# zaphB/freecad.optics_design_workbench

Measured on AMD Instinct MI355X. Metric: Monte-Carlo rays/sec (whole node), lensesAndMirrors.FCStd, higher is better.
Workload: dtype f64; 1 GPU; benchmark/lensesAndMirrors.FCStd, 1e+08 Monte-Carlo rays per step per GPU (BASELINE configs[2]), Gaussian point source sigma=1e-2, Philox4x32-10 seed 0x0D15EA5E; record_hit_rows=True, histogram=1024x1024 u64, parallelism=ray-index sharding x1, one RCCL reduce

## Files before the change

freecad/optics_design_workbench_amd/_native.py:

```python
import ctypes as C
import os
import shutil
import subprocess

import numpy as np

os.environ.setdefault('GPU_MAX_HW_QUEUES', '16')

_HERE = os.path.dirname(os.path.abspath(__file__))
CSRC = os.path.join(_HERE, 'csrc')
LIB_PATH = os.path.join(CSRC, 'libodw_trace.so')
_SOURCES = ['odw_capi.hip', 'odw_kernels.hip', 'odw_grid.hip', 'odw_mesh.hip', 'odw_posthoc.hip', 'odw_posthoc_batch.hip', 'odw_spec.hip', 'odw_device.h', 'odw_build.h']
_HEADER = os.path.normpath(os.path.join(_HERE, '..', '..', 'include', 'odw_trace.h'))

ABI_VERSION = 12
CNT_NAMES = ['traced_rays', 'recorded_hits', 'segments', 'escaped', 'died', 'capped',
             'hist_overflow', 'hits_dropped', 'grating_in_medium']
TRACE_RECORD_HITS, TRACE_HISTOGRAM, TRACE_RECORD_SEGMENTS, TRACE_POWER_HISTOGRAM = 1, 2, 4, 8
POWER_QUANTUM_BITS = 32
FLAG_FLIP_NORMAL, FLAG_CONVEX = 1, 2
COMPILE_OFF, COMPILE_STRUCTURE, COMPILE_AUTO = 0, 1, 2
COMPILE_MODES = {None: 0, False: 0, 'off': 0, 0: 0, 'structure': 1, 1: 1, True: 1, 'auto': 2, 2: 2}
ERRORS = {1: 'invalid argument', 2: 'device error', 3: 'no scene', 4: 'capacity', 5: 'unsupported'}
BUSY = 6

HIT_DTYPE = np.dtype([('point', '<f8', 3), ('direction', '<f8', 3), ('power', '<f8'), ('tag', '<u8')])
SEGMENT_DTYPE = np.dtype([('p1', '<f8', 3), ('p2', '<f8', 3), ('power', '<f8'), ('tag', '<u8')])

SYMBOLS = ['odw_abi_version', 'odw_create', 'odw_destroy', 'odw_last_error', 'odw_upload_scene',
           'odw_upload_source', 'odw_upload_surface_source', 'odw_generate_rays', 'odw_upload_surface_samplers', 'odw_set_surface_seed', 'odw_set_wavelength', 'odw_set_limits', 'odw_set_detector', 'odw_reserve_hits', 'odw_reserve_segments', 'odw_trace',
           'odw_trace_rays', 'odw_sync', 'odw_reset_results', 'odw_reset_hits', 'odw_fetch_counters', 'odw_hit_count',
           'odw_fetch_hits', 'odw_fetch_histogram', 'odw_segment_count', 'odw_fetch_segments', 'odw_reset_segments', 'odw_sample', 'odw_device_histogram',
           'odw_device_counters', 'odw_device_results', 'odw_stream', 'odw_timing_enable', 'odw_timing_read',
           'odw_swap_hit_lists', 'odw_fetch_swapped_hits', 'odw_release_swapped_hits', 'odw_mem_info', 'odw_host_alloc', 'odw_host_free', 'odw_load_hits', 'odw_hits_select', 'odw_hits_gather', 'odw_hits_project', 'odw_hits_range', 'odw_hits_bin', 'odw_hits_moments', 'odw_plane_screen',
           'odw_compile_scene', 'odw_compiled_info', 'odw_compile_check', 'odw_build_check', 'odw_hits_columns',
           'odw_upload_scene_batch', 'odw_trace_batch', 'odw_batch_select', 'odw_batch_rows',
           'odw_plane_screen_batch', 'odw_archive_append', 'odw_archive_select', 'odw_archive_reset', 'odw_batch_hits_select', 'odw_batch_hits_sample', 'odw_batch_hits_project', 'odw_batch_hits_bin',
           'odw_batch_reserve', 'odw_batch_hits_begin', 'odw_batch_hits_sampled', 'odw_batch_hits_measure', 'odw_batch_hits_measured',
           'odw_enable_power_histogram', 'odw_fetch_power_histogram', 'odw_device_power_histogram', 'odw_hits_bin_power', 'odw_compiled_power_info']

_pd = C.POINTER(C.c_double)
_pi = C.POINTER(C.c_int32)
_pu = C.POINTER(C.c_uint64)


class SceneDesc(C.Structure):
  _fields_ = [('n_prims', C.c_int32), ('prim_type', _pi), ('prim_group', _pi), ('prim_solid', _pi),
              ('prim_flags', _pi), ('prim_xform', _pd), ('prim_params', _pd), ('prim_cond_off', _pi),
              ('n_conds', C.c_int32), ('cond_prim', _pi), ('cond_inside', _pi),
              ('n_groups', C.c_int32), ('group_type', _pi), ('group_ior', _pd), ('group_refl', _pd),
              ('group_abslen', _pd), ('group_record', _pi), ('group_grating_type', _pi),
              ('group_grating_lpm', _pd), ('group_grating_dir', _pd), ('group_grating_order', _pi),
              ('seq_enabled', C.c_int32), ('seq_len', C.c_int32), ('seq_mask', _pu),
              ('ignore_mask', C.c_uint64), ('tri_normals', _pd), ('tri_edges', _pi)]


class SourceDesc(C.Structure):
  _fields_ = [('xform', C.c_double * 12), ('focal_length', C.c_double), ('wavelength', C.c_double),
              ('power', C.c_double), ('n_phi_knots', C.c_int32), ('phi_edges', _pd), ('phi_cdf', _pd),
              ('n_t_knots', C.c_int32), ('n_t_rows', C.c_int32), ('t_edges', _pd), ('t_cdf', _pd)]


class SurfaceSamplerDesc(C.Structure):
  _fields_ = [('group', C.c_int32), ('kind', C.c_int32), ('family_axis', C.c_int32), ('n_family', C.c_int32),
              ('family_lo', C.c_double), ('family_hi', C.c_double), ('n_phi_knots', C.c_int32),
              ('phi_edges', _pd), ('phi_cdf', _pd), ('n_t_knots', C.c_int32), ('n_t_rows', C.c_int32),
              ('t_edges', _pd), ('t_cdf', _pd), ('mu', C.c_double), ('n_atoms', C.c_int32),
              ('atom_mass', _pd), ('atom_theta', _pd), ('atom_phi', _pd)]


class SurfaceSourceDesc(C.Structure):
  _fields_ = [('wavelength', C.c_double), ('power', C.c_double), ('dist_tol', C.c_double),
              ('n_prims', C.c_int32), ('prim_type', _pi), ('prim_flags', _pi), ('prim_xform', _pd),
              ('prim_params', _pd), ('prim_cond_off', _pi), ('n_conds', C.c_int32), ('cond_prim', _pi),
              ('cond_inside', _pi), ('n_faces', C.c_int32), ('face_prim', _pi), ('face_id', _pi),
              ('face_area', _pd), ('n_t_knots', C.c_int32), ('t_edges', _pd), ('t_cdf', _pd), ('tri_normals', _pd)]


class LimitsDesc(C.Structure):
  _fields_ = [('max_ray_length', C.c_double), ('max_intersections', C.c_int32),
              ('dist_tol', C.c_double), ('power_tol', C.c_double)]


class DetectorDesc(C.Structure):
  _fields_ = [('group', C.c_int32), ('origin', C.c_double * 3), ('ex', C.c_double * 3),
              ('ey', C.c_double * 3), ('x_lo', C.c_double), ('x_hi', C.c_double),
              ('y_lo', C.c_double), ('y_hi', C.c_double), ('nx', C.c_int32), ('ny', C.c_int32)]


class NativeError(RuntimeError):
  pass


def hipcc():
  for cand in (os.environ.get('HIPCC'), '/opt/rocm/bin/hipcc', shutil.which('hipcc')):
    if cand and os.path.exists(cand):
      return cand
  raise NativeError('hipcc not found; the HIP library cannot be built')


def sources_hash(csrc=None, header=None):
  import hashlib
  csrc = CSRC if csrc is None else csrc
  header = _HEADER if header is None else header
  h = hashlib.sha256()
  for name in sorted(_SOURCES):
    path = os.path.join(csrc, name)
    h.update(name.encode() + b'\0')
    with open(path, 'rb') as f:
      h.update(f.read())
    h.update(b'\0')
  h.update(b'odw_trace.h\0')
  with open(header, 'rb') as f:
    h.update(f.read())
  return h.hexdigest()


def needs_build():
# ... 27 lines not shown
  runtime = subprocess.run([hipcc(), '--print-file-name=libclang_rt.asan-x86_64.so'], capture_output=True, text=True).stdout.strip()
  if not os.path.isabs(runtime) or not os.path.exists(runtime):
    raise NativeError('the sanitizer runtime of hipcc\'s clang was not found')
  deps = [os.path.join(CSRC, s) for s in _SOURCES] + [_HEADER]
  if force or not os.path.exists(ASAN_LIB_PATH) or any(os.path.getmtime(d) > os.path.getmtime(ASAN_LIB_PATH) for d in deps):
    cmd = [hipcc(), '--offload-arch=gfx950', '-O1', '-g', '-std=c++17', '-ffp-contract=on', '-fPIC', '-shared',
           '-fsanitize=address,undefined', '-fno-gpu-sanitize', '-fno-omit-frame-pointer', '-shared-libasan',
           '-o', ASAN_LIB_PATH + '.tmp', os.path.join(CSRC, 'odw_capi.hip')]
    res = subprocess.run(cmd, cwd=CSRC, capture_output=True, text=True)
    if res.returncode != 0:
      raise NativeError('hipcc (sanitized build) failed:\n' + res.stdout + res.stderr)
    os.replace(ASAN_LIB_PATH + '.tmp', ASAN_LIB_PATH)
  return ASAN_LIB_PATH, runtime


_lib = None


def lib():
  global _lib
  if _lib is None:
    if not os.path.exists(LIB_PATH):
      raise NativeError(f'{LIB_PATH} is missing: run __graft_entry__.build() '
                        f'(or freecad.optics_design_workbench_amd._native.build()) first')
    l = C.CDLL(os.environ.get('ODW_TRACE_LIB') or LIB_PATH)
    l.odw_last_error.restype = C.c_char_p
    l.odw_last_error.argtypes = [C.c_void_p]
    l.odw_create.argtypes = [C.c_int, C.POINTER(C.c_void_p)]
    l.odw_destroy.argtypes = [C.c_void_p]
    l.odw_destroy.restype = None
    for name in SYMBOLS:
      getattr(l, name)
    if l.odw_abi_version() != ABI_VERSION:
      raise NativeError('libodw_trace.so ABI version mismatch; rebuild')
    _lib = l
  return _lib


def check(ctx, rc, what):
  if rc != 0:
    msg = lib().odw_last_error(ctx)
    raise NativeError(f'{what}: {ERRORS.get(rc, rc)}: {msg.decode() if msg else ""}')


def _arr(a, dtype):
  return np.ascontiguousarray(a, dtype=dtype)


def scene_desc(sc):
  keep = dict(
      prim_type=_arr(sc.prim_type, np.int32), prim_group=_arr(sc.prim_group, np.int32),
      prim_solid=_arr(sc.prim_solid, np.int32), prim_flags=_arr(sc.prim_flags, np.int32),
      prim_xform=_arr(sc.prim_xform, np.float64), prim_params=_arr(sc.prim_params, np.float64),
      prim_cond_off=_arr(sc.prim_cond_off, np.int32), cond_prim=_arr(sc.cond_prim, np.int32),
      cond_inside=_arr(sc.cond_inside, np.int32), group_type=_arr(sc.group_type, np.int32),
      group_ior=_arr(sc.group_ior, np.float64), group_refl=_arr(sc.group_refl, np.float64),
      group_abslen=_arr(sc.group_abslen, np.float64), group_record=_arr(sc.group_record, np.int32),
      group_grating_type=_arr(sc.group_grating_type, np.int32),
      group_grating_lpm=_arr(sc.group_grating_lpm, np.float64),
      group_grating_dir=_arr(sc.group_grating_dir, np.float64),
      group_grating_order=_arr(sc.group_grating_order, np.int32),
      seq_mask=_arr(sc.seq_mask, np.uint64))
  if getattr(sc, 'tri_normals', None) is not None:
    keep_tri = _arr(sc.tri_normals, np.float64).reshape(-1, 9)
    if len(keep_tri) != len(sc.prim_type):
      raise ValueError('tri_normals needs one row of 9 values per primitive')
  d = SceneDesc()
  d.n_prims, d.n_conds, d.n_groups = len(keep['prim_type']), len(keep['cond_prim']), len(keep['group_type'])
  for name, typ in SceneDesc._fields_:
    if name in keep:
      setattr(d, name, keep[name].ctypes.data_as(typ))
  d.seq_enabled, d.seq_len, d.ignore_mask = int(sc.seq_enabled), len(keep['seq_mask']), int(sc.ignore_mask)
  if getattr(sc, 'tri_normals', None) is not None:
    keep['tri_normals'] = keep_tri
    d.tri_normals = keep_tri.ctypes.data_as(_pd)
  if getattr(sc, 'tri_edges', None) is not None:
    keep['tri_edges'] = _arr(sc.tri_edges, np.int32)
    if len(keep['tri_edges']) != len(sc.prim_type):
      raise ValueError('tri_edges needs one entry per primitive')
    d.tri_edges = keep['tri_edges'].ctypes.data_as(_pi)
  return d, keep


def compile_check(scene, limits, mode='structure', arch=None):
  d, keep = scene_desc(scene)
  lim = LimitsDesc(float(limits.max_ray_length), int(limits.max_intersections), float(limits.dist_tol),
                   float(limits.power_tol))
  buf = C.create_string_buffer(1 << 20)
  size = C.c_uint64(0)
  f = lib().odw_compile_check
  f.argtypes = [C.POINTER(SceneDesc), C.POINTER(LimitsDesc), C.c_int32, C.c_char_p, C.c_char_p, C.c_uint64,
                C.POINTER(C.c_uint64)]
  rc = f(C.byref(d), C.byref(lim), COMPILE_MODES[mode], arch.encode() if arch else None, buf, len(buf), C.byref(size))
  check(None, rc, 'odw_compile_check')
  return buf.value.decode(), int(size.value)


STRUCTURES = {0: 'flat', 1: 'grid', 2: 'bvh', 3: 'wide-bvh'}


def build_check(scene, limits, library=None):
  d, keep = scene_desc(scene)
  lim = LimitsDesc(float(limits.max_ray_length), int(limits.max_intersections), float(limits.dist_tol),
                   float(limits.power_tol))
  structure = C.c_int32(-1)
  sizes = (C.c_uint64 * 6)()
  f = (library or lib()).odw_build_check
  f.argtypes = [C.POINTER(SceneDesc), C.POINTER(LimitsDesc), C.POINTER(C.c_int32), C.POINTER(C.c_uint64)]
  rc = f(C.byref(d), C.byref(lim), C.byref(structure), sizes)
  if rc != 0:
    msg = (library or lib()).odw_last_error(None)
    raise NativeError(f'odw_build_check: {ERRORS.get(rc, rc)}: {msg.decode() if msg else ""}')
  names = ('primitives', 'nodes', 'grid_cells', 'grid_items', 'grid_lds_bytes', 'dead_primitives')
  return dict(structure=STRUCTURES[int(structure.value)], **{k: int(v) for k, v in zip(names, sizes)})


def source_desc(src):
  t = src.tables
  keep = dict(phi_edges=_arr(t.phi_edges, np.float64), phi_cdf=_arr(t.phi_cdf, np.float64),
              t_edges=_arr(t.t_edges, np.float64), t_cdf=_arr(t.t_cdf, np.float64).reshape(-1, len(t.t_edges)))
  d = SourceDesc()
  d.xform = (C.c_double * 12)(*np.asarray(src.xform, dtype=np.float64).reshape(12))
  d.focal_length, d.wavelength, d.power = float(src.focal_length), float(src.wavelength), float(src.power)
  d.n_phi_knots, d.n_t_knots, d.n_t_rows = len(keep['phi_edges']), len(keep['t_edges']), keep['t_cdf'].shape[0]
  for name in keep:
    setattr(d, name, keep[name].ctypes.data_as(_pd))
  return d, keep


def surface_sampler_descs(samplers):
  samplers = list(samplers or [])
  arr = (SurfaceSamplerDesc * max(1, len(samplers)))()
  keep = [arr]
  for d, s in zip(arr, samplers):
    phi_edges, phi_cdf = _arr(s.phi_edges, np.float64), _arr(s.phi_cdf, np.float64)
    t_edges, t_cdf = _arr(s.t_edges, np.float64), _arr(s.t_cdf, np.float64)
    keep += [phi_edges, phi_cdf, t_edges, t_cdf]
    d.group, d.kind, d.family_axis, d.n_family = int(s.group), int(s.kind), int(s.axis), int(s.n_family)
    d.family_lo, d.family_hi = float(s.lo), float(s.hi)
    d.n_phi_knots, d.n_t_knots, d.n_t_rows = len(phi_edges), len(t_edges), int(t_cdf.shape[-2])
    for name, a in (('phi_edges', phi_edges), ('phi_cdf', phi_cdf), ('t_edges', t_edges), ('t_cdf', t_cdf)):
      setattr(d, name, a.ctypes.data_as(_pd))
    d.mu = float(getattr(s, 'mu', 0.0))
    d.n_atoms = int(getattr(s, 'n_atoms', 0) or 0)
    if d.n_atoms:
      for name in ('atom_mass', 'atom_theta', 'atom_phi'):
        a = _arr(getattr(s, name), np.float64)
        keep.append(a)
        setattr(d, name, a.ctypes.data_as(_pd))
  return arr, len(samplers), keep


def surface_source_desc(src):
  keep = dict(prim_type=_arr(src.prim_type, np.int32), prim_flags=_arr(src.prim_flags, np.int32),
              prim_xform=_arr(src.prim_xform, np.float64), prim_params=_arr(src.prim_params, np.float64),
              prim_cond_off=_arr(src.prim_cond_off, np.int32),
              cond_prim=_arr(src.cond_prim if len(src.cond_prim) else [0], np.int32),
              cond_inside=_arr(src.cond_inside if len(src.cond_inside) else [0], np.int32),
              face_prim=_arr(src.face_prim, np.int32), face_id=_arr(src.face_id, np.int32),
              face_area=_arr(src.face_area, np.float64), t_edges=_arr(src.t_edges, np.float64),
              t_cdf=_arr(src.t_cdf, np.float64))
  if getattr(src, 'tri_normals', None) is not None:
    keep['tri_normals'] = _arr(src.tri_normals, np.float64).reshape(-1, 9)
    if len(keep['tri_normals']) != len(keep['prim_type']):
      raise ValueError('tri_normals needs one row of 9 values per primitive')
  d = SurfaceSourceDesc()
  d.wavelength, d.power, d.dist_tol = float(src.wavelength), float(src.power), float(src.dist_tol)
  d.n_prims, d.n_conds, d.n_faces = len(keep['prim_type']), len(src.cond_prim), len(keep['face_prim'])
  d.n_t_knots = len(keep['t_edges'])
  for name, typ in SurfaceSourceDesc._fields_:
    if name in keep:
      setattr(d, name, keep[name].ctypes.data_as(typ))
  return d, keep
```

freecad/optics_design_workbench_amd/csrc/odw_build.h:

```cpp
#pragma once

#include <algorithm>
#include <cmath>
#include <cstdint>
#include <cstdio>
#include <cstring>
#include <limits>
#include <map>
#include <string>
#include <utility>
#include <vector>

namespace {

using namespace odw;

struct HostScene {
  std::vector<double> prim_f64;
  std::vector<int32_t> prim_i32;
  std::vector<int32_t> cond;
  std::vector<double> prim_hdr;
  std::vector<char> dead;
  std::vector<double> group_f64, group_gdir;
  std::vector<int32_t> group_i32;
  std::vector<uint64_t> seq;
  bool lean = false;
  int32_t n_prims = 0, n_groups = 0, seq_enabled = 0, seq_len = 0;
  uint64_t all_mask = 0, ignore_mask = 0;
};

inline int refuse(std::string& err, int code, const char* msg) {
  err = msg;
  return code;
}

int32_t pack_cond(int32_t prim, int32_t inside) {
  return (int32_t)((uint32_t)prim | ((uint32_t)(inside >> 1) & 1u) << 30 | ((uint32_t)inside & 1u) << 31);
}

bool clauses_marked(const int32_t* cond_off, int n, const std::vector<int32_t>& cond) {
  for (int p = 0; p < n; ++p) {
    const int off = cond_off[p], end = cond_off[p + 1];
    if (end <= off || cond_opens(cond[off])) continue;
    for (int c = off + 1; c < end; ++c)
      if (cond_opens(cond[c])) return false;
  }
  return true;
}

int scene_host_tables(const odw_scene_desc* s, HostScene& hs, std::string& err) {
  if (!s) return refuse(err, ODW_ERR_INVALID, "odw_upload_scene: null argument");
  if (s->n_prims < 0 || s->n_groups < 0 || s->n_groups > ODW_MAX_GROUPS || s->seq_len < 0 ||
      s->seq_len > ODW_MAX_SEQUENCE || s->n_conds < 0 || s->n_conds >= (1 << 24))
    return refuse(err, ODW_ERR_INVALID, "odw_upload_scene: counts out of range");
  if ((s->n_prims > 0 && (!s->prim_type || !s->prim_group || !s->prim_flags || !s->prim_xform || !s->prim_params ||
                          !s->prim_cond_off)) ||
      (s->n_conds > 0 && (!s->cond_prim || !s->cond_inside)) ||
      (s->n_groups > 0 && (!s->group_type || !s->group_ior || !s->group_refl || !s->group_abslen || !s->group_record)) ||
      (s->seq_len > 0 && !s->seq_mask))
    return refuse(err, ODW_ERR_INVALID, "odw_upload_scene: null table pointer");
  const int n = s->n_prims;
  int max_solid = 0;
  for (int p = 0; p < n && s->prim_solid; ++p) max_solid = std::max(max_solid, s->prim_solid[p]);
  hs.prim_f64.assign((size_t)n * 16, 0.0);
  hs.prim_i32.assign((size_t)n * 4, 0);
  for (int p = 0; p < n; ++p) {
    const int type = s->prim_type[p], group = s->prim_group[p];
    if (type < ODW_PRIM_BOX || type > ODW_PRIM_PARABOLOID) return refuse(err, ODW_ERR_UNSUPPORTED, "unknown primitive type");
    if (group < 0 || group >= s->n_groups) return refuse(err, ODW_ERR_INVALID, "primitive group out of range");
    const int off = s->prim_cond_off[p], cnt = s->prim_cond_off[p + 1] - off;
    if (off < 0 || cnt < 0 || cnt > 255 || off + cnt > s->n_conds)
      return refuse(err, ODW_ERR_INVALID, "bad condition offsets");
    if (type == ODW_PRIM_TRIANGLE) {
      if (cnt) return refuse(err, ODW_ERR_UNSUPPORTED, "triangles cannot carry trimming conditions");
      const double* v = s->prim_xform + 12 * (size_t)p;
      double* d = &hs.prim_f64[16 * (size_t)p];
      double e1[3], e2[3], e3[3], nn[3];
      for (int k = 0; k < 3; ++k) { d[k] = v[k]; e1[k] = v[3 + k] - v[k]; e2[k] = v[6 + k] - v[k]; e3[k] = e2[k] - e1[k]; }
      nn[0] = e1[1] * e2[2] - e1[2] * e2[1];
      nn[1] = e1[2] * e2[0] - e1[0] * e2[2];
      nn[2] = e1[0] * e2[1] - e1[1] * e2[0];
      const double a2 = std::sqrt(nn[0] * nn[0] + nn[1] * nn[1] + nn[2] * nn[2]);
      if (!(a2 > 0) || !std::isfinite(a2)) return refuse(err, ODW_ERR_INVALID, "degenerate triangle");
      auto len3 = [](const double* x) { return std::sqrt(x[0] * x[0] + x[1] * x[1] + x[2] * x[2]); };
      for (int k = 0; k < 3; ++k) { d[3 + k] = e1[k]; d[6 + k] = e2[k]; d[9 + k] = nn[k] / a2; }
      d[12] = len3(e2) / a2;
      d[13] = len3(e1) / a2;
      d[14] = len3(e3) / a2;
      const int face_edges = s->tri_edges ? s->tri_edges[p] : 7;
      for (int k = 0; k < 3; ++k)
        if (!((face_edges >> k) & 1)) d[12 + k] = -d[12 + k];
      d[15] = 0.0;
    } else {
      std::memcpy(&hs.prim_f64[16 * (size_t)p], s->prim_xform + 12 * (size_t)p, 12 * sizeof(double));
      std::memcpy(&hs.prim_f64[16 * (size_t)p + 12], s->prim_params + 4 * (size_t)p, 4 * sizeof(double));
      if (type == ODW_PRIM_SPHERE) {
        const double* m = &hs.prim_f64[16 * (size_t)p];
        for (int k = 0; k < 3; ++k)
          hs.prim_f64[16 * (size_t)p + 13 + k] = -(m[k] * m[3] + m[4 + k] * m[7] + m[8 + k] * m[11]);
      }
      if (type == ODW_PRIM_PARABOLOID) {
        double* par = &hs.prim_f64[16 * (size_t)p + 12];
        if (!(par[0] > 0) || !(par[1] > 0)) return refuse(err, ODW_ERR_INVALID, "paraboloid: focal length and height must be positive");
        par[2] = 2.0 * std::sqrt(par[0] * par[1]);
      }
    }
    hs.prim_i32[4 * p] = type;
    hs.prim_i32[4 * p + 1] = group;
    const int solid = s->prim_solid ? s->prim_solid[p] : 0;
    const bool fits = s->prim_solid && solid >= 0 && solid < 0x7fff && max_solid < 0x7fff;
    hs.prim_i32[4 * p + 2] = ((s->prim_flags[p] & 0xffff & ~ODW_FLAG_ISOLATED) & (fits ? ~0 : ~ODW_FLAG_CONVEX)) | ((fits ? solid : 0x7fff) << ODW_SOLID_SHIFT);
    hs.prim_i32[4 * p + 3] = off | (cnt << 24);
  }
  std::vector<int32_t> cond((size_t)std::max(1, s->n_conds), 0);
  for (int c = 0; c < s->n_conds; ++c) {
    if (s->cond_prim[c] < 0 || s->cond_prim[c] >= n || s->cond_prim[c] >= (1 << 30))
      return refuse(err, ODW_ERR_INVALID, "condition primitive out of range");
    if (s->prim_type[s->cond_prim[c]] == ODW_PRIM_TRIANGLE)
      return refuse(err, ODW_ERR_UNSUPPORTED, "trimming against a triangle (no inside/outside of a facet)");
    if (s->cond_inside[c] < 0 || s->cond_inside[c] > 3)
      return refuse(err, ODW_ERR_INVALID, "cond_inside: bit 0 inside, bit 1 opens a clause; nothing else");
    cond[c] = pack_cond(s->cond_prim[c], s->cond_inside[c]);
  }
  if (!clauses_marked(s->prim_cond_off, n, cond))
    return refuse(err, ODW_ERR_INVALID, "a trimming list of several clauses must mark its first condition too");
  hs.cond = cond;
  std::vector<double> gf(ODW_MAX_GROUPS * 4, 0.0), gd(ODW_MAX_GROUPS * 3, 0.0);
  std::vector<int32_t> gi(ODW_MAX_GROUPS * 4, 0);
  hs.lean = true;
  for (int g = 0; g < s->n_groups; ++g)
// ... 868 lines not shown
```

freecad/optics_design_workbench_amd/csrc/odw_capi.hip:

```cpp
#include <hip/hip_runtime.h>
#include <hipcub/hipcub.hpp>

#include <algorithm>
#include <atomic>
#include <array>
#include <cmath>
#include <cstdio>
#include <cstdlib>
#include <cstring>
#include <condition_variable>
#include <functional>
#include <mutex>
#include <new>
#include <thread>
#include <string>
#include <utility>
#include <vector>

#include "odw_kernels.hip"
#include "odw_grid.hip"
#include "odw_mesh.hip"
#include "odw_build.h"

using namespace odw;

namespace {

constexpr int kGuide = 1 << 16;
constexpr uint32_t kHitBlock = 512;
constexpr uint64_t kHitBlockMinRows = 1ull << 16;
static inline uint64_t hit_block_room(uint64_t capacity, uint64_t waves, uint64_t block) { return capacity * 64 / block + 64 + waves * block; }
constexpr int kPhiGuide = 1 << 8;
constexpr int kSurfaceGuide = 1 << 10;
constexpr int kBvhThreshold = 64;

std::string g_error;

struct DevBuf {
  void* p = nullptr;
  size_t bytes = 0;
};

}

struct odw_ctx {
  int device = 0;
  hipStream_t stream = nullptr;
  void* up_pin = nullptr;
  size_t up_off = 0;
  bool up_unstaged = false;
  int n_cu = 256;
  std::string err;

  HostScene hs;
  int compile_mode = 0;
  bool spec_dirty = true;
  hipFunction_t spec_fn = nullptr;
  bool spec_lean = false, spec_stoch = false;
  bool spec_pending = false;
  std::string spec_key;
  uint64_t spec_hot_rays = 50000000;
  double spec_seconds = 0;
  int spec_cache_hit = 0;
  bool have_scene = false, have_source = false, have_limits = false;
  bool bvh_dirty = true;
  int flat_limit = kBvhThreshold;

  DevBuf prim_f64, prim_hdr, prim_i32, cond_i32, group_f64, group_i32, group_gdir, seq_mask;
  DevBuf bvh_nodes, bvh_prims, tri_nrm;
  DevBuf bvh_leaf, bvh_wide;
  DevBuf grid_bounds, grid_cells, grid_items, dbg;
  DevBuf phi_tab, t_tab, t_guide, phi_guide, d_source, d_det;
  DeviceSource h_source;
  DeviceDetector h_det;
  DevBuf hits, hit_count, chunk_counter;
  DevBuf results, hist, counters;
  DevBuf segs, seg_count;
  uint64_t seg_capacity = 0;
  DevBuf ray_o, ray_d, ray_p, ray_aos, samp_t, samp_phi;
  DevBuf sort_keys[2], sort_vals[2], sort_tmp, sorted_rows;
  DevBuf ph_sel_entering, ph_flags, ph_x, ph_y, ph_sorted, ph_small, ph_part, ph_edges, ph_edges_b, ph_counts, ph_sel_hist;
  DevBuf ph_accel;
  DevBuf ph_bitmap, ph_before, ph_row_of;
  uint64_t alt_hit_ray_end = 0;
  uint64_t hit_ray_end = 0;
  uint64_t hit_ray_begin = 0, alt_hit_ray_begin = 0;
  uint64_t ph_n = 0, ph_n_entering = 0;
  int ph_group = -1;
  bool ph_valid = false, ph_projected = false, ph_entering_built = false;
  std::vector<double> ph_moment_sums;
  unsigned ph_moment_grid = 0;
  struct SurfaceBufs { DevBuf phi_tab, t_tab, t_guide, atom_mass; };
  std::vector<SurfaceBufs> surf_bufs;
  DevBuf d_samplers, d_group_sampler;
  int n_samplers = 0;
  uint64_t surface_seed = 0;
  DevBuf em_prim_f64, em_prim_i32, em_cond, em_face_i32, em_face_cdf, em_t_tab, em_t_guide, em_o, em_d, em_tri_nrm;
  DeviceEmitter h_emitter;
  bool emitter_active = false;
  uint64_t hit_capacity = 0, n_bins = 0;
  bool power_on = false;
  uint64_t hit_slots = 0;
  DevBuf batch_values, batch_hits, batch_hit_count, batch_rays_buf;
  int batch_n = 0;
  size_t batch_prims = 0;
  bool batch_launch = false;
  uint64_t batch_stride = 0;
  uint64_t batch_seg_slots = 0, batch_seg_capacity = 0, batch_rays = 0, batch_first = 0;
  int batch_traced = 0;
  bool batch_rows_ok = false;
  bool batch_marked = false;
  bool batch_pts = false;
  int batch_selected = -1;
  std::string batch_spec_text;
  hipFunction_t spec_batch_fn = nullptr;
  bool spec_batch_failed = false;
  hipFunction_t spec_power_fn = nullptr;
  bool spec_power_failed = false;
  const std::atomic<bool>* spec_power_wait = nullptr;
  DevBuf own_hits, own_hit_count;
  uint64_t own_capacity = 0, own_slots = 0, own_ray_begin = 0, own_ray_end = 0;
  DevBuf archive, archive_count;
  uint64_t archive_slots = 0, archive_unused = 0, archive_ray_begin = 0, archive_ray_end = 0;
  bool archive_selected = false;
  DevBuf phb_row_of, phb_words, phb_sel, phb_small, phb_rows, phb_x, phb_y, phb_part, phb_sel_hist, phb_cand, phb_counts;
  DevBuf phb_scenes, phb_hist, phb_planes, phb_strides, phb_origins, phb_accel, phb_pts;
  void* phb_pin_p = nullptr;
  size_t phb_pin_bytes = 0;
  hipEvent_t phb_ev = nullptr;
  int phb_stage = 0, phb_S = 0;
  uint64_t phb_cap = 0, phb_nbins = 0, phb_keep = 0;
  size_t phb_part_stride = 0;
  std::vector<double> phb_edges_host;
  int phb_edges_na = 0, phb_edges_nb = 0, phb_edges_polar = -1;
  std::vector<uint64_t> phb_used, phb_n, phb_leaving;
  std::vector<int32_t> phb_ordered;
  std::vector<char> phb_on;
  uint64_t phb_xy_stride = 0;
  int phb_group = -1;
// ... 179 lines not shown
  const uint64_t row = t >> 2;
  if (row < n) {
    const double2* src = reinterpret_cast<const double2*>(hits + order[row]);
    reinterpret_cast<double2*>(out + row)[t & 3] = src[t & 3];
  }
}

}
#include "odw_spec.hip"
namespace {

int presort_rays(odw_ctx* ctx, uint64_t first, uint64_t n, uint64_t seed) {
  const bool off = getenv("ODW_MESH_PRESORT") && getenv("ODW_MESH_PRESORT")[0] == '0';
  const char* e_min = getenv("ODW_MESH_PRESORT_MIN");
  const uint64_t min_rays = e_min ? (uint64_t)atoll(e_min) : (1ull << 16);
  if (off || n < min_rays || n > 0x7FFFFFFFull) return ODW_OK;
  int rc;
  for (int k = 0; k < 2; ++k) {
    if ((rc = ensure(ctx, ctx->sort_keys[k], n * sizeof(uint64_t)))) return rc;
    if ((rc = ensure(ctx, ctx->sort_vals[k], n * sizeof(uint32_t)))) return rc;
  }
  const DeviceScene& sc = ctx->P.scene;
  double lo[3], scale[3];
  for (int a = 0; a < 3; ++a) {
    lo[a] = sc.wide_lo[a];
    const double w = sc.wide_hi[a] - sc.wide_lo[a];
    scale[a] = w > 0 ? 1024.0 / w : 0.0;
  }
  uint64_t* k_in = (uint64_t*)ctx->sort_keys[0].p;
  uint64_t* k_out = (uint64_t*)ctx->sort_keys[1].p;
  uint32_t* v_in = (uint32_t*)ctx->sort_vals[0].p;
  uint32_t* v_out = (uint32_t*)ctx->sort_vals[1].p;
  const bool dir_only = ctx->h_source.finite_focal && ctx->h_source.focal_length == 0.0;
  const unsigned kgrid = (unsigned)((n + 255) / 256);
  size_t tmp_bytes = 0;
  if (dir_only) {
    uint32_t* k32_in = (uint32_t*)k_in;
    uint32_t* k32_out = (uint32_t*)k_out;
    hipLaunchKernelGGL(odw_ray_key_kernel<uint32_t>, dim3(kgrid), dim3(256), 0, ctx->stream, ctx->P.source, first, n, seed,
                       lo[0], lo[1], lo[2], scale[0], scale[1], scale[2], k32_in, v_in);
    HIPCHK(ctx, hipGetLastError());
    HIPCHK(ctx, hipcub::DeviceRadixSort::SortPairs(nullptr, tmp_bytes, k32_in, k32_out, v_in, v_out, (int)n, 0, 32, ctx->stream));
    if ((rc = ensure(ctx, ctx->sort_tmp, tmp_bytes))) return rc;
    HIPCHK(ctx, hipcub::DeviceRadixSort::SortPairs(ctx->sort_tmp.p, tmp_bytes, k32_in, k32_out, v_in, v_out, (int)n, 0, 32, ctx->stream));
  } else {
    hipLaunchKernelGGL(odw_ray_key_kernel<uint64_t>, dim3(kgrid), dim3(256), 0, ctx->stream, ctx->P.source, first, n, seed,
                       lo[0], lo[1], lo[2], scale[0], scale[1], scale[2], k_in, v_in);
    HIPCHK(ctx, hipGetLastError());
    HIPCHK(ctx, hipcub::DeviceRadixSort::SortPairs(nullptr, tmp_bytes, k_in, k_out, v_in, v_out, (int)n, 0, 62, ctx->stream));
    if ((rc = ensure(ctx, ctx->sort_tmp, tmp_bytes))) return rc;
    HIPCHK(ctx, hipcub::DeviceRadixSort::SortPairs(ctx->sort_tmp.p, tmp_bytes, k_in, k_out, v_in, v_out, (int)n, 0, 62, ctx->stream));
  }
  ctx->P.ray_order = v_out;
  ctx->ph_valid = false;
  return ODW_OK;
}


enum class TraceKernel { flat = kAccelFlat, grid = kAccelGrid, tree = kAccelTree, mesh = kAccelWide, compiled };

TraceKernel choose_kernel(const odw_ctx* ctx, uint32_t flags, bool batch) {
  const DeviceScene& S = ctx->P.scene;
  const bool segments = (flags & ODW_TRACE_RECORD_SEGMENTS) != 0, stoch = ctx->n_samplers > 0;
  const hipFunction_t fn = batch ? ctx->spec_batch_fn : (flags & ODW_TRACE_POWER_HISTOGRAM) ? ctx->spec_power_fn : ctx->spec_fn;
  if (fn && ctx->spec_lean == ctx->hs.lean && ctx->spec_stoch == stoch && !segments) return TraceKernel::compiled;
  return (TraceKernel)accel_kind(ctx->P.grid.nx > 0 && !stoch && !segments, S.n_nodes != 0, S.bvh_leaf != nullptr && !segments);
}

int launch_trace(odw_ctx* ctx, uint64_t first, uint64_t n, uint64_t seed, uint32_t flags,
                 const double* ray_o, const double* ray_d, const double* ray_p) {
  const bool explicit_rays = ray_o != nullptr;
  if (!ctx->have_scene || !ctx->have_limits) return fail(ctx, ODW_ERR_NO_SCENE, "scene/limits not uploaded");
  if (!explicit_rays && !ctx->have_source) return fail(ctx, ODW_ERR_NO_SCENE, "source not uploaded");
  if (n == 0) return ODW_OK;
  ctx->ph_valid = false;
  if (!ctx->batch_launch) {
    ctx->hit_ray_begin = ctx->hit_ray_end ? std::min<uint64_t>(ctx->hit_ray_begin, first) : first;
    ctx->hit_ray_end = std::max<uint64_t>(ctx->hit_ray_end, std::min<uint64_t>(first + n, 1ull << 48));
  }
  if (ctx->bvh_dirty) {
    int rc = build_bvh(ctx);
    if (rc) return rc;
  }
  if (ctx->spec_dirty) {
    if (spec_bind(ctx) != ODW_OK) ctx->spec_fn = nullptr;
  }
  if ((flags & ODW_TRACE_RECORD_HITS) && (ctx->batch_launch ? ctx->batch_seg_capacity : ctx->hit_capacity) == 0)
    return fail(ctx, ODW_ERR_CAPACITY, "ODW_TRACE_RECORD_HITS without odw_reserve_hits");
  if (flags & ODW_TRACE_RECORD_SEGMENTS) {
    if (ctx->seg_capacity == 0)
      return fail(ctx, ODW_ERR_CAPACITY, "ODW_TRACE_RECORD_SEGMENTS without odw_reserve_segments");
    if (first + n > ODW_SEG_MAX_RAY || ctx->P.lim.max_intersections > ODW_SEG_MAX_ORDINAL)
      return fail(ctx, ODW_ERR_INVALID, "ODW_TRACE_RECORD_SEGMENTS: ray index or max_intersections beyond the row tag");
  }
  if ((flags & ODW_TRACE_HISTOGRAM) && !ctx->P.det_enabled) flags &= ~ODW_TRACE_HISTOGRAM;
  if (!(flags & ODW_TRACE_HISTOGRAM) || !ctx->power_on) flags &= ~(uint32_t)ODW_TRACE_POWER_HISTOGRAM;
  TraceParams& P = ctx->P;
  const bool batch = ctx->batch_launch;
  std::memset(&P.batch, 0, sizeof P.batch);
  if (batch) {
    if (P.scene.n_nodes || P.grid.nx > 0 || ctx->n_samplers > 0 || explicit_rays || (flags & ODW_TRACE_RECORD_SEGMENTS))
      return fail(ctx, ODW_ERR_UNSUPPORTED, "odw_trace_batch: batches are traced by the flat kernels (analytic scenes of up to 64 "
                                            "primitives, no stochastic surfaces, no segment rows)");
    flags &= ~(uint32_t)(ODW_TRACE_HISTOGRAM | ODW_TRACE_POWER_HISTOGRAM);
  }
  P.first_ray = first;
  P.n_rays = n;
  P.seed = seed;
  P.flags = flags;
  P.samplers = (const DeviceSurfaceSampler*)ctx->d_samplers.p;
  P.group_sampler = (const int32_t*)ctx->d_group_sampler.p;
  P.ray_origins = ray_o;
  P.ray_dirs = ray_d;
  P.ray_powers = ray_p;
  P.ray_stride = n;
  P.dbg = (unsigned long long*)ctx->dbg.p;
  P.out.hits = (odw_hit*)(batch ? ctx->batch_hits.p : ctx->hits.p);
  P.out.hit_capacity = batch ? ctx->batch_seg_slots : ctx->hit_slots;
  P.out.hit_block = 0;
  P.out.hit_count = (unsigned long long*)(batch ? ctx->batch_hit_count.p : ctx->hit_count.p);
  P.out.hist = (unsigned long long*)ctx->hist.p;
  P.out.counters = (unsigned long long*)ctx->counters.p;
  P.out.chunk_counter = (unsigned long long*)ctx->chunk_counter.p;
  P.out.segs = (odw_segment*)ctx->segs.p;
  P.out.seg_capacity = ctx->seg_capacity;
  P.out.seg_count = (unsigned long long*)ctx->seg_count.p;
  P.out.row_of = (batch && ctx->batch_marked && (flags & ODW_TRACE_RECORD_HITS)) ? (uint32_t*)ctx->phb_row_of.p : nullptr;
  P.out.row_stride = batch ? (n + 31) / 32 * 32 : 0;
  P.out.pts = (P.out.row_of && ctx->batch_pts) ? (double*)ctx->phb_pts.p : nullptr;

  constexpr int grid_mult = 8;
  const bool pw = (flags & ODW_TRACE_POWER_HISTOGRAM) != 0;
  if (pw && ctx->spec_fn && !ctx->spec_power_fn && !ctx->spec_power_failed &&
      !(ctx->spec_power_wait && !ctx->spec_power_wait->load())) {
    const std::string keep_err = ctx->err;
    const bool waited = ctx->spec_power_wait != nullptr;
    ctx->spec_power_wait = nullptr;
    if (spec_bind(ctx, kSpecPower) != ODW_OK || (!ctx->spec_power_fn && (waited || !ctx->spec_power_wait))) {
      ctx->spec_power_fn = nullptr;
      ctx->spec_power_failed = true;
      ctx->err = keep_err;
    }
  }
  if (batch && ctx->spec_fn && !ctx->spec_batch_fn && !ctx->spec_batch_failed) {
    const std::string keep_err = ctx->err;
    if (spec_bind(ctx, kSpecBatch) != ODW_OK) {
      ctx->spec_batch_fn = nullptr;
      ctx->spec_batch_failed = true;
      ctx->err = keep_err;
    }
  }
  const TraceKernel kernel = choose_kernel(ctx, flags, batch);
  const bool use_spec = kernel == TraceKernel::compiled, use_grid = kernel == TraceKernel::grid, use_mesh = kernel == TraceKernel::mesh,
             use_tree = kernel == TraceKernel::tree;
  {
    const bool ring = use_grid || use_mesh;
    const uint64_t waves = (uint64_t)ctx->n_cu * 16;
    const uint64_t want = ring ? std::max<uint64_t>(64, std::min<uint64_t>(256, n / (waves * 32)))
                               : std::max<uint64_t>(512, std::min<uint64_t>(1024, n / (waves * 4)));
    P.chunk = (uint32_t)(want & ~(uint64_t)63);
  }
  uint64_t n_chunks = (n + P.chunk - 1) / P.chunk;
  if (batch) {
    const uint64_t total = n * (uint64_t)ctx->batch_traced, waves = (uint64_t)ctx->n_cu * 16;
    P.chunk = (uint32_t)(std::max<uint64_t>(512, std::min<uint64_t>(1024, total / (waves * 4))) & ~(uint64_t)63);
    const uint64_t cps = (n + P.chunk - 1) / P.chunk;
// ... 254 lines not shown
  release(ctx->d_samplers);
  release(ctx->d_group_sampler);
  for (DevBuf* b : {&ctx->grid_bounds, &ctx->grid_cells, &ctx->grid_items}) release(*b);
  for (DevBuf* b : {&ctx->ph_bitmap, &ctx->ph_before, &ctx->ph_row_of}) release(*b);
  for (DevBuf* b : {&ctx->ph_sel_entering, &ctx->ph_flags, &ctx->ph_x, &ctx->ph_y, &ctx->ph_sorted, &ctx->ph_small,
                    &ctx->ph_part, &ctx->ph_edges, &ctx->ph_edges_b, &ctx->ph_counts, &ctx->ph_sel_hist, &ctx->ph_accel})
    release(*b);
  release(ctx->archive);
  release(ctx->archive_count);
  release(ctx->batch_values);
  release(ctx->batch_rays_buf);
  release(ctx->batch_hits);
  release(ctx->batch_hit_count);
  if (ctx->phb_pin_p) (void)hipHostFree(ctx->phb_pin_p);
  if (ctx->up_pin) (void)hipHostFree(ctx->up_pin);
  if (ctx->phb_ev) (void)hipEventDestroy(ctx->phb_ev);
  for (DevBuf* b : {&ctx->phb_row_of, &ctx->phb_words, &ctx->phb_sel, &ctx->phb_small, &ctx->phb_rows, &ctx->phb_x, &ctx->phb_y,
                    &ctx->phb_part, &ctx->phb_sel_hist, &ctx->phb_cand, &ctx->phb_counts, &ctx->phb_scenes, &ctx->phb_hist, &ctx->phb_planes,
                    &ctx->phb_strides, &ctx->phb_origins, &ctx->phb_accel, &ctx->phb_pts})
    release(*b);
  release(ctx->alt_hits);
  release(ctx->alt_hit_count);
  if (ctx->alt_ready) (void)hipEventDestroy(ctx->alt_ready);
  if (ctx->copy_stream) (void)hipStreamDestroy(ctx->copy_stream);
  if (ctx->stream) (void)hipStreamDestroy(ctx->stream);
  delete ctx;
}


int odw_upload_scene(odw_ctx* ctx, const odw_scene_desc* s) {
  if (!ctx) return fail(ctx, ODW_ERR_INVALID, "odw_upload_scene: null argument");
  HostScene hs;
  std::string err;
  int rc = scene_host_tables(s, hs, err);
  if (rc) return fail(ctx, rc, err);
  ctx->hs = std::move(hs);
  HIPCHK(ctx, hipSetDevice(ctx->device));
  const int n = s->n_prims;
  const std::vector<int32_t>& cond = ctx->hs.cond;
  const std::vector<double>&gf = ctx->hs.group_f64, &gd = ctx->hs.group_gdir;
  const std::vector<int32_t>& gi = ctx->hs.group_i32;
  const std::vector<uint64_t>& seq = ctx->hs.seq;
  if ((rc = upload(ctx, ctx->prim_f64, ctx->hs.prim_f64.data(), ctx->hs.prim_f64.size() * sizeof(double)))) return rc;
  if ((rc = upload(ctx, ctx->prim_i32, ctx->hs.prim_i32.data(), ctx->hs.prim_i32.size() * sizeof(int32_t)))) return rc;
  if ((rc = upload(ctx, ctx->cond_i32, cond.data(), cond.size() * sizeof(int32_t)))) return rc;
  if ((rc = upload(ctx, ctx->group_f64, gf.data(), gf.size() * sizeof(double)))) return rc;
  if ((rc = upload(ctx, ctx->group_i32, gi.data(), gi.size() * sizeof(int32_t)))) return rc;
  if ((rc = upload(ctx, ctx->group_gdir, gd.data(), gd.size() * sizeof(double)))) return rc;
  if ((rc = upload(ctx, ctx->seq_mask, seq.data(), seq.size() * sizeof(uint64_t)))) return rc;
  if (s->tri_normals && n > 0) {
    if ((rc = upload(ctx, ctx->tri_nrm, s->tri_normals, (size_t)n * 9 * sizeof(double)))) return rc;
  }
  if ((rc = upload_done(ctx))) return rc;
  DeviceScene& d = ctx->P.scene;
  d.n_prims = ctx->hs.n_prims;
  d.n_groups = ctx->hs.n_groups;
  d.n_nodes = 0;
  d.seq_enabled = ctx->hs.seq_enabled;
  d.seq_len = ctx->hs.seq_len;
  d.all_mask = ctx->hs.all_mask;
  d.ignore_mask = ctx->hs.ignore_mask;
  d.tri_nrm = (s->tri_normals && n > 0) ? (const double*)ctx->tri_nrm.p : nullptr;
  d.prim_f64 = (const double*)ctx->prim_f64.p;
  d.prim_i32 = (const int32_t*)ctx->prim_i32.p;
  d.cond_i32 = (const int32_t*)ctx->cond_i32.p;
  d.group_f64 = (const double*)ctx->group_f64.p;
  d.group_i32 = (const int32_t*)ctx->group_i32.p;
  d.group_gdir = (const double*)ctx->group_gdir.p;
  d.seq_mask = (const uint64_t*)ctx->seq_mask.p;
  ctx->have_scene = true;
  ctx->bvh_dirty = true;
  ctx->spec_dirty = true;
  ctx->spec_fn = nullptr;
  ctx->n_samplers = 0;
  ctx->batch_n = 0;
  return ODW_OK;
}

int odw_compile_scene(odw_ctx* ctx, int32_t mode) {
  if (!ctx || mode < ODW_COMPILE_OFF || mode > ODW_COMPILE_AUTO) return fail(ctx, ODW_ERR_INVALID, "odw_compile_scene: bad argument");
  ctx->compile_mode = mode;
  ctx->spec_dirty = true;
  ctx->spec_fn = nullptr;
  if (mode == ODW_COMPILE_OFF || !ctx->have_scene || !ctx->have_limits) return ODW_OK;
  HIPCHK(ctx, hipSetDevice(ctx->device));
  if (ctx->bvh_dirty) {
    int rc = build_bvh(ctx);
    if (rc) return rc;
  }
  return spec_bind(ctx);
}

int odw_compiled_info(odw_ctx* ctx, int32_t* bound, double* compile_seconds, int32_t* cache_hit) {
  if (!ctx) return fail(ctx, ODW_ERR_INVALID, "odw_compiled_info: null context");
  if (bound) *bound = (ctx->spec_fn && !ctx->spec_dirty && !ctx->bvh_dirty) ? ctx->compile_mode : 0;
  if (compile_seconds) *compile_seconds = ctx->spec_seconds;
  if (cache_hit) *cache_hit = ctx->spec_cache_hit;
  return ODW_OK;
}

int odw_compiled_power_info(odw_ctx* ctx, int32_t* bound) {
  if (!ctx || !bound) return fail(ctx, ODW_ERR_INVALID, "odw_compiled_power_info: bad argument");
  *bound = (ctx->spec_fn && ctx->spec_power_fn && !ctx->spec_dirty && !ctx->bvh_dirty) ? ctx->compile_mode : 0;
  return ODW_OK;
}

int odw_compile_check(const odw_scene_desc* scene, const odw_limits* limits, int32_t mode, const char* arch,
                      char* header_out, uint64_t header_capacity, uint64_t* code_bytes) {
  if (!scene || !limits || mode != ODW_COMPILE_STRUCTURE)
    return fail(nullptr, ODW_ERR_INVALID, "odw_compile_check: bad argument");
  HostScene tmp;
  std::string refusal;
  int rc = scene_host_tables(scene, tmp, refusal);
  if (rc) return fail(nullptr, rc, refusal);
  std::vector<Box> boxes;
  compute_boxes(tmp, limits->dist_tol, boxes);
  const std::string why = spec_ineligible(tmp);
  if (!why.empty()) return fail(nullptr, ODW_ERR_UNSUPPORTED, "odw_compile_check: " + why);
  const std::string text = spec_text(tmp, 0);
  if (header_out && header_capacity) {
    const size_t k = std::min<size_t>(text.size(), (size_t)header_capacity - 1);
    std::memcpy(header_out, text.data(), k);
    header_out[k] = 0;
  }
  std::vector<char> code;
  std::string err;
  if (!spec_compile(text, arch && *arch ? arch : "gfx950", code, err))
    return fail(nullptr, ODW_ERR_DEVICE, err);
  if (code_bytes) *code_bytes = code.size();
  return ODW_OK;
}

int odw_build_check(const odw_scene_desc* scene, const odw_limits* limits, int32_t* structure, uint64_t* sizes) {
  if (!scene || !limits) return fail(nullptr, ODW_ERR_INVALID, "odw_build_check: null argument");
  if (!(limits->dist_tol > 0) || limits->max_intersections < 0 || !(limits->max_ray_length > 0))
    return fail(nullptr, ODW_ERR_INVALID, "odw_build_check: limits out of range");
  int flat_limit = kBvhThreshold;
  if (const char* e = getenv("ODW_BVH_THRESHOLD")) flat_limit = atoi(e);
  HostScene tmp;
  SceneAccel A;
  std::string err;
  int rc = scene_host_tables(scene, tmp, err);
  if (!rc) {
    std::vector<Box> boxes;
    compute_boxes(tmp, limits->dist_tol, boxes);
    rc = build_accel(tmp, std::move(boxes), limits->dist_tol, flat_limit, build_options(), A, err);
  }
  if (rc) return fail(nullptr, rc, err);
  if (structure) *structure = A.kind();
  if (sizes) {
    uint64_t dead = 0;
    for (char d : tmp.dead) dead += d ? 1 : 0;
    sizes[0] = (uint64_t)tmp.n_prims;
    sizes[1] = (uint64_t)A.nodes.size();
    sizes[2] = (uint64_t)A.grid.nx * (uint64_t)A.grid.ny * (uint64_t)A.grid.nz;
    sizes[3] = (uint64_t)A.grid.n_items;
    sizes[4] = (uint64_t)A.grid.lds_bytes;
    sizes[5] = dead;
  }
  return ODW_OK;
}

int odw_upload_surface_samplers(odw_ctx* ctx, const odw_surface_sampler_desc* samplers, int32_t n) {
  if (!ctx || n < 0 || (n && !samplers)) return fail(ctx, ODW_ERR_INVALID, "odw_upload_surface_samplers: bad argument");
  if (!ctx->have_scene) return fail(ctx, ODW_ERR_NO_SCENE, "odw_upload_surface_samplers before odw_upload_scene");
  HIPCHK(ctx, hipSetDevice(ctx->device));
  if (n == 0 && ctx->n_samplers == 0) return ODW_OK;
  HIPCHK(ctx, hipStreamSynchronize(ctx->stream));
  ctx->n_samplers = 0;
  ctx->spec_dirty = true;
  if (n == 0) return ODW_OK;
  std::vector<int32_t> gs(ODW_MAX_GROUPS * 2, -1);
  std::vector<DeviceSurfaceSampler> ds((size_t)n);
  if ((int)ctx->surf_bufs.size() < n) ctx->surf_bufs.resize((size_t)n);
  for (int i = 0; i < n; ++i) {
    const odw_surface_sampler_desc& s = samplers[i];
    if (s.group < 0 || s.group >= ctx->P.scene.n_groups || s.kind < ODW_SURF_PRIMARY || s.kind > ODW_SURF_MODIFY)
      return fail(ctx, ODW_ERR_INVALID, "surface sampler: group/kind out of range");
    for (int j = gs[2 * s.group + s.kind]; j >= 0; j = ds[(size_t)j].next)
      if (ds[(size_t)j].mu == s.mu) return fail(ctx, ODW_ERR_INVALID, "surface sampler: duplicate (group, kind, mu)");
    if (s.n_atoms < 0 || s.n_atoms > ODW_SURF_MAX_ATOMS || (s.n_atoms && (!s.atom_mass || !s.atom_theta || !s.atom_phi)))
      return fail(ctx, ODW_ERR_INVALID, "surface sampler: atoms");
    for (int k = 0; k < s.n_family * s.n_atoms; ++k)
      if (!(s.atom_mass[k] >= 0.0 && s.atom_mass[k] <= 1.0)) return fail(ctx, ODW_ERR_INVALID, "surface sampler: atom probability outside [0, 1]");
    if (s.n_family < 1 || s.family_axis < ODW_SURF_AXIS_NONE || s.family_axis > ODW_SURF_AXIS_THETA_REFL ||
        (s.family_axis == ODW_SURF_AXIS_NONE && s.n_family != 1) ||
        (s.n_family > 1 && !(s.family_hi > s.family_lo)))
      return fail(ctx, ODW_ERR_INVALID, "surface sampler: family");
    if (s.n_phi_knots < 2 || s.n_t_knots < 2 || s.n_t_rows < 1 ||
        (s.n_t_rows != 1 && s.n_t_rows != s.n_phi_knots - 1))
      return fail(ctx, ODW_ERR_INVALID, "surface sampler: table shape");
    if (!s.phi_edges || !s.phi_cdf || !s.t_edges || !s.t_cdf)
      return fail(ctx, ODW_ERR_INVALID, "surface sampler: null table pointer");
    const size_t np = (size_t)s.n_phi_knots, nt = (size_t)s.n_t_knots, rows = (size_t)s.n_t_rows, nf = (size_t)s.n_family;
    std::vector<double> ptab(nf * np * 2), ttab(nf * rows * nt * 2);
    std::vector<int32_t> guide(nf * rows * (kSurfaceGuide + 1));
    for (size_t k = 0; k < nf; ++k) {
      const double* pc = s.phi_cdf + k * np;
      if (pc[0] != 0.0 || pc[np - 1] != 1.0) return fail(ctx, ODW_ERR_INVALID, "surface sampler: phi cdf must run from 0 to 1");
      for (size_t j = 0; j < np; ++j) {
        if (j && pc[j] < pc[j - 1]) return fail(ctx, ODW_ERR_INVALID, "surface sampler: cdf not monotone");
        ptab[(k * np + j) * 2] = pc[j];
        ptab[(k * np + j) * 2 + 1] = s.phi_edges[j];
      }
      for (size_t r = 0; r < rows; ++r) {
        const double* cdf = s.t_cdf + (k * rows + r) * nt;
        if (cdf[0] != 0.0 || cdf[nt - 1] != 1.0) return fail(ctx, ODW_ERR_INVALID, "surface sampler: theta cdf rows must run from 0 to 1");
        double* dst = ttab.data() + (k * rows + r) * nt * 2;
        for (size_t j = 0; j < nt; ++j) {
          if (j && cdf[j] < cdf[j - 1]) return fail(ctx, ODW_ERR_INVALID, "surface sampler: cdf not monotone");
          dst[2 * j] = cdf[j];
          dst[2 * j + 1] = s.t_edges[j];
        }
        int32_t* g = guide.data() + (k * rows + r) * (kSurfaceGuide + 1);
        size_t j = 0;
        for (int q = 0; q <= kSurfaceGuide; ++q) {
          const double x = (double)q / (double)kSurfaceGuide;
          while (j + 1 < nt && cdf[j + 1] <= x) ++j;
          g[q] = (int32_t)j;
        }
      }
    }
    odw_ctx::SurfaceBufs& sb = ctx->surf_bufs[(size_t)i];
    int rc;
    if ((rc = upload(ctx, sb.phi_tab, ptab.data(), ptab.size() * sizeof(double)))) return rc;
    if ((rc = upload(ctx, sb.t_tab, ttab.data(), ttab.size() * sizeof(double)))) return rc;
    if ((rc = upload(ctx, sb.t_guide, guide.data(), guide.size() * sizeof(int32_t)))) return rc;
    HIPCHK(ctx, hipStreamSynchronize(ctx->stream));
    DeviceSurfaceSampler& d = ds[(size_t)i];
    d.phi_tab = (const double*)sb.phi_tab.p;
    d.t_tab = (const double*)sb.t_tab.p;
    d.t_guide = (const int32_t*)sb.t_guide.p;
    d.n_phi_knots = s.n_phi_knots;
    d.n_t_knots = s.n_t_knots;
    d.n_t_rows = s.n_t_rows;
    d.n_guide = kSurfaceGuide;
    d.axis = s.family_axis;
    d.n_family = s.n_family;
    d.lo = s.family_lo;
    d.inv_step = s.n_family > 1 ? (double)(s.n_family - 1) / (s.family_hi - s.family_lo) : 0.0;
    d.mu = s.mu;
    d.n_atoms = s.n_atoms;
    d.atom_mass = nullptr;
    std::memset(d.atom_theta, 0, sizeof d.atom_theta);
    std::memset(d.atom_phi, 0, sizeof d.atom_phi);
    if (s.n_atoms) {
      if ((rc = upload(ctx, sb.atom_mass, s.atom_mass, (size_t)s.n_family * (size_t)s.n_atoms * sizeof(double)))) return rc;
      HIPCHK(ctx, hipStreamSynchronize(ctx->stream));
      d.atom_mass = (const double*)sb.atom_mass.p;
      for (int j = 0; j < s.n_atoms; ++j)
        for (int c = 0; c < 3; ++c) { d.atom_theta[j][c] = s.atom_theta[3 * j + c]; d.atom_phi[j][c] = s.atom_phi[3 * j + c]; }
    }
    d.next = gs[2 * s.group + s.kind];
    gs[2 * s.group + s.kind] = i;
  }
  int rc;
  if ((rc = upload(ctx, ctx->d_samplers, ds.data(), ds.size() * sizeof(DeviceSurfaceSampler)))) return rc;
  if ((rc = upload(ctx, ctx->d_group_sampler, gs.data(), gs.size() * sizeof(int32_t)))) return rc;
  HIPCHK(ctx, hipStreamSynchronize(ctx->stream));
  ctx->n_samplers = n;
  return ODW_OK;
}

int odw_set_wavelength(odw_ctx* ctx, double wavelength_nm) {
  if (!ctx || !(wavelength_nm > 0)) return fail(ctx, ODW_ERR_INVALID, "odw_set_wavelength: bad argument");
  ctx->P.wavelength = wavelength_nm;
  return ODW_OK;
}

int odw_set_surface_seed(odw_ctx* ctx, uint64_t seed) {
  if (!ctx) return fail(ctx, ODW_ERR_INVALID, "odw_set_surface_seed: null ctx");
  ctx->surface_seed = seed;
  return ODW_OK;
}

int odw_upload_source(odw_ctx* ctx, const odw_source_desc* s) {
  if (!ctx || !s) return fail(ctx, ODW_ERR_INVALID, "odw_upload_source: null argument");
  if (s->n_phi_knots < 2 || s->n_t_knots < 2 || s->n_t_rows < 1 ||
      (s->n_t_rows != 1 && s->n_t_rows != s->n_phi_knots - 1))
    return fail(ctx, ODW_ERR_INVALID, "odw_upload_source: table shape");
  if (!s->phi_edges || !s->phi_cdf || !s->t_edges || !s->t_cdf)
    return fail(ctx, ODW_ERR_INVALID, "odw_upload_source: null table pointer");
  HIPCHK(ctx, hipSetDevice(ctx->device));
  const int np = s->n_phi_knots, nt = s->n_t_knots, rows = s->n_t_rows;
  if (s->phi_cdf[0] != 0.0 || s->phi_cdf[np - 1] != 1.0)
    return fail(ctx, ODW_ERR_INVALID, "phi cdf must run from 0 to 1");
  std::vector<double> ptab((size_t)np * 2), ttab((size_t)rows * nt * 2);
  for (int i = 0; i < np; ++i) { ptab[2 * i] = s->phi_cdf[i]; ptab[2 * i + 1] = s->phi_edges[i]; }
  std::vector<int32_t> guide((size_t)rows * (kGuide + 1));
  for (int r = 0; r < rows; ++r) {
    const double* cdf = s->t_cdf + (size_t)r * nt;
    if (cdf[0] != 0.0 || cdf[nt - 1] != 1.0) return fail(ctx, ODW_ERR_INVALID, "theta cdf rows must run from 0 to 1");
    double* dst = ttab.data() + (size_t)r * nt * 2;
    for (int i = 0; i < nt; ++i) {
      if (i && cdf[i] < cdf[i - 1]) return fail(ctx, ODW_ERR_INVALID, "cdf not monotone");
      dst[2 * i] = cdf[i];
      dst[2 * i + 1] = s->t_edges[i];
    }
    int32_t* g = guide.data() + (size_t)r * (kGuide + 1);
    int j = 0;
    for (int k = 0; k <= kGuide; ++k) {
      const double x = (double)k / (double)kGuide;
      while (j + 1 < nt && cdf[j + 1] <= x) ++j;
      g[k] = j;
    }
  }
  int rc;
  if ((rc = upload(ctx, ctx->phi_tab, ptab.data(), ptab.size() * sizeof(double)))) return rc;
  if ((rc = upload(ctx, ctx->t_tab, ttab.data(), ttab.size() * sizeof(double)))) return rc;
  if ((rc = upload(ctx, ctx->t_guide, guide.data(), guide.size() * sizeof(int32_t)))) return rc;
  std::vector<int32_t> pguide(kPhiGuide + 1);
  for (int k = 0, j = 0; k <= kPhiGuide; ++k) {
    const double x = (double)k / (double)kPhiGuide;
    while (j + 1 < np && s->phi_cdf[j + 1] <= x) ++j;
    pguide[k] = j;
  }
  if ((rc = upload(ctx, ctx->phi_guide, pguide.data(), pguide.size() * sizeof(int32_t)))) return rc;
  HIPCHK(ctx, hipStreamSynchronize(ctx->stream));
  DeviceSource& d = ctx->h_source;
  std::memcpy(d.m, s->xform, sizeof d.m);
  d.focal_length = s->focal_length;
  d.finite_focal = std::isfinite(s->focal_length) ? 1 : 0;
  d.wavelength = s->wavelength;
  d.power = s->power;
  d.phi_tab = (const double*)ctx->phi_tab.p;
  d.t_tab = (const double*)ctx->t_tab.p;
  d.t_guide = (const int32_t*)ctx->t_guide.p;
  d.phi_guide = (const int32_t*)ctx->phi_guide.p;
  d.n_phi_guide = kPhiGuide;
  d.n_phi_knots = np;
  d.n_t_knots = nt;
  d.n_t_rows = rows;
  d.n_guide = kGuide;
  if ((rc = upload(ctx, ctx->d_source, &ctx->h_source, sizeof(DeviceSource)))) return rc;
  HIPCHK(ctx, hipStreamSynchronize(ctx->stream));
  ctx->P.source = (const DeviceSource*)ctx->d_source.p;
  ctx->P.wavelength = s->wavelength;
  ctx->have_source = true;
  ctx->emitter_active = false;
  return ODW_OK;
}

int odw_upload_surface_source(odw_ctx* ctx, const odw_surface_source_desc* s) {
  if (!ctx || !s) return fail(ctx, ODW_ERR_INVALID, "odw_upload_surface_source: null argument");
  if (s->n_prims < 1 || s->n_faces < 1 || s->n_conds < 0 || s->n_t_knots < 2 || !(s->dist_tol > 0))
    return fail(ctx, ODW_ERR_INVALID, "odw_upload_surface_source: counts out of range");
  if (!s->prim_type || !s->prim_flags || !s->prim_xform || !s->prim_params || !s->prim_cond_off || !s->face_prim ||
      !s->face_id || !s->face_area || !s->t_edges || !s->t_cdf || (s->n_conds > 0 && (!s->cond_prim || !s->cond_inside)))
    return fail(ctx, ODW_ERR_INVALID, "odw_upload_surface_source: null table pointer");
  HIPCHK(ctx, hipSetDevice(ctx->device));
  HIPCHK(ctx, hipStreamSynchronize(ctx->stream));
  const int n = s->n_prims;
  std::vector<double> pf((size_t)n * 16);
  std::vector<int32_t> pi((size_t)n * 4);
  for (int p = 0; p < n; ++p) {
    if (s->prim_type[p] < ODW_PRIM_BOX || s->prim_type[p] > ODW_PRIM_PARABOLOID)
      return fail(ctx, ODW_ERR_UNSUPPORTED, "surface source: unknown primitive kind");
    const int off = s->prim_cond_off[p], cnt = s->prim_cond_off[p + 1] - off;
    if (s->prim_type[p] == ODW_PRIM_TRIANGLE && cnt != 0)
      return fail(ctx, ODW_ERR_INVALID, "surface source: facets cannot carry trimming conditions");
    if (off < 0 || cnt < 0 || off + cnt > s->n_conds) return fail(ctx, ODW_ERR_INVALID, "surface source: bad condition offsets");
    std::memcpy(&pf[16 * (size_t)p], s->prim_xform + 12 * (size_t)p, 12 * sizeof(double));
    std::memcpy(&pf[16 * (size_t)p + 12], s->prim_params + 4 * (size_t)p, 4 * sizeof(double));
    pi[4 * p] = s->prim_type[p];
    pi[4 * p + 1] = s->prim_flags[p];
    pi[4 * p + 2] = off;
    pi[4 * p + 3] = cnt;
  }
  std::vector<int32_t> cond((size_t)std::max(1, s->n_conds), 0);
  for (int c = 0; c < s->n_conds; ++c) {
    if (s->cond_prim[c] < 0 || s->cond_prim[c] >= n || s->cond_prim[c] >= (1 << 30) ||
        s->prim_type[s->cond_prim[c]] == ODW_PRIM_TRIANGLE)
      return fail(ctx, ODW_ERR_INVALID, "surface source: condition primitive out of range");
    if (s->cond_inside[c] < 0 || s->cond_inside[c] > 3)
      return fail(ctx, ODW_ERR_INVALID, "surface source: cond_inside: bit 0 inside, bit 1 opens a clause; nothing else");
    cond[c] = pack_cond(s->cond_prim[c], s->cond_inside[c]);
  }
  if (!clauses_marked(s->prim_cond_off, n, cond))
    return fail(ctx, ODW_ERR_INVALID, "surface source: a trimming list of several clauses must mark its first condition too");
  static const int n_faces_of[7] = {6, 1, 3, 3, 1, 1, 0};
  std::vector<int32_t> fi((size_t)s->n_faces * 2);
  std::vector<double> fc((size_t)s->n_faces + 1, 0.0);
  double total = 0;
  for (int f = 0; f < s->n_faces; ++f) {
    const int p = s->face_prim[f];
    if (p < 0 || p >= n || s->face_id[f] < 0 || s->face_id[f] >= n_faces_of[s->prim_type[p]] || !(s->face_area[f] >= 0))
      return fail(ctx, ODW_ERR_INVALID, "surface source: face out of range");
    fi[2 * f] = p;
    fi[2 * f + 1] = s->face_id[f];
    total += s->face_area[f];
  }
  if (!(total > 0)) return fail(ctx, ODW_ERR_INVALID, "surface source: emitting faces have no area");
  double run = 0;
  for (int f = 0; f < s->n_faces; ++f) { run += s->face_area[f]; fc[f + 1] = run / total; }
  fc[s->n_faces] = 1.0;
  const int nt = s->n_t_knots;
  if (s->t_cdf[0] != 0.0 || s->t_cdf[nt - 1] != 1.0) return fail(ctx, ODW_ERR_INVALID, "surface source: theta cdf must run from 0 to 1");
  std::vector<double> ttab((size_t)nt * 2);
  for (int i = 0; i < nt; ++i) {
    if (i && s->t_cdf[i] < s->t_cdf[i - 1]) return fail(ctx, ODW_ERR_INVALID, "surface source: cdf not monotone");
    ttab[2 * i] = s->t_cdf[i];
    ttab[2 * i + 1] = s->t_edges[i];
  }
  std::vector<int32_t> guide((size_t)kGuide + 1);
  for (int k = 0, j = 0; k <= kGuide; ++k) {
    const double x = (double)k / (double)kGuide;
    while (j + 1 < nt && s->t_cdf[j + 1] <= x) ++j;
    guide[k] = j;
  }
  int rc;
  if ((rc = upload(ctx, ctx->em_prim_f64, pf.data(), pf.size() * sizeof(double)))) return rc;
  if ((rc = upload(ctx, ctx->em_prim_i32, pi.data(), pi.size() * sizeof(int32_t)))) return rc;
  if ((rc = upload(ctx, ctx->em_cond, cond.data(), cond.size() * sizeof(int32_t)))) return rc;
  if ((rc = upload(ctx, ctx->em_face_i32, fi.data(), fi.size() * sizeof(int32_t)))) return rc;
  if ((rc = upload(ctx, ctx->em_face_cdf, fc.data(), fc.size() * sizeof(double)))) return rc;
  if ((rc = upload(ctx, ctx->em_t_tab, ttab.data(), ttab.size() * sizeof(double)))) return rc;
  if ((rc = upload(ctx, ctx->em_t_guide, guide.data(), guide.size() * sizeof(int32_t)))) return rc;
  if (s->tri_normals && (rc = upload(ctx, ctx->em_tri_nrm, s->tri_normals, (size_t)n * 9 * sizeof(double)))) return rc;
  HIPCHK(ctx, hipStreamSynchronize(ctx->stream));
  DeviceEmitter& e = ctx->h_emitter;
  e.tri_nrm = s->tri_normals ? (const double*)ctx->em_tri_nrm.p : nullptr;
  e.prim_f64 = (const double*)ctx->em_prim_f64.p;
  e.prim_i32 = (const int32_t*)ctx->em_prim_i32.p;
  e.cond_i32 = (const int32_t*)ctx->em_cond.p;
  e.face_i32 = (const int32_t*)ctx->em_face_i32.p;
  e.face_cdf = (const double*)ctx->em_face_cdf.p;
  e.t_tab = (const double*)ctx->em_t_tab.p;
  e.t_guide = (const int32_t*)ctx->em_t_guide.p;
  e.n_faces = s->n_faces;
  e.n_t_knots = nt;
  e.n_guide = kGuide;
  e.dist_tol = s->dist_tol;
  e.wavelength = s->wavelength;
  e.power = s->power;
  ctx->P.wavelength = s->wavelength;
  ctx->have_source = true;
  ctx->emitter_active = true;
  return ODW_OK;
}

int odw_generate_rays(odw_ctx* ctx, uint64_t first_ray, uint64_t n_rays, uint64_t seed, double* origins,
                      double* directions) {
  if (!ctx || !origins || !directions) return fail(ctx, ODW_ERR_INVALID, "odw_generate_rays: bad argument");
  if (!ctx->have_source) return fail(ctx, ODW_ERR_NO_SCENE, "source not uploaded");
  HIPCHK(ctx, hipSetDevice(ctx->device));
  for (uint64_t off = 0; off < n_rays; off += kEmitChunk) {
    const uint64_t m = std::min<uint64_t>(kEmitChunk, n_rays - off);
    int rc;
    if (ctx->emitter_active) {
      if ((rc = emit_rays(ctx, first_ray + off, m, seed, false))) return rc;
    } else {
      if ((rc = ensure(ctx, ctx->em_o, m * 3 * sizeof(double)))) return rc;
      if ((rc = ensure(ctx, ctx->em_d, m * 3 * sizeof(double)))) return rc;
      const unsigned grid = (unsigned)std::max<uint64_t>(1, std::min<uint64_t>((m + 255) / 256, (uint64_t)ctx->n_cu * 16));
      hipLaunchKernelGGL(odw_make_rays_kernel, dim3(grid), dim3(256), 0, ctx->stream, ctx->P.source, first_ray + off,
                         m, seed, (double*)ctx->em_o.p, (double*)ctx->em_d.p);
      HIPCHK(ctx, hipGetLastError());
    }
    HIPCHK(ctx, hipMemcpyAsync(origins + 3 * off, ctx->em_o.p, m * 3 * sizeof(double), hipMemcpyDeviceToHost, ctx->stream));
    HIPCHK(ctx, hipMemcpyAsync(directions + 3 * off, ctx->em_d.p, m * 3 * sizeof(double), hipMemcpyDeviceToHost, ctx->stream));
    HIPCHK(ctx, hipStreamSynchronize(ctx->stream));
  }
  return ODW_OK;
}

int odw_set_limits(odw_ctx* ctx, const odw_limits* l) {
  if (!ctx || !l) return fail(ctx, ODW_ERR_INVALID, "odw_set_limits: null argument");
  if (!(l->dist_tol > 0) || l->max_intersections < 0 || !(l->max_ray_length > 0))
    return fail(ctx, ODW_ERR_INVALID, "odw_set_limits: values out of range");
  if (!ctx->have_limits || ctx->P.lim.dist_tol != l->dist_tol) {
    ctx->bvh_dirty = true;
    ctx->batch_n = 0;
  }
  ctx->P.lim.max_ray_length = l->max_ray_length;
  ctx->P.lim.max_intersections = l->max_intersections;
  ctx->P.lim.dist_tol = l->dist_tol;
  ctx->P.lim.power_tol = l->power_tol;
  ctx->have_limits = true;
  return ODW_OK;
}

int odw_set_detector(odw_ctx* ctx, const odw_detector_desc* det) {
  if (!ctx) return fail(ctx, ODW_ERR_INVALID, "odw_set_detector: null ctx");
  HIPCHK(ctx, hipSetDevice(ctx->device));
  DeviceDetector& d = ctx->h_det;
  ctx->power_on = false;
  if (!det) { d.enabled = 0; ctx->P.det_enabled = 0; ctx->n_bins = 0; return ODW_OK; }
  if (det->nx <= 0 || det->ny <= 0 || !(det->x_hi > det->x_lo) || !(det->y_hi > det->y_lo))
    return fail(ctx, ODW_ERR_INVALID, "odw_set_detector: bad window");
  ctx->det_desc = *det;
  for (int k = 0; k < 3; ++k) { d.origin[k] = det->origin[k]; d.ex[k] = det->ex[k]; d.ey[k] = det->ey[k]; }
  d.x_lo = det->x_lo;
  d.y_lo = det->y_lo;
  d.x_scale = det->nx / (det->x_hi - det->x_lo);
  d.y_scale = det->ny / (det->y_hi - det->y_lo);
  d.nx = det->nx;
  d.ny = det->ny;
  d.nx_f = (double)det->nx;
  d.ny_f = (double)det->ny;
  d.group = det->group;
  d.enabled = 1;
  ctx->n_bins = (uint64_t)det->nx * (uint64_t)det->ny;
  int rc = ensure_results(ctx, ctx->n_bins);
  if (rc) return rc;
  HIPCHK(ctx, hipStreamSynchronize(ctx->stream));
  if ((rc = upload(ctx, ctx->d_det, &ctx->h_det, sizeof(DeviceDetector)))) return rc;
  ctx->P.det = (const DeviceDetector*)ctx->d_det.p;
  ctx->P.det_enabled = 1;
  HIPCHK(ctx, hipMemsetAsync(ctx->hist.p, 0, ctx->n_bins * sizeof(uint64_t), ctx->stream));
  return ODW_OK;
}

int odw_reserve_hits(odw_ctx* ctx, uint64_t capacity) {
  if (!ctx) return fail(ctx, ODW_ERR_INVALID, "odw_reserve_hits: null ctx");
  HIPCHK(ctx, hipSetDevice(ctx->device));
  batch_unselect(ctx);
  HIPCHK(ctx, hipStreamSynchronize(ctx->stream));
  if (capacity == 0) { release(ctx->hits); ctx->hit_capacity = ctx->hit_slots = 0; return ODW_OK; }
  if (capacity > ctx->hit_capacity) {
    release(ctx->hits);
// ... 728 lines not shown
```

freecad/optics_design_workbench_amd/csrc/odw_kernels.hip:

```cpp
#include "odw_device.h"

namespace odw {

#define ODW_CONST __attribute__((address_space(4)))
typedef const double ODW_CONST* cf64;
typedef const int32_t ODW_CONST* ci32;
typedef const uint64_t ODW_CONST* cu64;
template <class T>
__device__ __forceinline__ const T ODW_CONST* as_const(const T* p) {
  return (const T ODW_CONST*)(uintptr_t)p;
}
template <class T>
__device__ __forceinline__ const T* opaque(const T* p) {
  asm volatile("" : "+s"(p));
  return p;
}
typedef const DeviceSource ODW_CONST* csource;
typedef const DeviceDetector ODW_CONST* cdetector;

__device__ __forceinline__ double frcp(double x) {
  double r = __builtin_amdgcn_rcp(x);
  r = fma(fma(-x, r, 1.0), r, r);
  r = fma(fma(-x, r, 1.0), r, r);
  return r;
}
__device__ __forceinline__ double frcp1(double x) {
  const double r = __builtin_amdgcn_rcp(x);
  return fma(fma(-x, r, 1.0), r, r);
}
__device__ __forceinline__ double fsqrt(double x) {
  const double y = __builtin_amdgcn_rsq(x);
  double g = x * y, h = 0.5 * y;
  const double r = fma(-h, g, 0.5);
  g = fma(g, r, g);
  h = fma(h, r, h);
  g = fma(fma(-g, g, x), h, g);
  return x > 0 ? g : 0.0;
}
__device__ __forceinline__ double frsqrt(double x) {
  double y = __builtin_amdgcn_rsq(x);
  y = y * fma(-0.5 * x * y, y, 1.5);
  y = y * fma(-0.5 * x * y, y, 1.5);
  return y;
}

__device__ __forceinline__ void philox4x32_10(uint32_t& c0, uint32_t& c1, uint32_t& c2,
                                              uint32_t& c3, uint32_t k0, uint32_t k1) {
#pragma unroll
  for (int r = 0; r < 10; ++r) {
    const uint64_t p0 = (uint64_t)0xD2511F53u * c0, p1 = (uint64_t)0xCD9E8D57u * c2;
    const uint32_t hi0 = (uint32_t)(p0 >> 32), lo0 = (uint32_t)p0;
    const uint32_t hi1 = (uint32_t)(p1 >> 32), lo1 = (uint32_t)p1;
    const uint32_t n0 = hi1 ^ c1 ^ k0, n2 = hi0 ^ c3 ^ k1;
    c0 = n0; c1 = lo1; c2 = n2; c3 = lo0;
    k0 += 0x9E3779B9u;
    k1 += 0xBB67AE85u;
  }
}

__device__ __forceinline__ double u53(uint32_t a, uint32_t b) {
  return ((double)(a >> 5) * 67108864.0 + (double)(b >> 6)) * (1.0 / 9007199254740992.0);
}

__device__ __forceinline__ void ray_uniforms(uint64_t ray, uint64_t seed, double& u_phi,
                                             double& u_t) {
  uint32_t c0 = (uint32_t)ray, c1 = (uint32_t)(ray >> 32), c2 = 0u, c3 = 0u;
  philox4x32_10(c0, c1, c2, c3, (uint32_t)seed, (uint32_t)(seed >> 32));
  u_phi = u53(c0, c1);
  u_t = u53(c2, c3);
}

__device__ __forceinline__ double inv_cdf(const double* __restrict__ tab, int lo, int hi, double u) {
#pragma clang fp contract(off)
  while (hi - lo > 1) {
    const int mid = (lo + hi) >> 1;
    if (u >= tab[2 * mid]) lo = mid; else hi = mid;
  }
  const double2 a = *reinterpret_cast<const double2*>(tab + 2 * lo);
  const double2 b = *reinterpret_cast<const double2*>(tab + 2 * lo + 2);
  if (a.x == u) return a.y;
  const double slope = (b.y - a.y) / (b.x - a.x);
  const double prod = slope * (u - a.x);
  return prod + a.y;
}

struct TableView {
  const double* phi_tab; const double* t_tab; const int32_t* t_guide;
  int n_phi_knots, n_t_knots, n_t_rows, n_guide;
  const int32_t* phi_guide; int n_phi_guide;
};
__device__ __forceinline__ void sample_tables(const TableView& s, double u_phi, double u_t,
                                              double& t_out, double& phi_out) {
#pragma clang fp contract(off)
  int plo = 0, phi_hi = s.n_phi_knots - 1;
  if (s.phi_guide) {
    const int k = (int)(u_phi * (double)s.n_phi_guide);
    plo = s.phi_guide[k];
    phi_hi = min(s.phi_guide[k + 1] + 1, s.n_phi_knots - 1);
  }
  const double phi = inv_cdf(s.phi_tab, plo, phi_hi, u_phi);
  int row = 0;
  if (s.n_t_rows > 1) {
    const double e0 = s.phi_tab[1], e1 = s.phi_tab[2 * (s.n_phi_knots - 1) + 1];
    int r = (int)floor((phi - e0) / (e1 - e0) * (double)s.n_t_rows);
    r = max(0, min(s.n_t_rows - 1, r));
    double best = INFINITY;
    for (int i = max(0, r - 1); i <= min(s.n_t_rows - 1, r + 1); ++i) {
      const double mid = (s.phi_tab[2 * (i + 1) + 1] + s.phi_tab[2 * i + 1]) / 2.0;
      const double d = fabs(mid - phi);
      if (d < best) { best = d; row = i; }
    }
  }
  const double* tab = s.t_tab + (size_t)row * (size_t)s.n_t_knots * 2;
  const int32_t* guide = s.t_guide + (size_t)row * (size_t)(s.n_guide + 1);
  const int k = (int)(u_t * (double)s.n_guide);
  const int lo = guide[k];
  const int hi = min(guide[k + 1] + 1, s.n_t_knots - 1);
  t_out = inv_cdf(tab, lo, hi, u_t);
  phi_out = phi;
}

__device__ __forceinline__ void sample_source(csource sp_, double u_phi, double u_t,
                                              double& t_out, double& phi_out) {
  TableView s;
  s.phi_tab = sp_->phi_tab; s.t_tab = sp_->t_tab; s.t_guide = sp_->t_guide;
  s.n_phi_knots = sp_->n_phi_knots; s.n_t_knots = sp_->n_t_knots; s.n_t_rows = sp_->n_t_rows; s.n_guide = sp_->n_guide;
  s.phi_guide = sp_->phi_guide; s.n_phi_guide = sp_->n_phi_guide;
  sample_tables(s, u_phi, u_t, t_out, phi_out);
}

template <class P>
__device__ __forceinline__ d3 xf_point(P m, d3 p) {
  return mk(m[0] * p.x + m[1] * p.y + m[2] * p.z + m[3],
            m[4] * p.x + m[5] * p.y + m[6] * p.z + m[7],
            m[8] * p.x + m[9] * p.y + m[10] * p.z + m[11]);
}
template <class P>
__device__ __forceinline__ d3 xf_vec(P m, d3 v) {
  return mk(m[0] * v.x + m[1] * v.y + m[2] * v.z, m[4] * v.x + m[5] * v.y + m[6] * v.z,
            m[8] * v.x + m[9] * v.y + m[10] * v.z);
}
template <class P>
__device__ __forceinline__ d3 xf_vec_t(P m, d3 v) {
  return mk(m[0] * v.x + m[4] * v.y + m[8] * v.z, m[1] * v.x + m[5] * v.y + m[9] * v.z,
            m[2] * v.x + m[6] * v.y + m[10] * v.z);
}

struct NoSpec {
  static constexpr bool enabled = false;
  static constexpr int N = 0;
  static constexpr unsigned long long xf(int) { return 0xfffull; }
  static constexpr int type(int) { return 0; }
  static constexpr int cond(int) { return 0; }
  static constexpr bool isolated() { return true; }
};
template <unsigned long long XF, int IA, int IB, int IC, int IT, class P>
__device__ __forceinline__ double xf_comb(P m, double a, double b, double c) {
  double acc = 0.0;
  bool have = false;
#define ODW_XF_TERM(I, V)                                                                            \
  if constexpr (((XF >> (I)) & 1ull) != 0) {                                                         \
    if constexpr (((XF >> (12 + (I))) & 1ull) != 0) acc = have ? acc + (V) : (V);                    \
    else if constexpr (((XF >> (24 + (I))) & 1ull) != 0) acc = have ? acc - (V) : -(V);              \
    else acc = have ? fma(m[I], (V), acc) : m[I] * (V);                                              \
    have = true;                                                                                     \
  }
  ODW_XF_TERM(IB, b)
  ODW_XF_TERM(IA, a)
  ODW_XF_TERM(IC, c)
#undef ODW_XF_TERM
  if constexpr (IT >= 0) {
    if constexpr (((XF >> (IT < 0 ? 0 : IT)) & 1ull) != 0) acc = have ? m[IT < 0 ? 0 : IT] + acc : m[IT < 0 ? 0 : IT];
  }
  return acc;
}
template <unsigned long long XF, class P>
__device__ __forceinline__ d3 xf_point_nz(P m, d3 p) {
  return mk(xf_comb<XF, 0, 1, 2, 3>(m, p.x, p.y, p.z), xf_comb<XF, 4, 5, 6, 7>(m, p.x, p.y, p.z),
            xf_comb<XF, 8, 9, 10, 11>(m, p.x, p.y, p.z));
}
template <unsigned long long XF, class P>
__device__ __forceinline__ d3 xf_vec_nz(P m, d3 v) {
  return mk(xf_comb<XF, 0, 1, 2, -1>(m, v.x, v.y, v.z), xf_comb<XF, 4, 5, 6, -1>(m, v.x, v.y, v.z),
            xf_comb<XF, 8, 9, 10, -1>(m, v.x, v.y, v.z));
}
template <unsigned long long XF, class P>
__device__ __forceinline__ d3 xf_vec_t_nz(P m, d3 v) {
  return mk(xf_comb<XF, 0, 4, 8, -1>(m, v.x, v.y, v.z), xf_comb<XF, 1, 5, 9, -1>(m, v.x, v.y, v.z),
            xf_comb<XF, 2, 6, 10, -1>(m, v.x, v.y, v.z));
}

__device__ __forceinline__ void sincos_bounded(double x, double& s, double& c) {
  const double k = rint(x * 0.63661977236758134308);
  double r = fma(-k, 1.5707963267948966, x);
  r = fma(-k, 6.123233995736766e-17, r);
  const double z = r * r;
  const double ps = 8.33333333332248946124e-03 + z * (-1.98412698298579493134e-04 + z * (2.75573137070700676789e-06 +
                    z * (-2.50507602534068634195e-08 + z * 1.58969099521155010221e-10)));
  const double sn = r + (z * r) * (-1.66666666666666324348e-01 + z * ps);
  const double pc = z * (4.16666666666666019037e-02 + z * (-1.38888888888741095749e-03 + z * (2.48015872894767294178e-05 +
                    z * (-2.75573143513906633035e-07 + z * (2.08757232129817482790e-09 + z * -1.13596475577881948265e-11)))));
  const double cs = 1.0 - (0.5 * z - z * pc);
  const int q = (int)k & 3;
  const double a = (q & 1) ? cs : sn, b = (q & 1) ? sn : cs;
  s = (q & 2) ? -a : a;
  c = ((q + 1) & 2) ? -b : b;
}

__device__ __forceinline__ void make_ray(csource s, double t_or_r, double phi,
                                         d3& origin, d3& dir) {
  d3 ldir, lorg;
  double sp, cp;
  sincos_bounded(phi, sp, cp);
  if (s->finite_focal) {
    double st, ct;
    sincos_bounded(t_or_r, st, ct);
    ldir = mk(st * sp, -st * cp, ct);
    lorg = (mk(0, 0, 1) - ldir) * s->focal_length;
  } else {
    ldir = mk(0, 0, 1);
    lorg = mk(t_or_r * cp, -t_or_r * sp, 0.0);
  }
  const d3 ln = ldir * frsqrt(dot(ldir, ldir));
  const d3 p1 = xf_point(s->m, lorg);
  const d3 p2 = xf_point(s->m, lorg + ln);
  const d3 d = p2 - p1;
  origin = p1;
  dir = d * frsqrt(dot(d, d));
}

template <bool PARAB, class PP>
__device__ __forceinline__ double prim_sdist(int type, PP par, d3 p) {
  if (PARAB && type == ODW_PRIM_PARABOLOID) {
    const double r2 = p.x * p.x + p.y * p.y;
    const double lat = (r2 - 4.0 * par[0] * p.z) * 0.5 * frsqrt(r2 + 4.0 * par[0] * par[0]);
    return fmax(lat, p.z - par[1]);
  }
  switch (type) {
    case ODW_PRIM_BOX: {
      const double dx = fmax(-p.x, p.x - par[0]);
      const double dy = fmax(-p.y, p.y - par[1]);
      const double dz = fmax(-p.z, p.z - par[2]);
      return fmax(dx, fmax(dy, dz));
    }
    case ODW_PRIM_SPHERE: return fsqrt(dot(p, p)) - par[0];
    case ODW_PRIM_CYLINDER: {
      const double rho = fsqrt(p.x * p.x + p.y * p.y);
      return fmax(rho - par[0], fmax(-p.z, p.z - par[1]));
    }
    case ODW_PRIM_CONE: {
      const double k = (par[1] - par[0]) / par[2];
      const double rho = fsqrt(p.x * p.x + p.y * p.y);
      const double lat = (rho - (par[0] + k * p.z)) * frsqrt(1 + k * k);
      return fmax(lat, fmax(-p.z, p.z - par[2]));
    }
    default: {
      const double rho = fsqrt(p.x * p.x + p.y * p.y);
      const double a = rho - par[0];
      return fsqrt(a * a + p.z * p.z) - par[1];
    }
  }
}

__device__ __forceinline__ double signed_like(double m, double s) { return __builtin_copysign(m, s + 0.0); }

__device__ __forceinline__ int quad_roots(double a, double bh, double c, double& t0, double& t1) {
  if (a == 0) {
    if (bh == 0) return 0;
    t0 = t1 = -c * frcp(2 * bh);
    return 1;
  }
  const double disc = bh * bh - a * c;
  if (!(disc >= 0)) return 0;
  const double sq = fsqrt(disc);
  const double q = -(bh + signed_like(sq, bh));
  const double r0 = q * frcp(a);
  const double r1 = (q != 0) ? c * frcp(q) : r0;
  t0 = fmin(r0, r1); t1 = fmax(r0, r1);
  return 2;
}
__device__ __forceinline__ int quad_roots_unit(double bh, double c, double& t0, double& t1) {
  const double disc = bh * bh - c;
  if (!(disc >= 0)) return 0;
  const double sq = fsqrt(disc);
  const double q = -(bh + signed_like(sq, bh));
  const double r1 = (q != 0) ? c * frcp(q) : q;
  t0 = fmin(q, r1); t1 = fmax(q, r1);
  return 2;
}

#ifndef ODW_DOUBLE
#define ODW_DOUBLE 0
#endif
__device__ __forceinline__ double opq(double x) { asm volatile("" : "+v"(x)); return x; }

struct Best {
  double t;
  int prim, face;
};
__device__ __forceinline__ bool better(double t, int p, int f, const Best& b) {
  return (bool)((int)(t < b.t) | ((int)(t == b.t) & ((int)(p < b.prim) | ((int)(p == b.prim) & (int)(f < b.face)))));
}

struct Query {
  d3 start, dn;
  double tol, tmax;
  int medium;
  bool in_medium;
// ... 247 lines not shown
    const d3 cc = o + d * t0;
    const double bound = (R1 + R2) * 1.0000001 + 1e-9;
    const double h2 = bound * bound - dot(cc, cc);
    if (!(h2 > 0)) return;
    double s_lo = -fsqrt(h2), s_hi = -s_lo;
    const double zs = R2 * 1.0000001 + 1e-9;
    if (d.z != 0) {
      const double iz = frcp(d.z);
      double a = (-zs - cc.z) * iz, b = (zs - cc.z) * iz;
      if (a > b) { const double tmp = a; a = b; b = tmp; }
      s_lo = fmax(s_lo, a);
      s_hi = fmin(s_hi, b);
    } else if (fabs(cc.z) > zs) {
      return;
    }
    if (!(s_hi > s_lo)) return;
    {
      const double xa = cc.x + s_lo * d.x, ya = cc.y + s_lo * d.y;
      const double xb = cc.x + s_hi * d.x, yb = cc.y + s_hi * d.y;
      const double rin = (R1 - R2) * 0.9999999 - 1e-9;
      if (rin > 0 && xa * xa + ya * ya < rin * rin && xb * xb + yb * yb < rin * rin) return;
    }
    const double s_begin = fmax(s_lo, 0.5 * tol - t0);
    const double step_min = 1e-7 * R2;
    double sc = s_begin, fc;
    {
      const double px = cc.x + sc * d.x, py = cc.y + sc * d.y, pz = cc.z + sc * d.z;
      const double a = fsqrt(px * px + py * py) - R1;
      fc = fsqrt(a * a + pz * pz) - R2;
    }
    int nfound = 0;
    double h = fmax(fabs(fc), step_min);
    for (int it = 0; it < 16384 && sc < s_hi && nfound < 4; ++it) {
      const double sn = fmin(sc + h, s_hi);
      double fn, rho;
      {
        const double px = cc.x + sn * d.x, py = cc.y + sn * d.y, pz = cc.z + sn * d.z;
        rho = fsqrt(px * px + py * py);
        const double a = rho - R1;
        fn = fsqrt(a * a + pz * pz) - R2;
      }
      h = fmax(fabs(fn), step_min);
      if (it >= ODW_TORUS_PLAIN && (fc > 0) == (fn > 0)) {
        const double hp = sn - sc, rr = fn + R2, room = 0.5 * fmin(rr, rho);
        if (hp <= room) {
          const double K = 2.0 * (frcp(rr) + frcp(rho));
          const double G = (fabs(fn) - fabs(fc)) * frcp(hp) - K * hp;
          const double hs = 0.99 * (G + fsqrt(G * G + 2.0 * K * fabs(fn))) * frcp(K);
          h = fmax(h, fmin(hs, room));
        }
      }
      if ((fc > 0) != (fn > 0)) {
        double lo = sc, hi = sn, x = sn;
        const bool lo_pos = fc > 0;
        for (int j = 0; j < 48; ++j) {
          const double px = cc.x + x * d.x, py = cc.y + x * d.y, pz = cc.z + x * d.z;
          const double rho = fsqrt(px * px + py * py);
          const double a = rho - R1;
          const double rr = fsqrt(a * a + pz * pz);
          const double f = rr - R2;
          if (f == 0) break;
          if ((f > 0) == lo_pos) lo = x; else hi = x;
          const double ir = frcp(rr * rho);
          const double df = (a * (px * d.x + py * d.y)) * ir + pz * d.z * frcp(rr);
          double xn = x - f * frcp(df);
          if (!(xn >= lo && xn <= hi)) xn = 0.5 * (lo + hi);
          const bool done = xn == x || (hi - lo) <= 4e-16 * (fabs(lo) + fabs(hi));
          x = xn;
          if (done) break;
        }
        const double tr = x + t0;
        if (nfound == 0) c.t0 = tr; else if (nfound == 1) c.t1 = tr; else if (nfound == 2) c.t2 = tr; else c.t3 = tr;
        ++nfound;
      }
      sc = sn;
      fc = fn;
    }
  }
  }
  if (cond_cnt == 0) {
    double bt = INFINITY;
    int bf = 0;
#define ODW_PICK(T, F) { const bool w_ = (bool)((int)((T) > tol) & ((int)((T) < bt) | ((int)((T) == bt) & (int)((F) < bf)))); bt = w_ ? (T) : bt; bf = w_ ? (F) : bf; }
    ODW_PICK(c.t0, c.f0)
    ODW_PICK(c.t1, c.f1)
    ODW_PICK(c.t2, c.f2)
    ODW_PICK(c.t3, c.f3)
#undef ODW_PICK
    if constexpr (SPEC::enabled) consider_spec<PARAB, SPEC, PI>(sv, q, bt, bf);
    else consider<PARAB>(sv, q, bt, p, bf, group, 0, 0);
  } else if constexpr (SPEC::enabled) {
    constexpr int fm = (SPEC::flags(PI) >> ODW_FACEMASK_SHIFT) & 0xff;
    constexpr bool quadric = SPEC::type(PI) == ODW_PRIM_CYLINDER || SPEC::type(PI) == ODW_PRIM_CONE || SPEC::type(PI) == ODW_PRIM_PARABOLOID;
    if constexpr (!quadric || (fm & 1) != 0) {
      consider_spec<PARAB, SPEC, PI>(sv, q, c.t0, c.f0);
      consider_spec<PARAB, SPEC, PI>(sv, q, c.t1, c.f1);
    }
    if constexpr (SPEC::type(PI) != ODW_PRIM_SPHERE) {
      if constexpr (!quadric || (fm & 2) != 0) consider_spec<PARAB, SPEC, PI>(sv, q, c.t2, c.f2);
      if constexpr (!quadric || (fm & 4) != 0) consider_spec<PARAB, SPEC, PI>(sv, q, c.t3, c.f3);
    }
  } else {
#pragma unroll 1
    for (int k = 0; k < 4; ++k) {
      const double t = k == 0 ? c.t0 : (k == 1 ? c.t1 : (k == 2 ? c.t2 : c.t3));
      const int f = k == 0 ? c.f0 : (k == 1 ? c.f1 : (k == 2 ? c.f2 : c.f3));
      consider<PARAB>(sv, q, t, p, f, group, cond_off, cond_cnt);
    }
  }
}

__device__ __forceinline__ double seg_dist2(d3 w, d3 e) {
#pragma clang fp contract(off)
  const double s = fmin(fmax(dot(w, e) / dot(e, e), 0.0), 1.0);
  const d3 r = w - e * s;
  return dot(r, r);
}

__device__ __forceinline__ void intersect_tri(const SceneView& sv, Query& q, int p, int group) {
  cf64 pf = sv.prim_f64 + (size_t)p * 16;
  const d3 e1 = mk(pf[3], pf[4], pf[5]), e2 = mk(pf[6], pf[7], pf[8]);
  const d3 pv = cross(q.dn, e2);
  const double det = dot(e1, pv);
  if (det == 0) return;
  const double inv = frcp(det);
  const d3 tv = q.start - mk(pf[0], pf[1], pf[2]);
  const double u = dot(tv, pv) * inv;
  const d3 qv = cross(tv, e1);
  const double v = dot(q.dn, qv) * inv;
  const double tol = q.tol;
  const double s0 = pf[12], s1 = pf[13], s2 = pf[14];
  if (u < -(s0 < 0 ? 1e-9 : tol * s0) || v < -(s1 < 0 ? 1e-9 : tol * s1) || u + v > 1.0 + (s2 < 0 ? 1e-9 : tol * s2)) return;
  if ((u < 0 && s0 >= 0) || (v < 0 && s1 >= 0) || (u + v > 1.0 && s2 >= 0)) {
#pragma clang fp contract(off)
    const d3 w = e1 * u + e2 * v;
    double best = seg_dist2(w, e1);
    best = fmin(best, seg_dist2(w, e2));
    best = fmin(best, seg_dist2(w - e1, e2 - e1));
    if (best > tol * tol) return;
  }
  consider(sv, q, dot(e2, qv) * inv, p, 0, group, 0, 0);
}

__device__ __forceinline__ d3 tri_normal(cf64 pf, const double* __restrict__ vn, d3 gp) {
  const d3 ng = mk(pf[9], pf[10], pf[11]);
  if (!vn) return ng;
  const d3 e1 = mk(pf[3], pf[4], pf[5]), e2 = mk(pf[6], pf[7], pf[8]);
  const d3 tv = gp - mk(pf[0], pf[1], pf[2]);
  const d3 nn = cross(e1, e2);
  const double inv = frcp(dot(nn, nn));
  const double u = dot(cross(tv, e2), nn) * inv, v = dot(cross(e1, tv), nn) * inv;
  const double w = 1.0 - u - v;
  const d3 n = mk(w * vn[0] + u * vn[3] + v * vn[6], w * vn[1] + u * vn[4] + v * vn[7],
                  w * vn[2] + u * vn[5] + v * vn[8]);
  const double l2 = dot(n, n);
  return l2 > 0 ? n * frsqrt(l2) : ng;
}

template <bool PARAB = true>
__device__ __forceinline__ d3 face_normal(int type, cf64 par, int face, d3 lp) {
  if (type == ODW_PRIM_BOX) {
    const double s = (face & 1) ? 1.0 : -1.0;
    const int a = face >> 1;
    return mk(a == 0 ? s : 0.0, a == 1 ? s : 0.0, a == 2 ? s : 0.0);
  }
  if (type == ODW_PRIM_SPHERE) return lp * frsqrt(dot(lp, lp));
  if (type == ODW_PRIM_CYLINDER || type == ODW_PRIM_CONE || (PARAB && type == ODW_PRIM_PARABOLOID)) {
    if (face == 1) return mk(0, 0, -1);
    if (face == 2) return mk(0, 0, 1);
    double k = 0;
// ... 199 lines not shown
  return use_oth ? q.oth.prim : q.any.prim;
}

__device__ __forceinline__ d3 mirror(d3 r, d3 n) { return r - n * (2.0 * dot(r, n)); }

__device__ __forceinline__ d3 snells_law(d3 r, double n1, double n2, d3 n, bool& tir) {
  const double d = dot(n, r);
  const double mu = n1 * frcp(n2);
  const double root = 1.0 - mu * mu * (1.0 - d * d);
  if (root < 0) { tir = true; return r - n * (2.0 * d); }
  tir = false;
  const d3 perp = r - n * d;
  return perp * mu + n * fsqrt(root);
}

__device__ __forceinline__ d3 line_grating(d3 ray, double n1, double n2, d3 normal, double wavelength_nm,
                                        int order, double lpm, d3 gdir, bool transmission) {
  const double wl = wavelength_nm / 1000;
  ray = ray * (1.0 / sqrt(dot(ray, ray)));
  const d3 sn = normal * (1.0 / sqrt(dot(normal, normal)));
  const d3 g = gdir * (1.0 / sqrt(dot(gdir, gdir)));
  d3 P = cross(g, sn);
  P = P * (1.0 / sqrt(dot(P, P)));
  d3 D = cross(sn, P);
  D = D * (1.0 / sqrt(dot(D, D)));
  const double mu = n1 / n2, d = 1000 / lpm;
  const double T = (order * wl) / (n1 * d);
  const double V = (mu * dot(ray, sn)) / dot(sn, sn);
  const double W = (mu * mu - 1 + T * T - 2 * mu * T * dot(ray, D)) / dot(sn, sn);
  const double sq = sqrt((2 * V) * (2 * V) - 4 * W);
  const double Q0 = (-2 * V + sq) / 2, Q1 = (-2 * V - sq) / 2;
  const double Q = transmission ? fmin(Q0, Q1) : fmax(Q0, Q1);
  const d3 S = ray * mu - D * T + sn * Q;
  return S * -1.0;
}

__device__ __forceinline__ d3 rotate(d3 axis, double angle, d3 v) {
  const double l2 = dot(axis, axis);
  if (l2 == 0) return v;
  const d3 k = axis * (1.0 / sqrt(l2));
  double s, c;
  sincos_bounded(angle, s, c);
  return v * c + cross(k, v) * s + k * (dot(k, v) * (1.0 - c));
}
__device__ __forceinline__ double acos_clamped(double x) { return acos(fmax(-1.0, fmin(1.0, x))); }

__device__ __forceinline__ void surface_draw(const DeviceSurfaceSampler* sp, double theta_in, double theta_refl,
                                             uint64_t ray, uint64_t seed, uint32_t ordinal, uint32_t stream,
                                             double& theta, double& phi) {
  const DeviceSurfaceSampler S = *sp;
  int k = 0;
  if (S.axis != ODW_SURF_AXIS_NONE) {
    const double c = S.axis == ODW_SURF_AXIS_THETA_IN ? theta_in : theta_refl;
    const double kf = fmin(fmax((c - S.lo) * S.inv_step, 0.0), (double)(S.n_family - 1));
    const int k0 = (int)floor(kf);
    const double frac = kf - (double)k0;
    uint32_t m0 = (uint32_t)ray, m1 = (uint32_t)(ray >> 32), m2 = ordinal, m3 = stream + 16u;
    philox4x32_10(m0, m1, m2, m3, (uint32_t)seed, (uint32_t)(seed >> 32));
    k = k0 + (u53(m0, m1) < frac ? 1 : 0);
  }
  uint32_t c0 = (uint32_t)ray, c1 = (uint32_t)(ray >> 32), c2 = ordinal, c3 = stream;
  philox4x32_10(c0, c1, c2, c3, (uint32_t)seed, (uint32_t)(seed >> 32));
  double u_phi = u53(c0, c1);
  const double u_t = u53(c2, c3);
  if (S.n_atoms) {
    double acc = 0.0;
    for (int j = 0; j < S.n_atoms; ++j) {
      const double pj = S.atom_mass[(size_t)k * (size_t)S.n_atoms + j];
      if (u_phi < acc + pj) {
        theta = S.atom_theta[j][0] + S.atom_theta[j][1] * theta_in + S.atom_theta[j][2] * theta_refl;
        phi = S.atom_phi[j][0] != 0.0 ? S.atom_phi[j][1] + (u_phi - acc) / pj * (S.atom_phi[j][2] - S.atom_phi[j][1]) : S.atom_phi[j][1];
        return;
      }
      acc += pj;
    }
    u_phi = fmin((u_phi - acc) / (1.0 - acc), 0.99999999999999989);
  }
  TableView tv;
  tv.phi_tab = S.phi_tab + (size_t)k * (size_t)S.n_phi_knots * 2;
  tv.t_tab = S.t_tab + (size_t)k * (size_t)S.n_t_rows * (size_t)S.n_t_knots * 2;
  tv.t_guide = S.t_guide + (size_t)k * (size_t)S.n_t_rows * (size_t)(S.n_guide + 1);
  tv.n_phi_knots = S.n_phi_knots; tv.n_t_knots = S.n_t_knots; tv.n_t_rows = S.n_t_rows; tv.n_guide = S.n_guide;
  tv.phi_guide = nullptr; tv.n_phi_guide = 0;
  sample_tables(tv, u_phi, u_t, theta, phi);
}

__device__ __forceinline__ int pick_sampler(const DeviceSurfaceSampler* samplers, int first, double mu) {
  int best = first;
  double dist = INFINITY;
  for (int j = first; j >= 0; j = samplers[j].next) {
    const double m = samplers[j].mu;
    if (m == 0.0) return j;
    const double d = (m < 0 || mu <= 0) ? ((m < 0) == (mu <= 0) ? 0.0 : INFINITY) : fabs(log(m / mu));
    if (d < dist) { dist = d; best = j; }
  }
  return best;
}

__device__ __noinline__ d3 scatter(const DeviceSurfaceSampler* samplers, int s_primary, int s_modify,
                                   uint64_t ray, uint64_t seed, uint32_t ordinal, d3 din, d3 ideal, d3 n, double mu) {
  if (s_primary < 0 && s_modify < 0) return ideal;
  if (s_primary >= 0 && samplers[s_primary].next >= 0) s_primary = pick_sampler(samplers, s_primary, mu);
  const double nl = sqrt(dot(n, n));
  const double theta_in = acos_clamped(dot(din, n) / nl);
  const double theta_refl = acos_clamped(dot(ideal, n) / (sqrt(dot(ideal, ideal)) * nl));
  d3 out = ideal;
  double theta, phi;
  if (s_primary >= 0) {
    surface_draw(samplers + s_primary, theta_in, theta_refl, ray, seed, ordinal, 1u + ODW_SURF_PRIMARY, theta, phi);
    out = rotate(n, phi, rotate(cross(n, din), theta, n));
  }
  if (s_modify >= 0) {
    surface_draw(samplers + s_modify, theta_in, theta_refl, ray, seed, ordinal, 1u + ODW_SURF_MODIFY, theta, phi);
    out = rotate(out, phi, rotate(cross(out, din), theta, out));
  }
  return out * (1.0 / sqrt(dot(out, out)));
}

__device__ __noinline__ void next_hit_block(unsigned long long* hit_count, uint32_t block, volatile uint32_t* hit_state, bool leader) {
  if (leader) {
    const unsigned long long base = atomicAdd(hit_count, (unsigned long long)block);
    hit_state[0] = (uint32_t)base;
    hit_state[1] = (uint32_t)(base >> 32);
  }
}

#ifndef ODW_HIST_WIN
#define ODW_HIST_WIN 88
#endif
__device__ __forceinline__ void hist_window_open(uint32_t* win, int ix, int iy, int nx, int ny) {
  atomicAdd(win + 2, (uint32_t)min(ix, 4095) | (1u << 20));
  atomicAdd(win + 3, (uint32_t)min(iy, 4095) | (1u << 20));
  if (atomicCAS(win, 0u, ~0u) == 0u) {
    volatile uint32_t* vw = win;
    const uint32_t sx = vw[2], sy = vw[3];
    const int mx = (sx >> 20) ? (int)((sx & 0xfffffu) / (sx >> 20)) : ix, my = (sy >> 20) ? (int)((sy & 0xfffffu) / (sy >> 20)) : iy;
    vw[1] = (uint32_t)max(0, min(my - ODW_HIST_WIN / 2, ny - ODW_HIST_WIN));
    vw[0] = (uint32_t)max(0, min(mx - ODW_HIST_WIN / 2, nx - ODW_HIST_WIN)) + 1u;
  }
}
__device__ __forceinline__ bool hist_window_add(uint32_t* win, int ix, int iy, int nx, int ny) {
  volatile uint32_t* vw = win;
  uint32_t x1 = vw[0];
  if (x1 == 0u) {
    hist_window_open(win, ix, iy, nx, ny);
    x1 = vw[0];
  }
  if (x1 == 0u || x1 == ~0u) return false;
  const uint32_t dx = (uint32_t)ix - (x1 - 1u), dy = (uint32_t)iy - vw[1];
  if (dx >= (uint32_t)ODW_HIST_WIN || dy >= (uint32_t)ODW_HIST_WIN) return false;
  atomicAdd(win + 4 + dx * ODW_HIST_WIN + dy, 1u);
  return true;
}
__device__ __forceinline__ unsigned long long power_quanta(double power) {
  const double c = power > 0.0 ? fmin(power, ODW_POWER_MAX) : 0.0;
  return (unsigned long long)(long long)rint(c * (double)(1ull << ODW_POWER_QUANTUM_BITS));
}
template <bool BLOCKS, int CS = 256, bool CA = false, bool POWER = false, class PT>
__device__ __forceinline__ void record_hit(const PT& P, uint64_t ray, int group, d3 p, d3 d,
                                           double power, bool entering, uint32_t* cnt,
                                           volatile uint32_t* hit_state, uint32_t* win = nullptr) {
  if (P.flags & ODW_TRACE_RECORD_HITS) {
    const uint64_t active = __ballot(1);
    const int lane = __lane_id();
    const int leader = __ffsll((unsigned long long)active) - 1;
    const uint32_t n_act = __popcll(active);
// ... 37 lines not shown
      vd2* rw = reinterpret_cast<vd2*>(row);
      __builtin_nontemporal_store((vd2){p.x, p.y}, rw);
      __builtin_nontemporal_store((vd2){p.z, d.x}, rw + 1);
      __builtin_nontemporal_store((vd2){d.y, d.z}, rw + 2);
      __builtin_nontemporal_store((vd2){power, __longlong_as_double((long long)tag)}, rw + 3);
      if (BLOCKS && row_of) row_of[ray - P.first_ray] = (uint32_t)slot;
      if (BLOCKS && pts) {
        double* q = pts + slot;
        __builtin_nontemporal_store(p.x, q);
        __builtin_nontemporal_store(p.y, q + P.out.hit_capacity);
        __builtin_nontemporal_store(p.z, q + 2 * P.out.hit_capacity);
      }
    } else if (CA) {
      atomicAdd(&cnt[ODW_CNT_HITS_DROPPED * CS], 1u);
    } else {
      cnt[ODW_CNT_HITS_DROPPED * CS] += 1u;
    }
  }
  if ((P.flags & ODW_TRACE_HISTOGRAM) && P.det_enabled) {
#pragma clang fp contract(off)
    cdetector det = as_const(opaque(P.det));
    if (det->group < 0 || det->group == group) {
      const d3 r = p - mk(det->origin[0], det->origin[1], det->origin[2]);
      const double x = dot(r, mk(det->ex[0], det->ex[1], det->ex[2]));
      const double y = dot(r, mk(det->ey[0], det->ey[1], det->ey[2]));
      const double fx = floor((x - det->x_lo) * det->x_scale);
      const double fy = floor((y - det->y_lo) * det->y_scale);
      if (fx >= 0 && fx < det->nx_f && fy >= 0 && fy < det->ny_f) {
        const int ix = (int)fx, iy = (int)fy;
        if (!(win && hist_window_add(win, ix, iy, det->nx, det->ny)))
          atomicAdd(P.out.hist + ((size_t)ix * (size_t)det->ny + (size_t)iy), 1ull);
        if constexpr (POWER)
          atomicAdd(P.out.hist + ((size_t)(det->nx * det->ny) + (size_t)(ix * det->ny + iy)), power_quanta(power));
      } else if (CA)
        atomicAdd(&cnt[ODW_CNT_HIST_OVERFLOW * CS], 1u);
      else
        cnt[ODW_CNT_HIST_OVERFLOW * CS] += 1u;
    }
  }
}

typedef const TraceParams ODW_CONST* ckargs;
template <bool POWER>
__device__ __noinline__ void record_hit_flat(ckargs kargs, uint64_t ray, int group, d3 p, d3 d, double power,
                                             bool entering, uint32_t* cnt, uint32_t* hit_state, uint32_t* win) {
  const uint64_t a = (uint64_t)(uintptr_t)kargs;
  const uint64_t u = ((uint64_t)(uint32_t)__builtin_amdgcn_readfirstlane((uint32_t)(a >> 32)) << 32) |
                     (uint64_t)(uint32_t)__builtin_amdgcn_readfirstlane((uint32_t)a);
  record_hit<true, 256, false, POWER>(*(ckargs)(uintptr_t)u, ray, group, p, d, power, entering, cnt, hit_state, win);
}

__device__ __noinline__ void record_segment(odw_segment* segs, uint64_t capacity, unsigned long long* seg_count,
                                            uint64_t ray, int ordinal, int medium, d3 p1, d3 p2, double power) {
  const uint64_t slot = atomicAdd(seg_count, 1ull);
  if (slot < capacity) {
    double2* row = reinterpret_cast<double2*>(segs + slot);
    const uint64_t tag = (ray & 0xFFFFFFFFFFull) | ((uint64_t)(ordinal & 0xFFF) << 40) |
                         ((uint64_t)((medium + 1) & 0xFFF) << 52);
    row[0] = make_double2(p1.x, p1.y);
    row[1] = make_double2(p1.z, p2.x);
    row[2] = make_double2(p2.y, p2.z);
    row[3] = make_double2(power, __longlong_as_double((long long)tag));
  }
}

__device__ __forceinline__ uint32_t wave_sum(uint32_t v) {
#pragma unroll
  for (int off = 32; off > 0; off >>= 1) v += __shfl_xor(v, off);
  return v;
}

struct RayInit { d3 point, dir; double power; };
__device__ __noinline__ RayInit generate_ray(const DeviceSource* sp, uint64_t ray, uint64_t seed) {
  RayInit r;
  double up, ut, t, phi;
  csource src = as_const(sp);
  ray_uniforms(ray, seed, up, ut);
  sample_source(src, up, ut, t, phi);
  make_ray(src, t, phi, r.point, r.dir);
  r.power = src->power;
  return r;
}

template <bool BVH, bool STOCH, bool LEAN, bool POWER = false>
__device__ __forceinline__ void interact(const TraceParams& P, cf64 group_f64, ci32 group_i32, cf64 group_gdir, int g,
                                         int gtype, bool record, d3 n, bool entering, uint64_t ray, int nint,
                                         uint32_t* cnt, uint32_t* hit_state, uint32_t* win, d3 point, d3& dir, double& power,
                                         int& medium, int& seq, bool& alive) {
  if (record) {
    cnt[ODW_CNT_RECORDED_HITS * 256] += 1u;
    if (BVH) record_hit<false, 256, false, POWER>(P, ray, g, point, dir, power, entering, cnt, hit_state);
    else record_hit_flat<POWER>((ckargs)__builtin_amdgcn_kernarg_segment_ptr(), ray, g, point, dir, power, entering, cnt,
                         hit_state, win);
  }
  if (gtype == ODW_OPT_MIRROR) {
#if ODW_DOUBLE == 7
    d3 ideal = mirror(dir, n);
    { const d3 again = mirror(mk(opq(dir.x), dir.y, dir.z), n); ideal = again.x == ideal.x ? ideal : again; }
#else
    const d3 ideal = mirror(dir, n);
#endif
    if (STOCH) dir = scatter(P.samplers, P.group_sampler[2 * g], P.group_sampler[2 * g + 1], ray, P.seed, (uint32_t)nint,
                             dir, ideal, n, 1.0);
    else dir = ideal;
    power *= group_f64[4 * g + 1];
    ++seq;
  } else if (gtype == ODW_OPT_LENS) {
    const double n1 = (medium >= 0) ? group_f64[4 * medium] : 1.0;
    double n2 = 1.0;
    if (entering) { medium = g; n2 = group_f64[4 * g]; }
    bool tir;
#if ODW_DOUBLE == 7
    d3 ideal = snells_law(dir, n1, n2, n, tir);
    { bool tir2; const d3 again = snells_law(mk(opq(dir.x), dir.y, dir.z), n1, n2, n, tir2); ideal = again.x == ideal.x ? ideal : again; tir = tir & tir2; }
#else
    const d3 ideal = snells_law(dir, n1, n2, n, tir);
#endif
    if (STOCH) dir = scatter(P.samplers, P.group_sampler[2 * g], P.group_sampler[2 * g + 1], ray, P.seed, (uint32_t)nint,
                             dir, ideal, n, tir ? -1.0 : n1 / n2);
    else dir = ideal;
    if (!entering && !tir && medium == g) { medium = -1; ++seq; }
  } else if (gtype == ODW_OPT_ABSORBER) {
    power = 0;
    ++seq;
  } else if (LEAN || gtype == ODW_OPT_VACUUM) {
    ++seq;
  } else {
    const d3 gd = mk(group_gdir[3 * g], group_gdir[3 * g + 1], group_gdir[3 * g + 2]);
    const double lpm = group_f64[4 * g + 3];
    const int order = group_i32[4 * g + 3];
    if (group_i32[4 * g + 2] == 0) {
      if (entering) {
        const double nn = (medium >= 0) ? group_f64[4 * medium] : 1.0;
        dir = line_grating(dir, nn, nn, n, P.wavelength, order, lpm, gd, false);
        ++seq;
      }
    } else if (entering) {
      if (medium >= 0) {
        atomicAdd(P.out.counters + ODW_CNT_GRATING_IN_MEDIUM, 1ull);
        cnt[ODW_CNT_DIED * 256] += 1u;
        alive = false;
      }
      medium = g;
      dir = line_grating(dir, 1.0, group_f64[4 * g], n, P.wavelength, order, lpm, gd, true);
    } else {
      const double n1 = (medium >= 0) ? group_f64[4 * medium] : 1.0;
      bool tir;
      dir = snells_law(dir, n1, 1.0, n, tir);
      if (!tir) { medium = -1; ++seq; }
    }
  }
}

template <bool STOCH, bool LEAN, bool POWER, class SPEC, int PI>
__device__ __forceinline__ void spec_hit(const TraceParams& P, const SceneView& sv, cf64 group_f64, ci32 group_i32,
                                         cf64 group_gdir, int face, uint64_t ray, int nint, uint32_t* cnt,
                                         uint32_t* hit_state, uint32_t* win, d3 point, d3& dir, double& power, int& medium, int& seq,
                                         int& skip, int& only, bool& alive) {
  constexpr int flags = SPEC::flags(PI), g = SPEC::group(PI);
  cf64 pf = sv.prim_f64 + (size_t)PI * 16;
  d3 n = face_normal<SPEC::parab()>(SPEC::type(PI), pf + 12, face, xf_point_nz<SPEC::xf(PI)>(pf, point));
  if constexpr ((flags & ODW_FLAG_FLIP_NORMAL) != 0) n = n * -1.0;
  n = xf_vec_t_nz<SPEC::xf(PI)>(pf, n);
#if ODW_DOUBLE == 6
  {
    d3 n2 = face_normal<SPEC::parab()>(SPEC::type(PI), pf + 12, face, xf_point_nz<SPEC::xf(PI)>(pf, mk(opq(point.x), point.y, point.z)));
    if constexpr ((flags & ODW_FLAG_FLIP_NORMAL) != 0) n2 = n2 * -1.0;
    n2 = xf_vec_t_nz<SPEC::xf(PI)>(pf, n2);
    n = n2.x == n.x ? n : n2;
  }
#endif
  const bool entering = dot(dir, n) < 0;
  if (entering) n = n * -1.0;
  interact<false, STOCH, LEAN, POWER>(P, group_f64, group_i32, group_gdir, g, SPEC::gtype(g), SPEC::record(g), n, entering, ray,
                               nint, cnt, hit_state, win, point, dir, power, medium, seq, alive);
  const double out = entering ? -dot(dir, n) : dot(dir, n);
  if constexpr ((flags & ODW_FLAG_CONVEX) != 0) skip = out > 0 ? (flags >> ODW_SOLID_SHIFT) : -1;
  else skip = -1;
  if constexpr ((flags & ODW_FLAG_ISOLATED) != 0) only = out < 0 ? (flags >> ODW_SOLID_SHIFT) : -1;
  else only = -1;
}
template <bool STOCH, bool LEAN, bool POWER, class SPEC, int... PI>
__device__ __forceinline__ void spec_hits(const TraceParams& P, const SceneView& sv, cf64 group_f64, ci32 group_i32,
                                          cf64 group_gdir, int prim, int face, uint64_t ray, int nint, uint32_t* cnt,
                                          uint32_t* hit_state, uint32_t* win, d3 point, d3& dir, double& power, int& medium, int& seq,
                                          int& skip, int& only, bool& alive, IndexList<int, PI...>) {
  (void)((prim == PI ? (spec_hit<STOCH, LEAN, POWER, SPEC, PI>(P, sv, group_f64, group_i32, group_gdir, face, ray, nint, cnt, hit_state, win,
                                                  point, dir, power, medium, seq, skip, only, alive), true)
                     : false) || ...);
}

__device__ __forceinline__ void close_hit_block(const TraceParams& P, volatile uint32_t* hit_state, uint32_t next_scene) {
  if (!P.out.hit_block) {
    if (P.batch.n_scenes && __lane_id() == 0) hit_state[3] = next_scene;
    return;
  }
  odw_hit* hits = P.out.hits;
  unsigned long long* hit_count = P.out.hit_count;
  if (P.batch.n_scenes) {
    const uint32_t cur = __builtin_amdgcn_readfirstlane(hit_state[3]);
    hits += (size_t)cur * P.out.hit_capacity;
    hit_count += 4 * cur;
  }
  const uint32_t hit_used = hit_state[2];
  const uint64_t hit_base = ((uint64_t)hit_state[1] << 32) | hit_state[0];
  if (hit_used < P.out.hit_block) {
    const uint32_t left = P.out.hit_block - hit_used;
    for (uint32_t k = __lane_id(); k < left; k += 64)
      if (hit_base + hit_used + k < P.out.hit_capacity) hits[hit_base + hit_used + k].tag = ODW_TAG_UNUSED;
    const uint64_t at = hit_base + hit_used;
    const uint64_t in_buf = at < P.out.hit_capacity ? (P.out.hit_capacity - at < left ? P.out.hit_capacity - at : left) : 0;
    if (__lane_id() == 0 && in_buf) atomicAdd(hit_count + 1, (unsigned long long)in_buf);
  }
  if (__lane_id() == 0) {
    hit_state[0] = 0u; hit_state[1] = 0u; hit_state[2] = P.out.hit_block; hit_state[3] = next_scene;
  }
}

template <bool ON> struct HitBlockState {
  __device__ static __forceinline__ uint32_t* lds() {
    __shared__ uint32_t state[4 * 4 + 4 + ODW_HIST_WIN * ODW_HIST_WIN];
    return state;
  }
};
template <> struct HitBlockState<false> {
  __device__ static __forceinline__ uint32_t* lds() { return nullptr; }
};

#ifndef ODW_CHUNK
#define ODW_CHUNK 2048ull
#endif
#ifndef ODW_REFILL_MIN
#define ODW_REFILL_MIN 16
#endif
#ifndef ODW_WAVES_PER_SIMD
#define ODW_WAVES_PER_SIMD 4
#endif
#ifndef ODW_WAVES_PER_SIMD_BVH
#define ODW_WAVES_PER_SIMD_BVH 4
#endif
template <bool BVH, bool STOCH, bool SEG, bool LEAN = false, class SPEC = NoSpec, bool BATCH = false, bool POWER = false>
__device__ __forceinline__ void trace_body(const TraceParams& P) {
  static_assert(!BATCH || (!BVH && !SEG), "batch launches: flat kernels, no segment rows");
  extern __shared__ int bvh_stack[];
  __shared__ uint32_t cnt_lds[ODW_CNT_LDS * 256];
#pragma unroll
  for (int k = 0; k < ODW_CNT_LDS; ++k) cnt_lds[k * 256 + threadIdx.x] = 0;
#define ODW_COUNT(k) (cnt_lds[(k) * 256 + threadIdx.x] += 1u)
  const DeviceScene& sc = P.scene;
  const DeviceLimits& lim = P.lim;
  SceneView sv;
  sv.prim_f64 = as_const(sc.prim_f64);
  sv.prim_hdr = as_const(sc.prim_hdr);
  sv.prim_i32 = as_const(sc.prim_i32);
  sv.cond_i32 = as_const(sc.cond_i32);
  cf64 group_f64 = as_const(sc.group_f64);
  ci32 group_i32 = as_const(sc.group_i32);
  cf64 group_gdir = as_const(sc.group_gdir);
  cu64 seq_mask = as_const(sc.seq_mask);
  uint32_t scene = 0, unit_scene = 0;
  const uint32_t lane = __lane_id();
  uint64_t next = 0, chunk_end = 0;
  bool alive = false;
  uint64_t i = 0;
  d3 point = mk(0, 0, 0), dir = mk(0, 0, 1);
  double power = 0;
  int seq = 0, nint = 0, medium = -1;
  int skip = -1;
  int only = -1;
  uint32_t* hit_lds = HitBlockState<!BVH>::lds();
  uint32_t* hist_win = BVH ? nullptr : hit_lds + 16;
  if (!BVH) {
    if (threadIdx.x < 16) hit_lds[threadIdx.x] = (threadIdx.x & 3) == 2 ? P.out.hit_block : 0u;
    for (int k = threadIdx.x; k < 4 + ODW_HIST_WIN * ODW_HIST_WIN; k += 256) hist_win[k] = 0u;
    __syncthreads();
  }
#ifdef ODW_FLAT_STATS
  uint64_t flat_t[3] = {0, 0, 0};
  uint64_t flat_mark = __builtin_readcyclecounter();
#define ODW_FTIME(k) do { const uint64_t t_ = __builtin_readcyclecounter(); flat_t[(k)] += t_ - flat_mark; flat_mark = t_; } while (0)
#else
#define ODW_FTIME(k) do {} while (0)
#endif
  for (;;) {
    ODW_FTIME(2);
    const uint64_t idle = __ballot(!alive);
    if (idle && (idle == ~0ull || __popcll(idle) >= ODW_REFILL_MIN)) {
      if (next >= chunk_end) {
        unsigned long long c = 0;
        if (lane == (uint32_t)(__ffsll((unsigned long long)__ballot(1)) - 1)) c = atomicAdd(P.out.chunk_counter, 1ull);
        const uint64_t chunk = ((uint64_t)(uint32_t)__builtin_amdgcn_readfirstlane((uint32_t)(c >> 32)) << 32) |
                               (uint64_t)(uint32_t)__builtin_amdgcn_readfirstlane((uint32_t)c);
        if (BATCH) {
          const uint32_t g = (uint32_t)chunk, cps = P.batch.chunks_per_scene;
          if (chunk < (uint64_t)cps * P.batch.n_scenes) {
            unit_scene = g / cps;
            next = (uint64_t)(g - unit_scene * cps) * P.chunk;
            chunk_end = next + P.chunk < P.batch.rays ? next + P.chunk : P.batch.rays;
          } else {
            next = chunk_end = 0;
          }
        } else {
        next = chunk * (uint64_t)P.chunk;
        if (next > P.n_rays) next = P.n_rays;
        chunk_end = next + P.chunk < P.n_rays ? next + P.chunk : P.n_rays;
        }
      }
      uint64_t avail = next < chunk_end ? chunk_end - next : 0;
      if (BATCH && avail && unit_scene != scene) {
        if (idle != ~0ull) {
          avail = 0;
        } else {
          close_hit_block(P, hit_lds + (threadIdx.x >> 6) * 4, unit_scene);
          scene = unit_scene;
          const size_t off = (size_t)scene * (size_t)P.batch.stride;
          sv.prim_f64 = as_const(sc.prim_f64 + off);
          sv.prim_hdr = as_const(sc.prim_hdr + off);
          group_f64 = as_const(sc.group_f64 + off);
          group_gdir = as_const(sc.group_gdir + off);
        }
      }
      const uint32_t rank = __popcll(idle & ((1ull << lane) - 1ull));
      const uint32_t want = __popcll(idle);
      const uint32_t take = want < avail ? want : (uint32_t)avail;
      if (!alive && rank < take) {
        i = next + rank;
        if (P.ray_origins) {
          point = mk(P.ray_origins[i], P.ray_origins[P.ray_stride + i], P.ray_origins[2 * P.ray_stride + i]);
          dir = mk(P.ray_dirs[i], P.ray_dirs[P.ray_stride + i], P.ray_dirs[2 * P.ray_stride + i]);
          dir = dir * (1.0 / sqrt(dot(dir, dir)));
          power = P.ray_powers ? P.ray_powers[i] : 1.0;
        } else if (BATCH && P.batch.gen_dirs) {
          const double* gd = P.batch.gen_dirs;
          const uint64_t gs = P.batch.gen_stride;
          dir = mk(gd[i], gd[gs + i], gd[2 * gs + i]);
          if (P.batch.gen_origins) point = mk(P.batch.gen_origins[i], P.batch.gen_origins[gs + i], P.batch.gen_origins[2 * gs + i]);
          else point = mk(gd[3 * gs], gd[3 * gs + 1], gd[3 * gs + 2]);
          power = as_const(P.source)->power;
        } else {
          const RayInit r = generate_ray(P.source, P.first_ray + i, P.seed);
          point = r.point; dir = r.dir; power = r.power;
#if ODW_DOUBLE == 8
          {
            uint32_t lo = (uint32_t)(P.first_ray + i);
            asm volatile("" : "+v"(lo));
            const RayInit r2 = generate_ray(P.source, ((P.first_ray + i) & ~0xFFFFFFFFull) | lo, P.seed);
            dir = r2.dir.x == dir.x ? dir : r2.dir;
          }
#endif
        }
        seq = 0; nint = 0; medium = -1; skip = -1; only = -1;
        alive = true;
      }
      next += take;
      if (take == 0 && idle == ~0ull) break;
    }
    ODW_FTIME(0);
    if (alive) {
      if (nint >= lim.max_intersections) {
        ODW_COUNT(ODW_CNT_CAPPED);
        alive = false;
      } else {
      ++nint;
      uint64_t mask = sc.all_mask;
      if (sc.seq_enabled) mask = (seq < sc.seq_len) ? seq_mask[seq] : 0ull;
      mask &= ~sc.ignore_mask;
      double t_hit;
      int face;
      const int prim = nearest<BVH, SPEC>(sc, sv, lim, point, dir, medium, mask, t_hit, face,
                                          bvh_stack + threadIdx.x, skip, BVH ? -1 : only);
      if (!BVH && prim < 0 && only >= 0) {
        only = -1;
        --nint;
        continue;
      }
      ODW_FTIME(1);
      if (SEG)
        record_segment(P.out.segs, P.out.seg_capacity, P.out.seg_count, P.first_ray + i, nint - 1, medium, point,
                       point + dir * (prim < 0 ? lim.max_ray_length : t_hit), power);
      if (prim < 0) {
        ODW_COUNT(ODW_CNT_ESCAPED);
        alive = false;
      } else {
      point = point + dir * t_hit;
      if (!LEAN && medium >= 0) {
        const double L = group_f64[4 * medium + 2];
        if (L == 0) power = 0;
        else if (L < INFINITY) power = exp(-t_hit / L);
      }
      uint32_t* cnt = cnt_lds + threadIdx.x;
      uint32_t* hit_state = hit_lds + (threadIdx.x >> 6) * 4;
      if constexpr (SPEC::enabled) {
        spec_hits<STOCH, LEAN, POWER, SPEC>(P, sv, group_f64, group_i32, group_gdir, prim, face, P.first_ray + i, nint, cnt, hit_state,
                              hist_win, point, dir, power, medium, seq, skip, only, alive, __make_integer_seq<IndexList, int, SPEC::N>{});
      } else {
      cf64 pf = sv.prim_f64 + (size_t)prim * 16;
      ci32 pi = sv.prim_i32 + 4 * prim;
      d3 n;
      if (BVH && pi[0] == ODW_PRIM_TRIANGLE) {
        n = tri_normal(pf, sc.tri_nrm ? sc.tri_nrm + (size_t)prim * 9 : nullptr, point);
        if (pi[2] & ODW_FLAG_FLIP_NORMAL) n = n * -1.0;
      } else {
        n = face_normal<BVH>(pi[0], pf + 12, face, xf_point(pf, point));
        if (pi[2] & ODW_FLAG_FLIP_NORMAL) n = n * -1.0;
        n = xf_vec_t(pf, n);
      }
      const bool entering = dot(dir, n) < 0;
      if (entering) n = n * -1.0;
      const int g = pi[1];
      interact<BVH, STOCH, LEAN, POWER>(P, group_f64, group_i32, group_gdir, g, group_i32[4 * g], group_i32[4 * g + 1] != 0, n,
                                 entering, P.first_ray + i, nint, cnt, hit_state, hist_win, point, dir, power, medium, seq, alive);
      double out = entering ? -dot(dir, n) : dot(dir, n);
      if (BVH && pi[0] == ODW_PRIM_TRIANGLE) {
        out = dot(dir, mk(pf[9], pf[10], pf[11]));
        if (pi[2] & ODW_FLAG_FLIP_NORMAL) out = -out;
      }
      skip = ((pi[2] & ODW_FLAG_CONVEX) && out > 0) ? (pi[2] >> ODW_SOLID_SHIFT) : -1;
      only = (!BVH && (pi[2] & ODW_FLAG_ISOLATED) && out < 0) ? (pi[2] >> ODW_SOLID_SHIFT) : -1;
      }
      if (alive && power < lim.power_tol) { ODW_COUNT(ODW_CNT_DIED); alive = false; }
      }
      }
      if (!alive) {
        cnt_lds[ODW_CNT_SEGMENTS * 256 + threadIdx.x] += (uint32_t)nint;
        ODW_COUNT(ODW_CNT_TRACED_RAYS);
      }
    }
  }
#ifdef ODW_FLAT_STATS
  if (!BVH && lane == 0 && P.dbg)
    for (int k = 0; k < 3; ++k) atomicAdd(P.dbg + 28 + k, (unsigned long long)flat_t[k]);
#endif
  if (!BVH) close_hit_block(P, hit_lds + (threadIdx.x >> 6) * 4, BATCH ? scene : 0u);
  if (!BVH) {
    __syncthreads();
    if (hist_win[0] != 0u) {
      cdetector det = as_const(opaque(P.det));
      const uint32_t x0 = hist_win[0] - 1u, y0 = hist_win[1];
      const uint32_t nx = (uint32_t)det->nx, ny = (uint32_t)det->ny;
      for (int k = threadIdx.x; k < ODW_HIST_WIN * ODW_HIST_WIN; k += 256) {
        const uint32_t c = hist_win[4 + k];
        const uint32_t x = x0 + (uint32_t)k / ODW_HIST_WIN, y = y0 + (uint32_t)k % ODW_HIST_WIN;
        if (c && x < nx && y < ny) atomicAdd(P.out.hist + ((size_t)x * ny + y), (unsigned long long)c);
      }
    }
  }
#pragma unroll
  for (int k = 0; k < ODW_CNT_LDS; ++k) {
    const uint32_t s = wave_sum(cnt_lds[k * 256 + threadIdx.x]);
    if (__lane_id() == 0) cnt_lds[k * 256 + (threadIdx.x & ~63u)] = s;
  }
  __syncthreads();
  if (threadIdx.x < ODW_CNT_LDS) {
    const uint32_t* col = cnt_lds + threadIdx.x * 256;
    const uint32_t s = col[0] + col[64] + col[128] + col[192];
    if (s) atomicAdd(P.out.counters + threadIdx.x, (unsigned long long)s);
  }
}

template <bool BVH, bool STOCH, bool SEG, bool LEAN = false, bool BATCH = false, bool POWER = false>
__global__ __launch_bounds__(256, BVH ? ODW_WAVES_PER_SIMD_BVH : ODW_WAVES_PER_SIMD) void odw_trace_kernel(const TraceParams P) {
  trace_body<BVH, STOCH, SEG, LEAN, NoSpec, BATCH, POWER>(P);
}

#ifdef ODW_SPEC_HEADER
#include ODW_SPEC_HEADER
#ifndef ODW_SPEC_WAVES
#define ODW_SPEC_WAVES 4
#endif
#ifndef ODW_SPEC_STOCH
#define ODW_SPEC_STOCH false
#endif
#ifndef ODW_SPEC_BATCH
#define ODW_SPEC_BATCH false
#endif
#ifndef ODW_SPEC_POWER
#define ODW_SPEC_POWER false
#endif
extern "C" __global__ __launch_bounds__(256, ODW_SPEC_WAVES) void odw_spec_kernel(const TraceParams P) {
  trace_body<false, ODW_SPEC_STOCH, false, ODW_SPEC_LEAN, Spec, ODW_SPEC_BATCH, ODW_SPEC_POWER>(P);
}
#endif

__global__ __launch_bounds__(256) void odw_sample_kernel(const DeviceSource* sp, uint64_t first,
                                                         uint64_t n, uint64_t seed,
                                                         double* __restrict__ t_out,
                                                         double* __restrict__ phi_out) {
  const uint64_t stride = (uint64_t)gridDim.x * blockDim.x;
  for (uint64_t i = (uint64_t)blockIdx.x * blockDim.x + threadIdx.x; i < n; i += stride) {
    double up, ut, t, phi;
    ray_uniforms(first + i, seed, up, ut);
    sample_source(as_const(sp), up, ut, t, phi);
    t_out[i] = t;
    phi_out[i] = phi;
  }
}


#define ODW_EMIT_MAX_ATTEMPTS 4096
__device__ __forceinline__ void philox_pair(uint64_t ray, uint64_t seed, uint32_t c2, uint32_t c3,
                                            double& a, double& b) {
  uint32_t c0 = (uint32_t)ray, c1 = (uint32_t)(ray >> 32);
  philox4x32_10(c0, c1, c2, c3, (uint32_t)seed, (uint32_t)(seed >> 32));
  a = u53(c0, c1);
  b = u53(c2, c3);
}

__device__ __forceinline__ double face_point(int type, const double* par, int face, double ua, double ub,
                                             d3& p, d3& n, d3& t) {
  const double two_pi = 6.283185307179586;
  if (type == ODW_PRIM_BOX) {
    const int a = face >> 1, b1 = (a + 1) % 3, b2 = (a + 2) % 3;
    double c[3];
    c[a] = (face & 1) ? par[a] : 0.0;
    c[b1] = ua * par[b1];
    c[b2] = ub * par[b2];
    p = mk(c[0], c[1], c[2]);
    const double s = (face & 1) ? 1.0 : -1.0;
    n = mk(a == 0 ? s : 0.0, a == 1 ? s : 0.0, a == 2 ? s : 0.0);
    t = mk(b1 == 0 ? 1.0 : 0.0, b1 == 1 ? 1.0 : 0.0, b1 == 2 ? 1.0 : 0.0);
    return 1.0;
  }
  double sa, ca;
  sincos_bounded(two_pi * ua, sa, ca);
  if (type == ODW_PRIM_SPHERE) {
    const double z = 2.0 * ub - 1.0, r = sqrt(fmax(0.0, 1.0 - z * z));
    n = mk(r * ca, r * sa, z);
    p = n * par[0];
    t = mk(-sa, ca, 0.0);
    return 1.0;
  }
  if (type == ODW_PRIM_TORUS) {
    double sv, cv;
    sincos_bounded(two_pi * ub, sv, cv);
    const double rho = par[0] + par[1] * cv;
    p = mk(rho * ca, rho * sa, par[1] * sv);
    n = mk(cv * ca, cv * sa, sv);
    t = mk(-sa, ca, 0.0);
    return rho / (par[0] + par[1]);
  }
  const double r1 = par[0], r2 = (type == ODW_PRIM_CONE) ? par[1] : par[0];
  const double h = (type == ODW_PRIM_CONE) ? par[2] : par[1];
  if (face == 0) {
    double z;
    if (r1 == r2) z = h * ub;
    else z = h * (sqrt(r1 * r1 + ub * (r2 * r2 - r1 * r1)) - r1) / (r2 - r1);
    const double k = (r2 - r1) / h, r = r1 + k * z;
    p = mk(r * ca, r * sa, z);
    const double inv = 1.0 / sqrt(1.0 + k * k);
    n = mk(ca * inv, sa * inv, -k * inv);
    t = mk(-sa, ca, 0.0);
    return 1.0;
  }
  const double rr = (face == 1 ? r1 : r2) * sqrt(ub);
  p = mk(rr * ca, rr * sa, face == 1 ? 0.0 : h);
  n = mk(0.0, 0.0, face == 1 ? -1.0 : 1.0);
  t = mk(1.0, 0.0, 0.0);
  return 1.0;
}

__global__ __launch_bounds__(256) void odw_emit_kernel(const DeviceEmitter E, uint64_t first, uint64_t n, uint64_t seed,
                                                       double* __restrict__ origins, double* __restrict__ dirs, uint64_t cs,
                                                       uint64_t rs) {
  const uint64_t stride = (uint64_t)gridDim.x * blockDim.x;
  for (uint64_t i = (uint64_t)blockIdx.x * blockDim.x + threadIdx.x; i < n; i += stride) {
    const uint64_t ray = first + i;
    d3 gp = mk(0, 0, 0), gn = mk(0, 0, 1), gt = mk(1, 0, 0);
    for (uint32_t attempt = 0; attempt < ODW_EMIT_MAX_ATTEMPTS; ++attempt) {
      double u_face, u_acc, ua, ub;
      philox_pair(ray, seed, attempt, 3u, u_face, u_acc);
      philox_pair(ray, seed, attempt, 4u, ua, ub);
      int f = 0, hi = E.n_faces - 1;
      while (f < hi) {
        const int mid = (f + hi + 1) >> 1;
        if (u_face >= E.face_cdf[mid]) f = mid; else hi = mid - 1;
      }
      const int prim = E.face_i32[2 * f], face = E.face_i32[2 * f + 1];
      const double* pf = E.prim_f64 + (size_t)prim * 16;
      const int32_t* pi = E.prim_i32 + 4 * prim;
      if (pi[0] == ODW_PRIM_TRIANGLE) {
#pragma clang fp contract(off)
        const d3 v0 = mk(pf[0], pf[1], pf[2]);
        const d3 e1 = mk(pf[3], pf[4], pf[5]) - v0, e2 = mk(pf[6], pf[7], pf[8]) - v0;
        double a = ua, b = ub;
        if (a + b > 1.0) { a = 1.0 - a; b = 1.0 - b; }
        gp = v0 + (e1 * a + e2 * b);
        const d3 fn = cross(e1, e2);
        gn = fn * (1.0 / sqrt(dot(fn, fn)));
        if (E.tri_nrm) {
          const double* vn = E.tri_nrm + (size_t)prim * 9;
          const d3 mix = mk(vn[0], vn[1], vn[2]) * (1.0 - a - b) + (mk(vn[3], vn[4], vn[5]) * a + mk(vn[6], vn[7], vn[8]) * b);
          gn = mix * (1.0 / sqrt(dot(mix, mix)));
        }
        if (pi[1] & ODW_FLAG_FLIP_NORMAL) gn = gn * -1.0;
        gt = e1 - gn * dot(e1, gn);
        gt = gt * (1.0 / sqrt(dot(gt, gt)));
        break;
      }
      d3 p, nl, tl;
      const double accept = face_point(pi[0], pf + 12, face, ua, ub, p, nl, tl);
      if (u_acc >= accept) continue;
      if (pi[1] & ODW_FLAG_FLIP_NORMAL) nl = nl * -1.0;
      const d3 q = mk(p.x - pf[3], p.y - pf[7], p.z - pf[11]);
      gp = xf_vec_t(pf, q);
      const bool dnf = pi[3] > 0 && cond_opens(E.cond_i32[pi[2]]);
      bool ok = true;
      for (int c = pi[2]; c < pi[2] + pi[3] && (ok || dnf); ++c) {
        const int cw = E.cond_i32[c];
        if (c != pi[2] && cond_opens(cw)) {
          if (ok) break;
          ok = true;
        }
        if (!ok) continue;
        const int qp = cond_operand(cw);
        const double* of = E.prim_f64 + (size_t)qp * 16;
        const double sd = prim_sdist<true>(E.prim_i32[4 * qp], of + 12, xf_point(of, gp));
        if (cw < 0 ? sd > E.dist_tol : sd < -E.dist_tol) ok = false;
      }
      if (!ok) continue;
      gn = xf_vec_t(pf, nl);
      gt = xf_vec_t(pf, tl);
      break;
    }
    double u_t, u_phi;
    philox_pair(ray, seed, 0u, 5u, u_t, u_phi);
    const int k = (int)(u_t * (double)E.n_guide);
    const double theta = inv_cdf(E.t_tab, E.t_guide[k], min(E.t_guide[k + 1] + 1, E.n_t_knots - 1), u_t);
    const double phi = 6.283185307179586 * u_phi;
    d3 d = rotate(gn, phi, rotate(gt, theta, gn));
    d = d * (1.0 / sqrt(dot(d, d)));
    origins[i * rs] = gp.x; origins[cs + i * rs] = gp.y; origins[2 * cs + i * rs] = gp.z;
    dirs[i * rs] = d.x; dirs[cs + i * rs] = d.y; dirs[2 * cs + i * rs] = d.z;
  }
}

__global__ __launch_bounds__(256) void odw_rays_to_components_kernel(const double* __restrict__ o_in, const double* __restrict__ d_in,
                                                                     uint64_t n, double* __restrict__ o_out,
                                                                     double* __restrict__ d_out) {
  const uint64_t stride = (uint64_t)gridDim.x * blockDim.x;
  for (uint64_t i = (uint64_t)blockIdx.x * blockDim.x + threadIdx.x; i < 3 * n; i += stride) {
    const uint64_t ray = i / 3, c = i - 3 * ray;
    o_out[c * n + ray] = o_in[i];
    d_out[c * n + ray] = d_in[i];
  }
}

__global__ __launch_bounds__(256) void odw_batch_rays_kernel(const DeviceSource* sp, uint64_t first, uint64_t n, uint64_t seed,
                                                             double* __restrict__ dirs, double* __restrict__ origins,
                                                             uint64_t stride) {
  const uint64_t step = (uint64_t)gridDim.x * blockDim.x;
  for (uint64_t i = (uint64_t)blockIdx.x * blockDim.x + threadIdx.x; i < n; i += step) {
    const RayInit r = generate_ray(sp, first + i, seed);
    dirs[i] = r.dir.x; dirs[stride + i] = r.dir.y; dirs[2 * stride + i] = r.dir.z;
    if (origins) { origins[i] = r.point.x; origins[stride + i] = r.point.y; origins[2 * stride + i] = r.point.z; }
    else if (i == 0) { dirs[3 * stride] = r.point.x; dirs[3 * stride + 1] = r.point.y; dirs[3 * stride + 2] = r.point.z; }
  }
}

__global__ __launch_bounds__(256) void odw_make_rays_kernel(const DeviceSource* sp, uint64_t first, uint64_t n,
                                                            uint64_t seed, double* __restrict__ origins,
                                                            double* __restrict__ dirs) {
  const uint64_t stride = (uint64_t)gridDim.x * blockDim.x;
  for (uint64_t i = (uint64_t)blockIdx.x * blockDim.x + threadIdx.x; i < n; i += stride) {
    double up, ut, t, phi;
    d3 o, d;
    ray_uniforms(first + i, seed, up, ut);
    sample_source(as_const(sp), up, ut, t, phi);
    make_ray(as_const(sp), t, phi, o, d);
    origins[3 * i] = o.x; origins[3 * i + 1] = o.y; origins[3 * i + 2] = o.z;
    dirs[3 * i] = d.x; dirs[3 * i + 1] = d.y; dirs[3 * i + 2] = d.z;
  }
}

}
```

freecad/optics_design_workbench_amd/csrc/odw_spec.hip:

```cpp
#include <dlfcn.h>
#include <hip/hiprtc.h>
#include <sys/stat.h>
#include <unistd.h>

#include <atomic>
#include <chrono>
#include <map>
#include <memory>
#include <mutex>
#include <thread>

#if !defined(__HIP_DEVICE_COMPILE__)
__asm__(
    ".pushsection .rodata\n"
    ".global odw_src_kernels\nodw_src_kernels:\n.incbin \"odw_kernels.hip\"\n.byte 0\n"
    ".global odw_src_device\nodw_src_device:\n.incbin \"odw_device.h\"\n.byte 0\n"
    ".global odw_src_trace\nodw_src_trace:\n.incbin \"../../../include/odw_trace.h\"\n.byte 0\n"
    ".popsection\n");
#endif
extern "C" const char odw_src_kernels[], odw_src_device[], odw_src_trace[];

namespace {

int spec_max_prims() {
  const char* e = getenv("ODW_SPEC_MAX_PRIMS");
  const int v = e ? atoi(e) : 0;
  return v > 0 ? v : 64;
}
const int kSpecMaxPrims = spec_max_prims();

struct Hiprtc {
  void* lib = nullptr;
  decltype(&hiprtcCreateProgram) create = nullptr;
  decltype(&hiprtcCompileProgram) compile = nullptr;
  decltype(&hiprtcGetProgramLogSize) log_size = nullptr;
  decltype(&hiprtcGetProgramLog) log = nullptr;
  decltype(&hiprtcGetCodeSize) code_size = nullptr;
  decltype(&hiprtcGetCode) code = nullptr;
  decltype(&hiprtcDestroyProgram) destroy = nullptr;
  decltype(&hiprtcVersion) version = nullptr;
  std::string error;
  std::string version_text;
};

Hiprtc& hiprtc() {
  static Hiprtc h;
  static std::once_flag once;
  std::call_once(once, [] {
    for (const char* name : {"libhiprtc.so", "libhiprtc.so.7", "/opt/rocm/lib/libhiprtc.so"}) {
      h.lib = dlopen(name, RTLD_NOW | RTLD_LOCAL);
      if (h.lib) break;
    }
    if (!h.lib) { h.error = std::string("hiprtc not available: ") + dlerror(); return; }
#define ODW_RTC_SYM(field, sym)                                             \
    h.field = reinterpret_cast<decltype(h.field)>(dlsym(h.lib, #sym));      \
    if (!h.field) h.error = "hiprtc: missing symbol " #sym;
    ODW_RTC_SYM(create, hiprtcCreateProgram)
    ODW_RTC_SYM(compile, hiprtcCompileProgram)
    ODW_RTC_SYM(log_size, hiprtcGetProgramLogSize)
    ODW_RTC_SYM(log, hiprtcGetProgramLog)
    ODW_RTC_SYM(code_size, hiprtcGetCodeSize)
    ODW_RTC_SYM(code, hiprtcGetCode)
    ODW_RTC_SYM(destroy, hiprtcDestroyProgram)
    ODW_RTC_SYM(version, hiprtcVersion)
#undef ODW_RTC_SYM
    if (h.version) {
      int major = 0, minor = 0;
      if (h.version(&major, &minor) == HIPRTC_SUCCESS) h.version_text = std::to_string(major) + "." + std::to_string(minor);
    }
  });
  return h;
}

template <class T, class F>
std::string table(const char* type, const char* name, int n, const T* v, F fmt) {
  std::string s = std::string("  static constexpr ") + type + " " + name + "(int i) { constexpr " + type + " T[] = {";
  for (int i = 0; i < std::max(1, n); ++i) s += (i ? ", " : "") + (i < n ? fmt(v[i]) : std::string("0"));
  return s + "}; return T[i]; }\n";
}

std::string spec_ineligible(const HostScene& hs) {
  const int n = hs.n_prims;
  if (n < 1) return "no primitives";
  if (n > kSpecMaxPrims) return "more primitives (" + std::to_string(n) + ") than a compiled kernel takes (" + std::to_string(kSpecMaxPrims) + ")";
  for (int p = 0; p < n; ++p) {
    const int t = hs.prim_i32[4 * p];
    if (t == ODW_PRIM_TRIANGLE) return "facets belong to the BVH kernels";
  }
  if (hs.prim_hdr.size() < (size_t)n * 8 || hs.dead.size() < (size_t)n) return "boxes not built";
  return "";
}

std::string spec_text(const HostScene& hs, int n_samplers) {
  const int n = hs.n_prims, ng = hs.n_groups;
  std::vector<int> type(n), group(n), flags(n), condw(n), dead(n);
  std::vector<unsigned long long> xf(n);
  for (int p = 0; p < n; ++p) {
    type[p] = hs.prim_i32[4 * p];
    group[p] = hs.prim_i32[4 * p + 1];
    flags[p] = hs.prim_i32[4 * p + 2] & ~ODW_FLAG_ISOLATED;
    condw[p] = hs.prim_i32[4 * p + 3];
    const int facemask = (flags[p] >> ODW_FACEMASK_SHIFT) & 0xff;
    dead[p] = facemask == 0;
    const double* m = &hs.prim_f64[16 * (size_t)p];
    unsigned long long w = 0;
    for (int i = 0; i < 12; ++i) {
      if (m[i] != 0.0) w |= 1ull << i;
      if (i % 4 != 3 && m[i] == 1.0) w |= 1ull << (12 + i);
      if (i % 4 != 3 && m[i] == -1.0) w |= 1ull << (24 + i);
    }
    xf[p] = w;
  }
  std::vector<int> box_of(n), box_shared(n, 0);
  {
    std::vector<std::vector<std::vector<int>>> inside(n);
    for (int p = 0; p < n; ++p) {
      const int off = condw[p] & 0xffffff, cnt = (condw[p] >> 24) & 0xff;
      const int end = std::min(off + cnt, (int)hs.cond.size());
      inside[p].push_back({p});
      for (int c = off; c < end; ++c) {
        if (c != off && cond_opens(hs.cond[c])) inside[p].push_back({p});
        if (hs.cond[c] < 0) inside[p].back().push_back(cond_operand(hs.cond[c]));
      }
      for (std::vector<int>& set : inside[p]) {
        std::sort(set.begin(), set.end());
        set.erase(std::unique(set.begin(), set.end()), set.end());
      }
      std::sort(inside[p].begin(), inside[p].end());
    }
    for (int p = 0; p < n; ++p) {
      box_of[p] = p;
      for (int q = 0; q < p; ++q)
        if (!dead[q] && !dead[p] && group[q] == group[p] && inside[q] == inside[p]) { box_of[p] = q; box_shared[q] = 1; break; }
    }
  }
  std::vector<int> gtype(std::max(1, ng)), grec(std::max(1, ng));
  for (int g = 0; g < ng; ++g) { gtype[g] = hs.group_i32[4 * g]; grec[g] = hs.group_i32[4 * g + 1]; }
  auto fi = [](int v) { return std::to_string(v); };
  auto fu = [](unsigned long long v) { char b[32]; snprintf(b, sizeof b, "0x%llxull", v); return std::string(b); };
  std::string s;
  s += "struct Spec {\n  static constexpr bool enabled = true;\n";
  s += "  static constexpr int N = " + std::to_string(n) + ";\n";
  s += table("int", "type", n, type.data(), fi) + table("int", "group", n, group.data(), fi) +
       table("int", "flags", n, flags.data(), fi) + table("int", "cond_word", n, condw.data(), fi) +
       table("bool", "dead", n, dead.data(), fi) + table("int", "box_of", n, box_of.data(), fi) +
       table("bool", "box_shared", n, box_shared.data(), fi) +
       table("int", "cond", (int)hs.cond.size(), hs.cond.data(), fi) +
       table("unsigned long long", "xf", n, xf.data(), fu) + table("int", "gtype", ng, gtype.data(), fi) +
       table("bool", "record", ng, grec.data(), fi);
  bool parab = false;
  for (int p = 0; p < n; ++p) parab |= type[p] == ODW_PRIM_PARABOLOID;
  s += std::string("  static constexpr bool parab() { return ") + (parab ? "true" : "false") + "; }\n";
  s += "  static constexpr bool isolated() { return false; }\n";
  s += "  static constexpr int cond_off(int i) { return cond_word(i) & 0xffffff; }\n"
       "  static constexpr int cond_cnt(int i) { return (cond_word(i) >> 24) & 0xff; }\n";
  s += "  static constexpr unsigned long long umask() { return " + fu(hs.all_mask & ~hs.ignore_mask) + "; }\n";
  s += std::string("  static constexpr bool seq() { return ") + (hs.seq_enabled ? "true" : "false") + "; }\n";
  s += "};\n";
  s += std::string("#define ODW_SPEC_LEAN ") + (hs.lean ? "true" : "false") + "\n";
  s += std::string("#define ODW_SPEC_STOCH ") + (n_samplers > 0 ? "true" : "false") + "\n";
  return s;
}

uint64_t fnv1a(const std::string& s, uint64_t h = 1469598103934665603ull) {
  for (unsigned char c : s) { h ^= c; h *= 1099511628211ull; }
  return h;
}

std::string cache_dir() {
  const char* e = getenv("ODW_KERNEL_CACHE");
  if (e) return *e ? e : "";
  const char* x = getenv("XDG_CACHE_HOME");
  if (x && *x) return std::string(x) + "/odw_trace";
  const char* h = getenv("HOME");
  return h && *h ? std::string(h) + "/.cache/odw_trace" : "";
}

void mkdirs(const std::string& path) {
  for (size_t i = 1; i <= path.size(); ++i)
    if (i == path.size() || path[i] == '/') (void)mkdir(path.substr(0, i).c_str(), 0755);
}

bool spec_compile(const std::string& text, const std::string& arch, std::vector<char>& code, std::string& err) {
  Hiprtc& rtc = hiprtc();
  if (!rtc.error.empty()) { err = rtc.error; return false; }
  const char* headers[] = {odw_src_kernels, odw_src_device, odw_src_trace, text.c_str()};
  const char* names[] = {"odw_kernels.hip", "odw_device.h", "odw_trace.h", "odw_spec.h"};
  hiprtcProgram prog = nullptr;
  if (rtc.create(&prog, "#include \"odw_kernels.hip\"\n", "odw_spec_kernel.hip", 4, headers, names) != HIPRTC_SUCCESS) {
    err = "hiprtcCreateProgram failed";
    return false;
  }
  const std::string a = "--offload-arch=" + arch;
  std::vector<const char*> opts = {a.c_str(), "-std=c++17", "-O3", "-ffp-contract=on", "-DODW_SPEC_HEADER=\"odw_spec.h\""};
  std::vector<std::string> extra;
  if (const char* e = getenv("ODW_SPEC_OPTS")) {
    std::string w;
    for (const char* c = e;; ++c) {
      if (*c == ' ' || *c == 0) { if (!w.empty()) extra.push_back(w); w.clear(); if (!*c) break; }
      else w += *c;
    }
  }
  for (const std::string& x : extra) opts.push_back(x.c_str());
  const hiprtcResult r = rtc.compile(prog, (int)opts.size(), opts.data());
  if (r != HIPRTC_SUCCESS) {
    size_t ls = 0;
    rtc.log_size(prog, &ls);
    std::string log(ls, '\0');
    if (ls) rtc.log(prog, &log[0]);
    err = "hiprtc: compilation of the scene kernel failed:\n" + log.substr(0, 4000);
    rtc.destroy(&prog);
    return false;
  }
  size_t cs = 0;
  rtc.code_size(prog, &cs);
  code.resize(cs);
  if (cs) rtc.code(prog, code.data());
  rtc.destroy(&prog);
  if (!cs) { err = "hiprtc returned no code"; return false; }
  return true;
}

struct SpecKernel {
  hipModule_t mod = nullptr;
  hipFunction_t fn = nullptr;
// ... 10 lines not shown
  std::map<std::string, SpecKernel> cache;
  std::map<std::string, std::shared_ptr<SpecJob>> jobs;
  std::map<std::string, uint64_t> rays;
  std::atomic<int> running{0};
};
SpecGlobal& spec_global() {
  static SpecGlobal* g = new SpecGlobal();
  return *g;
}

std::string spec_cache_file(const std::string& arch, const std::string& opts, const std::string& text) {
  const std::string dir = cache_dir();
  if (dir.empty()) return "";
  uint64_t h = fnv1a(arch + "|" + opts + "|" + text);
  h = fnv1a("|rtc " + hiprtc().version_text + "|hip " + std::to_string((long)HIP_VERSION), h);
  h = fnv1a(odw_src_kernels, h);
  h = fnv1a(odw_src_device, h);
  h = fnv1a(odw_src_trace, h);
  char name[40];
  snprintf(name, sizeof name, "/%016llx.hsaco", (unsigned long long)h);
  return dir + name;
}

bool spec_code(const std::string& text, const std::string& arch, std::vector<char>& code, std::string& err, int& hit,
               double& seconds) {
  const char* xo = getenv("ODW_SPEC_OPTS");
  const std::string file = spec_cache_file(arch, xo ? xo : "", text);
  hit = 0;
  seconds = 0;
  if (!file.empty()) {
    if (FILE* f = fopen(file.c_str(), "rb")) {
      fseek(f, 0, SEEK_END);
      const long sz = ftell(f);
      fseek(f, 0, SEEK_SET);
      if (sz > 0) { code.resize((size_t)sz); if (fread(code.data(), 1, (size_t)sz, f) != (size_t)sz) code.clear(); }
      fclose(f);
      if (!code.empty()) { hit = 2; return true; }
    }
  }
  const auto t0 = std::chrono::steady_clock::now();
  if (!spec_compile(text, arch, code, err)) return false;
  seconds = std::chrono::duration<double>(std::chrono::steady_clock::now() - t0).count();
  if (!file.empty()) {
    mkdirs(cache_dir());
    static std::atomic<unsigned> serial{0};
    const std::string tmp = file + "." + std::to_string((long)getpid()) + "." + std::to_string(serial.fetch_add(1));
    if (FILE* f = fopen(tmp.c_str(), "wb")) {
      const bool ok = fwrite(code.data(), 1, code.size(), f) == code.size();
      fclose(f);
      if (!ok || rename(tmp.c_str(), file.c_str()) != 0) (void)unlink(tmp.c_str());
    }
  }
  return true;
}

void spec_wait_at_exit() {
  for (int k = 0; k < 3000 && spec_global().running.load() > 0; ++k) usleep(10000);
}

enum { kSpecSingle = 0, kSpecBatch = 1, kSpecPower = 2 };
int spec_bind(odw_ctx* ctx, int variant = kSpecSingle) {
  const bool batch = variant != kSpecSingle;
  if (variant == kSpecBatch) {
    ctx->spec_batch_fn = nullptr;
  } else if (variant == kSpecPower) {
    ctx->spec_power_fn = nullptr;
  } else {
    ctx->spec_power_fn = nullptr;
    ctx->spec_power_failed = false;
    ctx->spec_power_wait = nullptr;
    ctx->spec_dirty = false;
    ctx->spec_fn = nullptr;
    ctx->spec_batch_fn = nullptr;
    ctx->spec_batch_failed = false;
    ctx->spec_seconds = 0;
    ctx->spec_cache_hit = 0;
    ctx->spec_pending = false;
  }
  if (ctx->compile_mode == ODW_COMPILE_OFF || !ctx->have_scene) return ODW_OK;
  if (!spec_ineligible(ctx->hs).empty()) return ODW_OK;
  hipDeviceProp_t prop;
  HIPCHK(ctx, hipGetDeviceProperties(&prop, ctx->device));
  const std::string arch = prop.gcnArchName;
  const std::string text = spec_text(ctx->hs, ctx->n_samplers) + (variant == kSpecBatch ? "#define ODW_SPEC_BATCH true\n" : variant == kSpecPower ? "#define ODW_SPEC_POWER true\n" : "");
  const char* xo = getenv("ODW_SPEC_OPTS");
  const std::string jkey = arch + "|" + (xo ? xo : "") + "|" + text;
  const std::string key = std::to_string(ctx->device) + "|" + jkey;
  SpecGlobal& G = spec_global();
  std::unique_lock<std::mutex> lock(G.mu);
  auto it = G.cache.find(key);
  if (it == G.cache.end()) {
    std::vector<char> code;
    std::string err;
    if (ctx->compile_mode == ODW_COMPILE_AUTO) {
      auto jt = G.jobs.find(jkey);
      if (jt == G.jobs.end()) {
        const std::string file = spec_cache_file(arch, xo ? xo : "", text);
        FILE* f = file.empty() ? nullptr : fopen(file.c_str(), "rb");
        if (f) {
          fclose(f);
        } else {
          if (!batch) { ctx->spec_pending = true; ctx->spec_key = jkey; }
          if (variant != kSpecPower && G.rays[jkey] < ctx->spec_hot_rays) return ODW_OK;
          auto job = std::make_shared<SpecJob>();
          G.jobs[jkey] = job;
          if (variant == kSpecPower) ctx->spec_power_wait = &job->done;
          static std::once_flag once;
          std::call_once(once, [] { (void)hiprtc(); atexit(spec_wait_at_exit); });
          G.running.fetch_add(1);
          std::thread([job, text, arch] {
            int hit;
            job->ok = spec_code(text, arch, job->code, job->err, hit, job->seconds);
            job->done.store(true);
            spec_global().running.fetch_sub(1);
          }).detach();
          return ODW_OK;
        }
      } else if (!jt->second->done.load()) {
        if (!batch) { ctx->spec_pending = true; ctx->spec_key = jkey; }
        if (variant == kSpecPower) ctx->spec_power_wait = &jt->second->done;
        return ODW_OK;
      } else {
        std::shared_ptr<SpecJob> job = jt->second;
        if (!job->ok) return fail(ctx, ODW_ERR_DEVICE, job->err);
        code = job->code;
        ctx->spec_seconds = job->seconds;
      }
    }
    if (code.empty()) {
      lock.unlock();
      const bool ok = spec_code(text, arch, code, err, ctx->spec_cache_hit, ctx->spec_seconds);
      lock.lock();
      if (!ok) return fail(ctx, ODW_ERR_DEVICE, err);
      it = G.cache.find(key);
    }
    if (it == G.cache.end()) {
      SpecKernel k;
      hipError_t le = hipModuleLoadData(&k.mod, code.data());
      if (le == hipSuccess) le = hipModuleGetFunction(&k.fn, k.mod, "odw_spec_kernel");
      if (le != hipSuccess && ctx->spec_cache_hit == 2) {
        (void)hipGetLastError();
        if (k.mod) { (void)hipModuleUnload(k.mod); k.mod = nullptr; }
        const std::string file = spec_cache_file(arch, xo ? xo : "", text);
        if (!file.empty()) (void)unlink(file.c_str());
        code.clear();
        lock.unlock();
        const bool ok = spec_code(text, arch, code, err, ctx->spec_cache_hit, ctx->spec_seconds);
        lock.lock();
        if (!ok) return fail(ctx, ODW_ERR_DEVICE, err);
        le = hipModuleLoadData(&k.mod, code.data());
        if (le == hipSuccess) le = hipModuleGetFunction(&k.fn, k.mod, "odw_spec_kernel");
      }
      HIPCHK(ctx, le);
      it = G.cache.find(key);
      if (it == G.cache.end()) it = G.cache.emplace(key, k).first;
    }
  } else {
    ctx->spec_cache_hit = 1;
  }
  if (batch) {
    (variant == kSpecBatch ? ctx->spec_batch_fn : ctx->spec_power_fn) = it->second.fn;
    return ODW_OK;
  }
  ctx->spec_fn = it->second.fn;
  ctx->spec_lean = ctx->hs.lean;
  ctx->spec_stoch = ctx->n_samplers > 0;
  return ODW_OK;
// ... 23 lines not shown
```

freecad/optics_design_workbench_amd/simulation/tracer.py:

```python
import atexit
import ctypes as C
import weakref

import numpy as np

from .. import _native
from .._native import (CNT_NAMES, HIT_DTYPE, POWER_QUANTUM_BITS, SEGMENT_DTYPE, TRACE_HISTOGRAM, TRACE_POWER_HISTOGRAM, TRACE_RECORD_HITS,
                       TRACE_RECORD_SEGMENTS)


_LIVE = weakref.WeakSet()


@atexit.register
def _close_live_tracers():
  for t in list(_LIVE):
    try:
      t.close()
    except Exception:
      pass


class _CudaArrayView:

# ... 58 lines not shown


_POOL = _PinnedPool()


def releasePinnedMemory(keep=0):
  _POOL.trim(keep)


class Tracer:

  def __init__(self, device=0, referenceStrict=None):
    import os
    if referenceStrict is None:
      referenceStrict = os.environ.get('ODW_STRICT', '') not in ('', '0')
    self.referenceStrict = bool(referenceStrict)
    self._lib = _native.lib()
    self._ctx = C.c_void_p()
    self.device = int(device)
    _native.check(None, self._lib.odw_create(self.device, C.byref(self._ctx)), 'odw_create')
    _LIVE.add(self)
    self._det = None
    self._power = False
    self._keep = {}
    if os.environ.get('ODW_COMPILE'):
      self.compileScene(os.environ['ODW_COMPILE'])

  def close(self):
    for extra in getattr(self, '_sweepLanes', None) or []:
      extra.close()
    self._sweepLanes = []
    if self._ctx:
      for p in getattr(self, '_pinned', []):
        self._lib.odw_host_free(self._ctx, p)
      self._pinned = []
      self._lib.odw_destroy(self._ctx)
      self._ctx = C.c_void_p()

  def __del__(self):
    try:
      self.close()
    except Exception:
      pass

  def __enter__(self):
    return self

  def __exit__(self, *a):
    self.close()

  def _chk(self, rc, what):
    _native.check(self._ctx, rc, what)

  def setScene(self, scene):
    if self.referenceStrict:
      import copy
      stripped = copy.copy(scene)
      stripped.prim_flags = np.asarray(scene.prim_flags, dtype=np.int32) & ~np.int32(_native.FLAG_CONVEX)
      d, keep = _native.scene_desc(stripped)
    else:
      d, keep = _native.scene_desc(scene)
    self._chk(self._lib.odw_upload_scene(self._ctx, C.byref(d)), 'odw_upload_scene')
    arr, n, keep = _native.surface_sampler_descs(getattr(scene, 'surface_samplers', None))
    self._chk(self._lib.odw_upload_surface_samplers(self._ctx, arr, C.c_int32(n)), 'odw_upload_surface_samplers')
    self.scene = scene

  def compileScene(self, mode='structure'):
    f = self._lib.odw_compile_scene
    f.argtypes = [C.c_void_p, C.c_int32]
    self._chk(f(self._ctx, _native.COMPILE_MODES[mode]), 'odw_compile_scene')
    self._compileMode = _native.COMPILE_MODES[mode]
    return self.compiledInfo()

  def compileMode(self):
    return getattr(self, '_compileMode', 0)

  def compiledInfo(self):
    f = self._lib.odw_compiled_info
    f.argtypes = [C.c_void_p, C.POINTER(C.c_int32), C.POINTER(C.c_double), C.POINTER(C.c_int32)]
    b, sec, hit = C.c_int32(0), C.c_double(0), C.c_int32(0)
    self._chk(f(self._ctx, C.byref(b), C.byref(sec), C.byref(hit)), 'odw_compiled_info')
    pw = C.c_int32(0)
    self._chk(self._lib.odw_compiled_power_info(self._ctx, C.byref(pw)), 'odw_compiled_power_info')
    return dict(mode=int(b.value), seconds=float(sec.value), cache=int(hit.value), power=int(pw.value))

  def setSurfaceSeed(self, seed):
    self._chk(self._lib.odw_set_surface_seed(self._ctx, C.c_uint64(int(seed))), 'odw_set_surface_seed')

  def setWavelength(self, wavelength_nm):
    self._chk(self._lib.odw_set_wavelength(self._ctx, C.c_double(float(wavelength_nm))), 'odw_set_wavelength')

  def setSource(self, source):
    if hasattr(source, 'face_prim'):
      d, keep = _native.surface_source_desc(source)
      self._chk(self._lib.odw_upload_surface_source(self._ctx, C.byref(d)), 'odw_upload_surface_source')
    else:
      d, keep = _native.source_desc(source)
      self._chk(self._lib.odw_upload_source(self._ctx, C.byref(d)), 'odw_upload_source')
    self.source = source

  def generateRays(self, first, n, seed):
    o = np.empty((int(n), 3))
    d = np.empty((int(n), 3))
    pd = C.POINTER(C.c_double)
    self._chk(self._lib.odw_generate_rays(self._ctx, C.c_uint64(int(first)), C.c_uint64(int(n)),
                                          C.c_uint64(int(seed)), o.ctypes.data_as(pd), d.ctypes.data_as(pd)),
              'odw_generate_rays')
    return o, d

  def setLimits(self, lim):
    d = _native.LimitsDesc(float(lim.max_ray_length), int(lim.max_intersections),
                           float(lim.dist_tol), float(lim.power_tol))
    self._chk(self._lib.odw_set_limits(self._ctx, C.byref(d)), 'odw_set_limits')
    self.limits = lim

  def setDetector(self, det, power=False):
    self._power = False
    if det is None:
      self._chk(self._lib.odw_set_detector(self._ctx, None), 'odw_set_detector')
      self._det = None
      return
    d = _native.DetectorDesc()
    d.group = int(det.get('group', -1))
    d.origin = (C.c_double * 3)(*det['origin'])
    d.ex = (C.c_double * 3)(*det['ex'])
    d.ey = (C.c_double * 3)(*det['ey'])
    d.x_lo, d.x_hi, d.y_lo, d.y_hi = (float(det[k]) for k in ('x_lo', 'x_hi', 'y_lo', 'y_hi'))
    d.nx, d.ny = int(det['nx']), int(det['ny'])
    self._chk(self._lib.odw_set_detector(self._ctx, C.byref(d)), 'odw_set_detector')
    self._det = dict(det)
    if power:
      self._chk(self._lib.odw_enable_power_histogram(self._ctx, C.c_int(1)), 'odw_enable_power_histogram')
      self._power = True

  def reserveHits(self, capacity):
    self._chk(self._lib.odw_reserve_hits(self._ctx, C.c_uint64(int(capacity))), 'odw_reserve_hits')

  def reserveSegments(self, capacity):
    self._chk(self._lib.odw_reserve_segments(self._ctx, C.c_uint64(int(capacity))), 'odw_reserve_segments')

  def _flags(self, record_hits, histogram, record_segments=False):
    return ((TRACE_RECORD_HITS if record_hits else 0) | (TRACE_HISTOGRAM if histogram else 0)
            | (TRACE_RECORD_SEGMENTS if record_segments else 0)
            | (TRACE_POWER_HISTOGRAM if histogram and self._power else 0))

  def trace(self, first, n, seed, record_hits=True, histogram=True, record_segments=False):
    self._chk(self._lib.odw_trace(self._ctx, C.c_uint64(int(first)), C.c_uint64(int(n)), C.c_uint64(int(seed)),
                                  C.c_uint32(self._flags(record_hits, histogram, record_segments))),
              'odw_trace')

  def traceRays(self, origins, directions, powers=None, first=0, record_hits=True, histogram=True,
                record_segments=False):
    o = np.ascontiguousarray(origins, dtype=np.float64).reshape(-1, 3)
    d = np.ascontiguousarray(directions, dtype=np.float64).reshape(-1, 3)
    if o.shape != d.shape:
      raise ValueError('origins and directions differ in shape')
    p = np.ascontiguousarray(powers, dtype=np.float64) if powers is not None else None
    pd = C.POINTER(C.c_double)
    self._chk(self._lib.odw_trace_rays(
        self._ctx, C.c_uint64(int(first)), C.c_uint64(len(o)), o.ctypes.data_as(pd), d.ctypes.data_as(pd),
        p.ctypes.data_as(pd) if p is not None else None,
        C.c_uint32(self._flags(record_hits, histogram, record_segments))), 'odw_trace_rays')

  def setSceneBatch(self, scenes):
    if not len(scenes):
      raise ValueError('empty batch')
    descs, keeps = [], []
# ... 289 lines not shown
```

include/odw_trace.h:

```cpp
#ifndef ODW_TRACE_H
#define ODW_TRACE_H

#ifndef __HIPCC_RTC__
#include <stdint.h>
#endif

#ifdef __cplusplus
extern "C" {
#endif

#define ODW_ABI_VERSION 12

enum {
  ODW_OK = 0,
  ODW_ERR_INVALID = 1,
  ODW_ERR_DEVICE = 2,
  ODW_ERR_NO_SCENE = 3,
  ODW_ERR_CAPACITY = 4,
  ODW_ERR_UNSUPPORTED = 5,
  ODW_BUSY = 6
};

enum {
  ODW_PRIM_BOX = 0,
// ... 102 lines not shown
  const double*  prim_params;
  const int32_t* prim_cond_off;
  int32_t n_conds;
  const int32_t* cond_prim;
  const int32_t* cond_inside;
  int32_t n_faces;
  const int32_t* face_prim;
  const int32_t* face_id;
  const double*  face_area;
  int32_t n_t_knots;
  const double* t_edges;
  const double* t_cdf;
  const double* tri_normals;
} odw_surface_source_desc;

typedef struct odw_limits {
  double max_ray_length;
  int32_t max_intersections;
  double dist_tol;
  double power_tol;
} odw_limits;

typedef struct odw_detector_desc {
  int32_t group;
  double origin[3], ex[3], ey[3];
  double x_lo, x_hi, y_lo, y_hi;
  int32_t nx, ny;
} odw_detector_desc;

typedef struct odw_hit {
  double point[3];
  double direction[3];
  double power;
  uint64_t tag;
} odw_hit;

#define ODW_HIT_RAY(tag)      ((tag) & 0xFFFFFFFFFFFFull)
#define ODW_HIT_GROUP(tag)    (((tag) >> 48) & 0x7FFF)
#define ODW_HIT_ENTERING(tag) ((tag) >> 63)

typedef struct odw_segment {
  double p1[3];
  double p2[3];
  double power;
  uint64_t tag;
} odw_segment;

#define ODW_SEG_RAY(tag)     ((tag) & 0xFFFFFFFFFFull)
#define ODW_SEG_ORDINAL(tag) (((tag) >> 40) & 0xFFF)
#define ODW_SEG_MEDIUM(tag)  ((int32_t)(((tag) >> 52) & 0xFFF) - 1)
#define ODW_SEG_MAX_RAY      (1ull << 40)
#define ODW_SEG_MAX_ORDINAL  4096

enum {
  ODW_CNT_TRACED_RAYS = 0,
  ODW_CNT_RECORDED_HITS = 1,
  ODW_CNT_SEGMENTS = 2,
  ODW_CNT_ESCAPED = 3,
  ODW_CNT_DIED = 4,
  ODW_CNT_CAPPED = 5,
  ODW_CNT_HIST_OVERFLOW = 6,
  ODW_CNT_HITS_DROPPED = 7,
  ODW_CNT_GRATING_IN_MEDIUM = 8,
  ODW_CNT_COUNT = 9
};

#define ODW_TRACE_RECORD_HITS 0x1
#define ODW_TRACE_HISTOGRAM   0x2
#define ODW_TRACE_RECORD_SEGMENTS 0x4
#define ODW_TRACE_POWER_HISTOGRAM 0x8

#define ODW_POWER_QUANTUM_BITS 32
#define ODW_POWER_MAX 1048576.0

typedef struct odw_ctx odw_ctx;

int odw_abi_version(void);
int odw_create(int device, odw_ctx** out);
void odw_destroy(odw_ctx* ctx);
const char* odw_last_error(const odw_ctx* ctx);

int odw_upload_scene(odw_ctx* ctx, const odw_scene_desc* scene);
int odw_upload_source(odw_ctx* ctx, const odw_source_desc* source);
int odw_upload_surface_source(odw_ctx* ctx, const odw_surface_source_desc* source);
int odw_upload_surface_samplers(odw_ctx* ctx, const odw_surface_sampler_desc* samplers,
                                int32_t n);
int odw_set_surface_seed(odw_ctx* ctx, uint64_t seed);
int odw_set_wavelength(odw_ctx* ctx, double wavelength_nm);
int odw_set_limits(odw_ctx* ctx, const odw_limits* limits);
int odw_set_detector(odw_ctx* ctx, const odw_detector_desc* det);
int odw_reserve_hits(odw_ctx* ctx, uint64_t capacity);
int odw_reserve_segments(odw_ctx* ctx, uint64_t capacity);

int odw_trace(odw_ctx* ctx, uint64_t first_ray, uint64_t n_rays, uint64_t seed,
              uint32_t flags);
int odw_trace_rays(odw_ctx* ctx, uint64_t first_ray, uint64_t n_rays,
                   const double* origins, const double* directions,
                   const double* powers, uint32_t flags);
int odw_sync(odw_ctx* ctx);

int odw_reset_results(odw_ctx* ctx);
int odw_reset_hits(odw_ctx* ctx);
int odw_fetch_counters(odw_ctx* ctx, uint64_t* out, int32_t n);
int odw_hit_count(odw_ctx* ctx, uint64_t* n);
int odw_fetch_hits(odw_ctx* ctx, odw_hit* out, uint64_t capacity, uint64_t* n);
int odw_fetch_histogram(odw_ctx* ctx, uint64_t* out, uint64_t n_bins);
int odw_enable_power_histogram(odw_ctx* ctx, int on);
int odw_fetch_power_histogram(odw_ctx* ctx, uint64_t* out, uint64_t n_bins);
int odw_swap_hit_lists(odw_ctx* ctx);
int odw_fetch_swapped_hits(odw_ctx* ctx, odw_hit* out, uint64_t capacity, uint64_t* n);
int odw_release_swapped_hits(odw_ctx* ctx);
int odw_mem_info(odw_ctx* ctx, uint64_t* free_bytes, uint64_t* total_bytes);
int odw_host_alloc(odw_ctx* ctx, uint64_t bytes, void** out);
int odw_host_free(odw_ctx* ctx, void* p);
int odw_segment_count(odw_ctx* ctx, uint64_t* n, uint64_t* dropped);
int odw_fetch_segments(odw_ctx* ctx, odw_segment* out, uint64_t capacity, uint64_t* n);
int odw_reset_segments(odw_ctx* ctx);
int odw_sample(odw_ctx* ctx, uint64_t first_ray, uint64_t n_rays, uint64_t seed,
               double* theta_out, double* phi_out);

int odw_generate_rays(odw_ctx* ctx, uint64_t first_ray, uint64_t n_rays, uint64_t seed,
                      double* origins, double* directions);

int odw_load_hits(odw_ctx* ctx, const odw_hit* rows, uint64_t n);
int odw_hits_select(odw_ctx* ctx, int32_t group, uint64_t* n_rows, uint64_t* n_leaving);
int odw_hits_gather(odw_ctx* ctx, int32_t entering_only, uint64_t stride, odw_hit* out,
                    uint64_t capacity, uint64_t* n);
int odw_hits_columns(odw_ctx* ctx, double* points, double* directions, double* powers, int64_t* is_entering,
                     int64_t* ray_index, uint64_t capacity, uint64_t* n);
int odw_hits_project(odw_ctx* ctx, int32_t key, const double* ex, const double* ey, double* stats);
int odw_hits_range(odw_ctx* ctx, int32_t polar, const double* origin, double* range);
int odw_hits_bin(odw_ctx* ctx, int32_t polar, const double* origin, const double* edges_a, int32_t n_a,
                 const double* edges_b, int32_t n_b, uint64_t* counts);
int odw_hits_bin_power(odw_ctx* ctx, int32_t polar, const double* origin, const double* edges_a, int32_t n_a,
                       const double* edges_b, int32_t n_b, uint64_t* counts, uint64_t* power);
int odw_hits_moments(odw_ctx* ctx, double* mean, double* var);
int odw_plane_screen(const double* cloud, uint64_t n, const double* phis, int32_t n_phi, const double* thetas, int32_t n_theta,
                     double* extent);
int odw_plane_screen_batch(const double* const* clouds, const uint64_t* n, int32_t n_clouds, const double* phis, int32_t n_phi,
                           const double* thetas, int32_t n_theta, double* extent);

#define ODW_COMPILE_OFF 0
#define ODW_COMPILE_STRUCTURE 1
#define ODW_COMPILE_AUTO 2
int odw_compile_scene(odw_ctx* ctx, int32_t mode);
int odw_compiled_info(odw_ctx* ctx, int32_t* bound, double* compile_seconds, int32_t* cache_hit);
int odw_compiled_power_info(odw_ctx* ctx, int32_t* bound);
int odw_compile_check(const odw_scene_desc* scene, const odw_limits* limits, int32_t mode, const char* arch,
                      char* header_out, uint64_t header_capacity, uint64_t* code_bytes);
int odw_build_check(const odw_scene_desc* scene, const odw_limits* limits, int32_t* structure, uint64_t* sizes);

int odw_upload_scene_batch(odw_ctx* ctx, const odw_scene_desc* scenes, int32_t n_scenes);
int odw_trace_batch(odw_ctx* ctx, uint64_t first_ray, uint64_t rays_per_scene, uint64_t seed, uint32_t flags,
                    uint64_t rows_per_scene);
int odw_batch_reserve(odw_ctx* ctx, int32_t n_scenes, uint64_t rays_per_scene, uint64_t rows_per_scene);
int odw_batch_select(odw_ctx* ctx, int32_t scene);
int odw_batch_rows(odw_ctx* ctx, uint64_t* rows, uint64_t* wanted, int32_t n);
int odw_batch_hits_select(odw_ctx* ctx, int32_t group, uint64_t* n_rows, uint64_t* n_leaving, int32_t* ordered);
int odw_batch_hits_sample(odw_ctx* ctx, uint64_t limit, const uint64_t* strides, odw_hit* rows, uint64_t cap, uint64_t* n_out);
int odw_batch_hits_project(odw_ctx* ctx, const double* ex, const double* ey, const int32_t* skip, double* stats, double* moments);
int odw_batch_hits_bin(odw_ctx* ctx, int32_t polar, const double* origins, const double* edges_a, int32_t n_a,
                       const double* edges_b, int32_t n_b, uint64_t* counts);
int odw_batch_hits_begin(odw_ctx* ctx, int32_t group, uint64_t limit);
int odw_batch_hits_sampled(odw_ctx* ctx, int32_t wait, uint64_t* n_rows, uint64_t* n_leaving, int32_t* ordered, odw_hit* rows,
                           uint64_t cap, uint64_t* n_sample);
int odw_batch_hits_measure(odw_ctx* ctx, const double* ex, const double* ey, const int32_t* skip, int32_t polar,
                           const double* edges_a, int32_t n_a, const double* edges_b, int32_t n_b, uint64_t keep);
int odw_batch_hits_measured(odw_ctx* ctx, int32_t wait, double* stats, double* moments, double* origins, uint64_t* counts,
                            uint32_t* flags, odw_hit* keep_rows, uint64_t keep_cap, uint64_t* n_keep);

int odw_archive_append(odw_ctx* ctx, odw_ctx* src, uint64_t* total_rows);
int odw_archive_select(odw_ctx* ctx, int32_t on);
int odw_archive_reset(odw_ctx* ctx);

int odw_device_results(odw_ctx* ctx, void** dptr, uint64_t* n_words, uint64_t* hist_offset_words);
int odw_device_histogram(odw_ctx* ctx, void** dptr, uint64_t* n_bins);
int odw_device_power_histogram(odw_ctx* ctx, void** dptr, uint64_t* n_bins);
int odw_device_counters(odw_ctx* ctx, void** dptr, uint64_t* n);
int odw_stream(odw_ctx* ctx, void** hip_stream);

int odw_timing_enable(odw_ctx* ctx, int on);
int odw_timing_read(odw_ctx* ctx, double* total_ms, uint64_t* launches);

#ifdef __cplusplus
}
#endif
#endif
```

Measured before the change: 9.573 billion rays/s.

## Precompute CDF slopes and specialize ray generation on source structure

Appends precomputed per-knot slopes to the inverse-CDF tables so sampling does a multiply instead of a division and one fewer table load. It also adds a source key (frame pattern, single-row, phi-guide, focal flag) that is baked into the runtime-compiled specialized kernel, so source branches and transform terms become compile-time constants. The cost is larger tables, more spec recompiles when the source changes, and slightly different rounding from the stored slope.

Result: faster. 9.804 billion rays/s, median of 6 (+2.4%).

```diff
diff --git a/freecad/optics_design_workbench_amd/_native.py b/freecad/optics_design_workbench_amd/_native.py
--- a/freecad/optics_design_workbench_amd/_native.py
+++ b/freecad/optics_design_workbench_amd/_native.py
@@ -33,7 +33,7 @@
            'odw_fetch_hits', 'odw_fetch_histogram', 'odw_segment_count', 'odw_fetch_segments', 'odw_reset_segments', 'odw_sample', 'odw_device_histogram',
            'odw_device_counters', 'odw_device_results', 'odw_stream', 'odw_timing_enable', 'odw_timing_read',
            'odw_swap_hit_lists', 'odw_fetch_swapped_hits', 'odw_release_swapped_hits', 'odw_mem_info', 'odw_host_alloc', 'odw_host_free', 'odw_load_hits', 'odw_hits_select', 'odw_hits_gather', 'odw_hits_project', 'odw_hits_range', 'odw_hits_bin', 'odw_hits_moments', 'odw_plane_screen',
-           'odw_compile_scene', 'odw_compiled_info', 'odw_compile_check', 'odw_build_check', 'odw_hits_columns',
+           'odw_compile_scene', 'odw_compiled_info', 'odw_compile_check', 'odw_compile_check_source', 'odw_compiled_source_info', 'odw_upload_source_unguided', 'odw_build_check', 'odw_table_slopes', 'odw_hits_columns',
            'odw_upload_scene_batch', 'odw_trace_batch', 'odw_batch_select', 'odw_batch_rows',
            'odw_plane_screen_batch', 'odw_archive_append', 'odw_archive_select', 'odw_archive_reset', 'odw_batch_hits_select', 'odw_batch_hits_sample', 'odw_batch_hits_project', 'odw_batch_hits_bin',
            'odw_batch_reserve', 'odw_batch_hits_begin', 'odw_batch_hits_sampled', 'odw_batch_hits_measure', 'odw_batch_hits_measured',
@@ -227,16 +227,18 @@
   return d, keep
 
 
-def compile_check(scene, limits, mode='structure', arch=None):
+def compile_check(scene, limits, mode='structure', arch=None, source=None):
   d, keep = scene_desc(scene)
   lim = LimitsDesc(float(limits.max_ray_length), int(limits.max_intersections), float(limits.dist_tol),
                    float(limits.power_tol))
   buf = C.create_string_buffer(1 << 20)
   size = C.c_uint64(0)
-  f = lib().odw_compile_check
-  f.argtypes = [C.POINTER(SceneDesc), C.POINTER(LimitsDesc), C.c_int32, C.c_char_p, C.c_char_p, C.c_uint64,
-                C.POINTER(C.c_uint64)]
-  rc = f(C.byref(d), C.byref(lim), COMPILE_MODES[mode], arch.encode() if arch else None, buf, len(buf), C.byref(size))
+  f = lib().odw_compile_check_source
+  f.argtypes = [C.POINTER(SceneDesc), C.POINTER(LimitsDesc), C.c_int32, C.c_char_p, C.POINTER(SourceDesc), C.c_char_p,
+                C.c_uint64, C.POINTER(C.c_uint64)]
+  sd, keep_source = source_desc(source) if source is not None else (None, None)
+  rc = f(C.byref(d), C.byref(lim), COMPILE_MODES[mode], arch.encode() if arch else None,
+         C.byref(sd) if sd is not None else None, buf, len(buf), C.byref(size))
   check(None, rc, 'odw_compile_check')
   return buf.value.decode(), int(size.value)
 
@@ -258,6 +260,17 @@
     raise NativeError(f'odw_build_check: {ERRORS.get(rc, rc)}: {msg.decode() if msg else ""}')
   names = ('primitives', 'nodes', 'grid_cells', 'grid_items', 'grid_lds_bytes', 'dead_primitives')
   return dict(structure=STRUCTURES[int(structure.value)], **{k: int(v) for k, v in zip(names, sizes)})
+
+
+def table_slopes(cdf, edges):
+  edges = _arr(edges, np.float64)
+  cdf = _arr(cdf, np.float64).reshape(-1, len(edges))
+  out = np.empty_like(cdf)
+  f = lib().odw_table_slopes
+  f.argtypes = [_pd, _pd, C.c_int32, C.c_int32, _pd]
+  rc = f(cdf.ctypes.data_as(_pd), edges.ctypes.data_as(_pd), cdf.shape[0], cdf.shape[1], out.ctypes.data_as(_pd))
+  check(None, rc, 'odw_table_slopes')
+  return out
 
 
 def source_desc(src):
diff --git a/freecad/optics_design_workbench_amd/csrc/odw_build.h b/freecad/optics_design_workbench_amd/csrc/odw_build.h
--- a/freecad/optics_design_workbench_amd/csrc/odw_build.h
+++ b/freecad/optics_design_workbench_amd/csrc/odw_build.h
@@ -46,6 +46,22 @@
       if (cond_opens(cond[c])) return false;
   }
   return true;
+}
+
+inline double table_slope(double cdf0, double edge0, double cdf1, double edge1) {
+  const double num = edge1 - edge0, den = cdf1 - cdf0;
+  if (den == 0.0) return num > 0.0 ? INFINITY : num < 0.0 ? -INFINITY : std::numeric_limits<double>::quiet_NaN();
+  return num / den;
+}
+
+inline void append_slopes(std::vector<double>& tab, size_t n_tables, size_t n_knots) {
+  const size_t n = n_tables * n_knots;
+  tab.resize(3 * n);
+  for (size_t t = 0; t < n_tables; ++t)
+    for (size_t j = 0; j < n_knots; ++j) {
+      const double* a = &tab[2 * (t * n_knots + j)];
+      tab[2 * n + t * n_knots + j] = j + 1 < n_knots ? table_slope(a[0], a[1], a[2], a[3]) : 0.0;
+    }
 }
 
 int scene_host_tables(const odw_scene_desc* s, HostScene& hs, std::string& err) {
diff --git a/freecad/optics_design_workbench_amd/csrc/odw_capi.hip b/freecad/optics_design_workbench_amd/csrc/odw_capi.hip
--- a/freecad/optics_design_workbench_amd/csrc/odw_capi.hip
+++ b/freecad/optics_design_workbench_amd/csrc/odw_capi.hip
@@ -55,6 +55,8 @@
   HostScene hs;
   int compile_mode = 0;
   bool spec_dirty = true;
+  uint64_t source_key = 0;
+  uint64_t spec_source_key = 0;
   hipFunction_t spec_fn = nullptr;
   bool spec_lean = false, spec_stoch = false;
   bool spec_pending = false;
@@ -400,6 +402,12 @@
     int rc = build_bvh(ctx);
     if (rc) return rc;
   }
+  {
+    uint64_t want = ctx->spec_source_key;
+    if (!explicit_rays && !ctx->batch_launch) want = ctx->source_key;
+    else if (ctx->spec_dirty) want = 0;
+    if (want != ctx->spec_source_key) { ctx->spec_source_key = want; ctx->spec_dirty = true; }
+  }
   if (ctx->spec_dirty) {
     if (spec_bind(ctx) != ODW_OK) ctx->spec_fn = nullptr;
   }
@@ -820,6 +828,7 @@
   ctx->compile_mode = mode;
   ctx->spec_dirty = true;
   ctx->spec_fn = nullptr;
+  ctx->spec_source_key = ctx->source_key;
   if (mode == ODW_COMPILE_OFF || !ctx->have_scene || !ctx->have_limits) return ODW_OK;
   HIPCHK(ctx, hipSetDevice(ctx->device));
   if (ctx->bvh_dirty) {
@@ -837,6 +846,12 @@
   return ODW_OK;
 }
 
+int odw_compiled_source_info(odw_ctx* ctx, uint64_t* structure) {
+  if (!ctx || !structure) return fail(ctx, ODW_ERR_INVALID, "odw_compiled_source_info: bad argument");
+  *structure = (ctx->spec_fn && !ctx->spec_dirty && !ctx->bvh_dirty) ? ctx->spec_source_key : 0;
+  return ODW_OK;
+}
+
 int odw_compiled_power_info(odw_ctx* ctx, int32_t* bound) {
   if (!ctx || !bound) return fail(ctx, ODW_ERR_INVALID, "odw_compiled_power_info: bad argument");
   *bound = (ctx->spec_fn && ctx->spec_power_fn && !ctx->spec_dirty && !ctx->bvh_dirty) ? ctx->compile_mode : 0;
@@ -845,6 +860,12 @@
 
 int odw_compile_check(const odw_scene_desc* scene, const odw_limits* limits, int32_t mode, const char* arch,
                       char* header_out, uint64_t header_capacity, uint64_t* code_bytes) {
+  return odw_compile_check_source(scene, limits, mode, arch, nullptr, header_out, header_capacity, code_bytes);
+}
+
+int odw_compile_check_source(const odw_scene_desc* scene, const odw_limits* limits, int32_t mode, const char* arch,
+                             const odw_source_desc* source, char* header_out, uint64_t header_capacity,
+                             uint64_t* code_bytes) {
   if (!scene || !limits || mode != ODW_COMPILE_STRUCTURE)
     return fail(nullptr, ODW_ERR_INVALID, "odw_compile_check: bad argument");
   HostScene tmp;
@@ -855,7 +876,8 @@
   compute_boxes(tmp, limits->dist_tol, boxes);
   const std::string why = spec_ineligible(tmp);
   if (!why.empty()) return fail(nullptr, ODW_ERR_UNSUPPORTED, "odw_compile_check: " + why);
-  const std::string text = spec_text(tmp, 0);
+  const std::string text = spec_text(tmp, 0) +
+      (source ? spec_source_text(spec_source_key(source->xform, source->n_t_rows, true, std::isfinite(source->focal_length))) : "");
   if (header_out && header_capacity) {
     const size_t k = std::min<size_t>(text.size(), (size_t)header_capacity - 1);
     std::memcpy(header_out, text.data(), k);
@@ -896,6 +918,18 @@
     sizes[4] = (uint64_t)A.grid.lds_bytes;
     sizes[5] = dead;
   }
+  return ODW_OK;
+}
+
+int odw_table_slopes(const double* cdf, const double* edges, int32_t n_tables, int32_t n_knots, double* slopes) {
+  if (!cdf || !edges || !slopes || n_tables < 1 || n_knots < 2)
+    return fail(nullptr, ODW_ERR_INVALID, "odw_table_slopes: bad argument");
+  const size_t nt = (size_t)n_tables, nk = (size_t)n_knots;
+  std::vector<double> tab(nt * nk * 2);
+  for (size_t t = 0; t < nt; ++t)
+    for (size_t j = 0; j < nk; ++j) { tab[2 * (t * nk + j)] = cdf[t * nk + j]; tab[2 * (t * nk + j) + 1] = edges[j]; }
+  append_slopes(tab, nt, nk);
+  std::memcpy(slopes, tab.data() + 2 * nt * nk, nt * nk * sizeof(double));
   return ODW_OK;
 }
 
@@ -959,6 +993,8 @@
         }
       }
     }
+    append_slopes(ptab, nf, np);
+    append_slopes(ttab, nf * rows, nt);
     odw_ctx::SurfaceBufs& sb = ctx->surf_bufs[(size_t)i];
     int rc;
     if ((rc = upload(ctx, sb.phi_tab, ptab.data(), ptab.size() * sizeof(double)))) return rc;
@@ -1012,7 +1048,13 @@
   return ODW_OK;
 }
 
-int odw_upload_source(odw_ctx* ctx, const odw_source_desc* s) {
+static int upload_source(odw_ctx* ctx, const odw_source_desc* s, bool guides);
+
+int odw_upload_source(odw_ctx* ctx, const odw_source_desc* s) { return upload_source(ctx, s, true); }
+
+int odw_upload_source_unguided(odw_ctx* ctx, const odw_source_desc* s) { return upload_source(ctx, s, false); }
+
+static int upload_source(odw_ctx* ctx, const odw_source_desc* s, bool guides) {
   if (!ctx || !s) return fail(ctx, ODW_ERR_INVALID, "odw_upload_source: null argument");
   if (s->n_phi_knots < 2 || s->n_t_knots < 2 || s->n_t_rows < 1 ||
       (s->n_t_rows != 1 && s->n_t_rows != s->n_phi_knots - 1))
@@ -1025,7 +1067,8 @@
     return fail(ctx, ODW_ERR_INVALID, "phi cdf must run from 0 to 1");
   std::vector<double> ptab((size_t)np * 2), ttab((size_t)rows * nt * 2);
   for (int i = 0; i < np; ++i) { ptab[2 * i] = s->phi_cdf[i]; ptab[2 * i + 1] = s->phi_edges[i]; }
-  std::vector<int32_t> guide((size_t)rows * (kGuide + 1));
+  const int n_guide = guides ? kGuide : 1;
+  std::vector<int32_t> guide((size_t)rows * (n_guide + 1));
   for (int r = 0; r < rows; ++r) {
     const double* cdf = s->t_cdf + (size_t)r * nt;
     if (cdf[0] != 0.0 || cdf[nt - 1] != 1.0) return fail(ctx, ODW_ERR_INVALID, "theta cdf rows must run from 0 to 1");
@@ -1035,14 +1078,16 @@
       dst[2 * i] = cdf[i];
       dst[2 * i + 1] = s->t_edges[i];
     }
-    int32_t* g = guide.data() + (size_t)r * (kGuide + 1);
+    int32_t* g = guide.data() + (size_t)r * (n_guide + 1);
     int j = 0;
-    for (int k = 0; k <= kGuide; ++k) {
-      const double x = (double)k / (double)kGuide;
+    for (int k = 0; k <= n_guide; ++k) {
+      const double x = (double)k / (double)n_guide;
       while (j + 1 < nt && cdf[j + 1] <= x) ++j;
       g[k] = j;
     }
   }
+  append_slopes(ptab, 1, (size_t)np);
+  append_slopes(ttab, (size_t)rows, (size_t)nt);
   int rc;
   if ((rc = upload(ctx, ctx->phi_tab, ptab.data(), ptab.size() * sizeof(double)))) return rc;
   if ((rc = upload(ctx, ctx->t_tab, ttab.data(), ttab.size() * sizeof(double)))) return rc;
@@ -1064,18 +1109,20 @@
   d.phi_tab = (const double*)ctx->phi_tab.p;
   d.t_tab = (const double*)ctx->t_tab.p;
   d.t_guide = (const int32_t*)ctx->t_guide.p;
-  d.phi_guide = (const int32_t*)ctx->phi_guide.p;
-  d.n_phi_guide = kPhiGuide;
+  d.phi_guide = guides ? (const int32_t*)ctx->phi_guide.p : nullptr;
+  d.n_phi_guide = guides ? kPhiGuide : 0;
   d.n_phi_knots = np;
   d.n_t_knots = nt;
   d.n_t_rows = rows;
-  d.n_guide = kGuide;
+  d.n_guide = n_guide;
   if ((rc = upload(ctx, ctx->d_source, &ctx->h_source, sizeof(DeviceSource)))) return rc;
   HIPCHK(ctx, hipStreamSynchronize(ctx->stream));
   ctx->P.source = (const DeviceSource*)ctx->d_source.p;
   ctx->P.wavelength = s->wavelength;
   ctx->have_source = true;
   ctx->emitter_active = false;
+  ctx->source_key = spec_source_key(ctx->h_source);
+  if (ctx->spec_source_key && ctx->spec_source_key != ctx->source_key) ctx->spec_dirty = true;
   return ODW_OK;
 }
 
@@ -1140,6 +1187,7 @@
     ttab[2 * i] = s->t_cdf[i];
     ttab[2 * i + 1] = s->t_edges[i];
   }
+  append_slopes(ttab, 1, (size_t)nt);
   std::vector<int32_t> guide((size_t)kGuide + 1);
   for (int k = 0, j = 0; k <= kGuide; ++k) {
     const double x = (double)k / (double)kGuide;
@@ -1174,6 +1222,7 @@
   ctx->P.wavelength = s->wavelength;
   ctx->have_source = true;
   ctx->emitter_active = true;
+  ctx->source_key = 0;
   return ODW_OK;
 }
 
diff --git a/freecad/optics_design_workbench_amd/csrc/odw_kernels.hip b/freecad/optics_design_workbench_amd/csrc/odw_kernels.hip
--- a/freecad/optics_design_workbench_amd/csrc/odw_kernels.hip
+++ b/freecad/optics_design_workbench_amd/csrc/odw_kernels.hip
@@ -70,37 +70,39 @@
   u_t = u53(c2, c3);
 }
 
-__device__ __forceinline__ double inv_cdf(const double* __restrict__ tab, int lo, int hi, double u) {
+__device__ __forceinline__ double inv_cdf(const double* __restrict__ tab, const double* __restrict__ slope, int lo, int hi,
+                                          double u) {
 #pragma clang fp contract(off)
   while (hi - lo > 1) {
     const int mid = (lo + hi) >> 1;
     if (u >= tab[2 * mid]) lo = mid; else hi = mid;
   }
   const double2 a = *reinterpret_cast<const double2*>(tab + 2 * lo);
-  const double2 b = *reinterpret_cast<const double2*>(tab + 2 * lo + 2);
+  const double sl = slope[lo];
   if (a.x == u) return a.y;
-  const double slope = (b.y - a.y) / (b.x - a.x);
-  const double prod = slope * (u - a.x);
+  const double prod = sl * (u - a.x);
   return prod + a.y;
 }
 
 struct TableView {
   const double* phi_tab; const double* t_tab; const int32_t* t_guide;
+  const double* phi_slope; const double* t_slope;
   int n_phi_knots, n_t_knots, n_t_rows, n_guide;
   const int32_t* phi_guide; int n_phi_guide;
 };
+template <bool KNOWN = false, bool PHI_GUIDE = false, bool SINGLE_ROW = false>
 __device__ __forceinline__ void sample_tables(const TableView& s, double u_phi, double u_t,
                                               double& t_out, double& phi_out) {
 #pragma clang fp contract(off)
   int plo = 0, phi_hi = s.n_phi_knots - 1;
-  if (s.phi_guide) {
+  if (KNOWN ? PHI_GUIDE : s.phi_guide != nullptr) {
     const int k = (int)(u_phi * (double)s.n_phi_guide);
     plo = s.phi_guide[k];
     phi_hi = min(s.phi_guide[k + 1] + 1, s.n_phi_knots - 1);
   }
-  const double phi = inv_cdf(s.phi_tab, plo, phi_hi, u_phi);
+  const double phi = inv_cdf(s.phi_tab, s.phi_slope, plo, phi_hi, u_phi);
   int row = 0;
-  if (s.n_t_rows > 1) {
+  if (KNOWN ? !SINGLE_ROW : s.n_t_rows > 1) {
     const double e0 = s.phi_tab[1], e1 = s.phi_tab[2 * (s.n_phi_knots - 1) + 1];
     int r = (int)floor((phi - e0) / (e1 - e0) * (double)s.n_t_rows);
     r = max(0, min(s.n_t_rows - 1, r));
@@ -112,21 +114,25 @@
     }
   }
   const double* tab = s.t_tab + (size_t)row * (size_t)s.n_t_knots * 2;
+  const double* slope = s.t_slope + (size_t)row * (size_t)s.n_t_knots;
   const int32_t* guide = s.t_guide + (size_t)row * (size_t)(s.n_guide + 1);
   const int k = (int)(u_t * (double)s.n_guide);
   const int lo = guide[k];
   const int hi = min(guide[k + 1] + 1, s.n_t_knots - 1);
-  t_out = inv_cdf(tab, lo, hi, u_t);
+  t_out = inv_cdf(tab, slope, lo, hi, u_t);
   phi_out = phi;
 }
 
+template <bool KNOWN = false, bool PHI_GUIDE = false, bool SINGLE_ROW = false>
 __device__ __forceinline__ void sample_source(csource sp_, double u_phi, double u_t,
                                               double& t_out, double& phi_out) {
   TableView s;
   s.phi_tab = sp_->phi_tab; s.t_tab = sp_->t_tab; s.t_guide = sp_->t_guide;
   s.n_phi_knots = sp_->n_phi_knots; s.n_t_knots = sp_->n_t_knots; s.n_t_rows = sp_->n_t_rows; s.n_guide = sp_->n_guide;
   s.phi_guide = sp_->phi_guide; s.n_phi_guide = sp_->n_phi_guide;
-  sample_tables(s, u_phi, u_t, t_out, phi_out);
+  s.phi_slope = s.phi_tab + (size_t)s.n_phi_knots * 2;
+  s.t_slope = s.t_tab + (size_t)s.n_t_rows * (size_t)s.n_t_knots * 2;
+  sample_tables<KNOWN, PHI_GUIDE, SINGLE_ROW>(s, u_phi, u_t, t_out, phi_out);
 }
 
 template <class P>
@@ -149,10 +155,17 @@
 struct NoSpec {
   static constexpr bool enabled = false;
   static constexpr int N = 0;
+  static constexpr int NG = 0;
   static constexpr unsigned long long xf(int) { return 0xfffull; }
   static constexpr int type(int) { return 0; }
+  static constexpr int gtype(int) { return 0; }
   static constexpr int cond(int) { return 0; }
   static constexpr bool isolated() { return true; }
+};
+struct NoSource {
+  static constexpr bool enabled = false;
+  static constexpr bool single_row = false, phi_guide = false, finite_focal = false;
+  static constexpr unsigned long long xf = 0xfffull;
 };
 template <unsigned long long XF, int IA, int IB, int IC, int IT, class P>
 __device__ __forceinline__ double xf_comb(P m, double a, double b, double c) {
@@ -207,12 +220,13 @@
   c = ((q + 1) & 2) ? -b : b;
 }
 
+template <class SRC = NoSource>
 __device__ __forceinline__ void make_ray(csource s, double t_or_r, double phi,
                                          d3& origin, d3& dir) {
   d3 ldir, lorg;
   double sp, cp;
   sincos_bounded(phi, sp, cp);
-  if (s->finite_focal) {
+  if (SRC::enabled ? SRC::finite_focal : s->finite_focal != 0) {
     double st, ct;
     sincos_bounded(t_or_r, st, ct);
     ldir = mk(st * sp, -st * cp, ct);
@@ -222,8 +236,14 @@
     lorg = mk(t_or_r * cp, -t_or_r * sp, 0.0);
   }
   const d3 ln = ldir * frsqrt(dot(ldir, ldir));
-  const d3 p1 = xf_point(s->m, lorg);
-  const d3 p2 = xf_point(s->m, lorg + ln);
+  d3 p1, p2;
+  if constexpr (SRC::enabled) {
+    p1 = xf_point_nz<SRC::xf>(s->m, lorg);
+    p2 = xf_point_nz<SRC::xf>(s->m, lorg + ln);
+  } else {
+    p1 = xf_point(s->m, lorg);
+    p2 = xf_point(s->m, lorg + ln);
+  }
   const d3 d = p2 - p1;
   origin = p1;
   dir = d * frsqrt(dot(d, d));
@@ -637,10 +657,23 @@
     double bt = INFINITY;
     int bf = 0;
 #define ODW_PICK(T, F) { const bool w_ = (bool)((int)((T) > tol) & ((int)((T) < bt) | ((int)((T) == bt) & (int)((F) < bf)))); bt = w_ ? (T) : bt; bf = w_ ? (F) : bf; }
+    if constexpr (SPEC::enabled) {
+      constexpr int ty = SPEC::type(PI), fm = (SPEC::flags(PI) >> ODW_FACEMASK_SHIFT) & 0xff;
+      constexpr bool quadric = ty == ODW_PRIM_CYLINDER || ty == ODW_PRIM_CONE || ty == ODW_PRIM_PARABOLOID;
+      constexpr bool pair = ty == ODW_PRIM_BOX || (fm & 1) != 0;
+      constexpr bool caps = ty != ODW_PRIM_BOX && ty != ODW_PRIM_SPHERE;
+      if constexpr (pair) {
+        ODW_PICK(c.t0, c.f0)
+        ODW_PICK(c.t1, c.f1)
+      }
+      if constexpr (caps && (quadric ? (fm & 2) != 0 : (fm & 1) != 0)) ODW_PICK(c.t2, c.f2)
+      if constexpr (caps && (quadric ? (fm & 4) != 0 : (fm & 1) != 0)) ODW_PICK(c.t3, c.f3)
+    } else {
     ODW_PICK(c.t0, c.f0)
     ODW_PICK(c.t1, c.f1)
     ODW_PICK(c.t2, c.f2)
     ODW_PICK(c.t3, c.f3)
+    }
 #undef ODW_PICK
     if constexpr (SPEC::enabled) consider_spec<PARAB, SPEC, PI>(sv, q, bt, bf);
     else consider<PARAB>(sv, q, bt, p, bf, group, 0, 0);
@@ -1006,6 +1039,8 @@
   tv.t_guide = S.t_guide + (size_t)k * (size_t)S.n_t_rows * (size_t)(S.n_guide + 1);
   tv.n_phi_knots = S.n_phi_knots; tv.n_t_knots = S.n_t_knots; tv.n_t_rows = S.n_t_rows; tv.n_guide = S.n_guide;
   tv.phi_guide = nullptr; tv.n_phi_guide = 0;
+  tv.phi_slope = S.phi_tab + ((size_t)S.n_family * 2 + (size_t)k) * (size_t)S.n_phi_knots;
+  tv.t_slope = S.t_tab + ((size_t)S.n_family * 2 + (size_t)k) * (size_t)S.n_t_rows * (size_t)S.n_t_knots;
   sample_tables(tv, u_phi, u_t, theta, phi);
 }
 
@@ -1209,7 +1244,45 @@
   return r;
 }
 
-template <bool BVH, bool STOCH, bool LEAN, bool POWER = false>
+template <class SRC>
+__device__ __forceinline__ RayInit generate_ray_spec(csource src, uint64_t ray, uint64_t seed) {
+  RayInit r;
+  double up, ut, t, phi;
+  ray_uniforms(ray, seed, up, ut);
+  sample_source<true, SRC::phi_guide, SRC::single_row>(src, up, ut, t, phi);
+  make_ray<SRC>(src, t, phi, r.point, r.dir);
+  r.power = src->power;
+  return r;
+}
+
+template <class SRC>
+__device__ __noinline__ RayInit generate_ray_spec_call(csource src, uint64_t ray, uint64_t seed) {
+  return generate_ray_spec<SRC>(src, ray, seed);
+}
+
+constexpr bool can_be_medium(int gtype) {
+  return gtype != ODW_OPT_MIRROR && gtype != ODW_OPT_ABSORBER && gtype != ODW_OPT_VACUUM;
+}
+template <class SPEC, int G = 0>
+constexpr int spec_media() {
+  if constexpr (G >= SPEC::NG) return 0;
+  else return (can_be_medium(SPEC::gtype(G)) ? 1 : 0) + spec_media<SPEC, G + 1>();
+}
+template <class SPEC, int K, int G = 0>
+__device__ __forceinline__ double spec_medium_word(cf64 group_f64, int medium, double v) {
+  if constexpr (G < SPEC::NG) {
+    v = spec_medium_word<SPEC, K, G + 1>(group_f64, medium, v);
+    if constexpr (can_be_medium(SPEC::gtype(G))) v = medium == G ? group_f64[4 * G + K] : v;
+  }
+  return v;
+}
+template <class SPEC, int K>
+__device__ __forceinline__ double medium_word(cf64 group_f64, int medium) {
+  if constexpr (SPEC::enabled && spec_media<SPEC>() <= 8) return spec_medium_word<SPEC, K>(group_f64, medium, 0.0);
+  else return group_f64[4 * medium + K];
+}
+
+template <bool BVH, bool STOCH, bool LEAN, bool POWER = false, class SPEC = NoSpec>
 __device__ __forceinline__ void interact(const TraceParams& P, cf64 group_f64, ci32 group_i32, cf64 group_gdir, int g,
                                          int gtype, bool record, d3 n, bool entering, uint64_t ray, int nint,
                                          uint32_t* cnt, uint32_t* hit_state, uint32_t* win, d3 point, d3& dir, double& power,
@@ -1233,7 +1306,7 @@
     power *= group_f64[4 * g + 1];
     ++seq;
   } else if (gtype == ODW_OPT_LENS) {
-    const double n1 = (medium >= 0) ? group_f64[4 * medium] : 1.0;
+    const double n1 = (medium >= 0) ? medium_word<SPEC, 0>(group_f64, medium) : 1.0;
     double n2 = 1.0;
     if (entering) { medium = g; n2 = group_f64[4 * g]; }
     bool tir;
@@ -1258,7 +1331,7 @@
     const int order = group_i32[4 * g + 3];
     if (group_i32[4 * g + 2] == 0) {
       if (entering) {
-        const double nn = (medium >= 0) ? group_f64[4 * medium] : 1.0;
+        const double nn = (medium >= 0) ? medium_word<SPEC, 0>(group_f64, medium) : 1.0;
         dir = line_grating(dir, nn, nn, n, P.wavelength, order, lpm, gd, false);
         ++seq;
       }
@@ -1271,7 +1344,7 @@
       medium = g;
       dir = line_grating(dir, 1.0, group_f64[4 * g], n, P.wavelength, order, lpm, gd, true);
     } else {
-      const double n1 = (medium >= 0) ? group_f64[4 * medium] : 1.0;
+      const double n1 = (medium >= 0) ? medium_word<SPEC, 0>(group_f64, medium) : 1.0;
       bool tir;
       dir = snells_law(dir, n1, 1.0, n, tir);
       if (!tir) { medium = -1; ++seq; }
@@ -1299,7 +1372,7 @@
 #endif
   const bool entering = dot(dir, n) < 0;
   if (entering) n = n * -1.0;
-  interact<false, STOCH, LEAN, POWER>(P, group_f64, group_i32, group_gdir, g, SPEC::gtype(g), SPEC::record(g), n, entering, ray,
+  interact<false, STOCH, LEAN, POWER, SPEC>(P, group_f64, group_i32, group_gdir, g, SPEC::gtype(g), SPEC::record(g), n, entering, ray,
                                nint, cnt, hit_state, win, point, dir, power, medium, seq, alive);
   const double out = entering ? -dot(dir, n) : dot(dir, n);
   if constexpr ((flags & ODW_FLAG_CONVEX) != 0) skip = out > 0 ? (flags >> ODW_SOLID_SHIFT) : -1;
@@ -1366,7 +1439,8 @@
 #ifndef ODW_WAVES_PER_SIMD_BVH
 #define ODW_WAVES_PER_SIMD_BVH 4
 #endif
-template <bool BVH, bool STOCH, bool SEG, bool LEAN = false, class SPEC = NoSpec, bool BATCH = false, bool POWER = false>
+template <bool BVH, bool STOCH, bool SEG, bool LEAN = false, class SPEC = NoSpec, bool BATCH = false, bool POWER = false,
+          class SRC = NoSource>
 __device__ __forceinline__ void trace_body(const TraceParams& P) {
   static_assert(!BATCH || (!BVH && !SEG), "batch launches: flat kernels, no segment rows");
   extern __shared__ int bvh_stack[];
@@ -1465,7 +1539,10 @@
           else point = mk(gd[3 * gs], gd[3 * gs + 1], gd[3 * gs + 2]);
           power = as_const(P.source)->power;
         } else {
-          const RayInit r = generate_ray(P.source, P.first_ray + i, P.seed);
+          RayInit r;
+          if constexpr (SRC::enabled && SRC::finite_focal) r = generate_ray_spec<SRC>(as_const(P.source), P.first_ray + i, P.seed);
+          else if constexpr (SRC::enabled) r = generate_ray_spec_call<SRC>(as_const(P.source), P.first_ray + i, P.seed);
+          else r = generate_ray(P.source, P.first_ray + i, P.seed);
           point = r.point; dir = r.dir; power = r.power;
 #if ODW_DOUBLE == 8
           {
@@ -1511,7 +1588,7 @@
       } else {
       point = point + dir * t_hit;
       if (!LEAN && medium >= 0) {
-        const double L = group_f64[4 * medium + 2];
+        const double L = medium_word<SPEC, 2>(group_f64, medium);
         if (L == 0) power = 0;
         else if (L < INFINITY) power = exp(-t_hit / L);
       }
@@ -1604,8 +1681,11 @@
 #ifndef ODW_SPEC_POWER
 #define ODW_SPEC_POWER false
 #endif
+#ifndef ODW_SPEC_SOURCE
+#define ODW_SPEC_SOURCE NoSource
+#endif
 extern "C" __global__ __launch_bounds__(256, ODW_SPEC_WAVES) void odw_spec_kernel(const TraceParams P) {
-  trace_body<false, ODW_SPEC_STOCH, false, ODW_SPEC_LEAN, Spec, ODW_SPEC_BATCH, ODW_SPEC_POWER>(P);
+  trace_body<false, ODW_SPEC_STOCH, false, ODW_SPEC_LEAN, Spec, ODW_SPEC_BATCH, ODW_SPEC_POWER, ODW_SPEC_SOURCE>(P);
 }
 #endif
 
@@ -1752,7 +1832,7 @@
     double u_t, u_phi;
     philox_pair(ray, seed, 0u, 5u, u_t, u_phi);
     const int k = (int)(u_t * (double)E.n_guide);
-    const double theta = inv_cdf(E.t_tab, E.t_guide[k], min(E.t_guide[k + 1] + 1, E.n_t_knots - 1), u_t);
+    const double theta = inv_cdf(E.t_tab, E.t_tab + (size_t)E.n_t_knots * 2, E.t_guide[k], min(E.t_guide[k + 1] + 1, E.n_t_knots - 1), u_t);
     const double phi = 6.283185307179586 * u_phi;
     d3 d = rotate(gn, phi, rotate(gt, theta, gn));
     d = d * (1.0 / sqrt(dot(d, d)));
diff --git a/freecad/optics_design_workbench_amd/csrc/odw_spec.hip b/freecad/optics_design_workbench_amd/csrc/odw_spec.hip
--- a/freecad/optics_design_workbench_amd/csrc/odw_spec.hip
+++ b/freecad/optics_design_workbench_amd/csrc/odw_spec.hip
@@ -91,6 +91,36 @@
   return "";
 }
 
+unsigned long long xf_pattern(const double* m) {
+  unsigned long long w = 0;
+  for (int i = 0; i < 12; ++i) {
+    if (m[i] != 0.0) w |= 1ull << i;
+    if (i % 4 != 3 && m[i] == 1.0) w |= 1ull << (12 + i);
+    if (i % 4 != 3 && m[i] == -1.0) w |= 1ull << (24 + i);
+  }
+  return w;
+}
+
+enum : uint64_t { kSrcEnabled = 1ull << 63, kSrcSingleRow = 1ull << 40, kSrcPhiGuide = 1ull << 41, kSrcFiniteFocal = 1ull << 42 };
+uint64_t spec_source_key(const double* frame, int n_t_rows, bool phi_guide, bool finite_focal) {
+  return kSrcEnabled | xf_pattern(frame) | (n_t_rows == 1 ? kSrcSingleRow : 0) | (phi_guide ? kSrcPhiGuide : 0) |
+         (finite_focal ? kSrcFiniteFocal : 0);
+}
+uint64_t spec_source_key(const DeviceSource& d) {
+  return spec_source_key(d.m, d.n_t_rows, d.phi_guide != nullptr, d.finite_focal != 0);
+}
+std::string spec_source_text(uint64_t key) {
+  if (!(key & kSrcEnabled)) return "";
+  auto fb = [&](uint64_t bit) { return (key & bit) ? "true" : "false"; };
+  char xf[32];
+  snprintf(xf, sizeof xf, "0x%llxull", (unsigned long long)(key & 0xfffffffffull));
+  return std::string("struct SpecSource {\n  static constexpr bool enabled = true;\n") +
+         "  static constexpr bool single_row = " + fb(kSrcSingleRow) + ";\n" +
+         "  static constexpr bool phi_guide = " + fb(kSrcPhiGuide) + ";\n" +
+         "  static constexpr bool finite_focal = " + fb(kSrcFiniteFocal) + ";\n" +
+         "  static constexpr unsigned long long xf = " + xf + ";\n};\n#define ODW_SPEC_SOURCE SpecSource\n";
+}
+
 std::string spec_text(const HostScene& hs, int n_samplers) {
   const int n = hs.n_prims, ng = hs.n_groups;
   std::vector<int> type(n), group(n), flags(n), condw(n), dead(n);
@@ -102,14 +132,7 @@
     condw[p] = hs.prim_i32[4 * p + 3];
     const int facemask = (flags[p] >> ODW_FACEMASK_SHIFT) & 0xff;
     dead[p] = facemask == 0;
-    const double* m = &hs.prim_f64[16 * (size_t)p];
-    unsigned long long w = 0;
-    for (int i = 0; i < 12; ++i) {
-      if (m[i] != 0.0) w |= 1ull << i;
-      if (i % 4 != 3 && m[i] == 1.0) w |= 1ull << (12 + i);
-      if (i % 4 != 3 && m[i] == -1.0) w |= 1ull << (24 + i);
-    }
-    xf[p] = w;
+    xf[p] = xf_pattern(&hs.prim_f64[16 * (size_t)p]);
   }
   std::vector<int> box_of(n), box_shared(n, 0);
   {
@@ -141,6 +164,7 @@
   std::string s;
   s += "struct Spec {\n  static constexpr bool enabled = true;\n";
   s += "  static constexpr int N = " + std::to_string(n) + ";\n";
+  s += "  static constexpr int NG = " + std::to_string(ng) + ";\n";
   s += table("int", "type", n, type.data(), fi) + table("int", "group", n, group.data(), fi) +
        table("int", "flags", n, flags.data(), fi) + table("int", "cond_word", n, condw.data(), fi) +
        table("bool", "dead", n, dead.data(), fi) + table("int", "box_of", n, box_of.data(), fi) +
@@ -317,7 +341,8 @@
   hipDeviceProp_t prop;
   HIPCHK(ctx, hipGetDeviceProperties(&prop, ctx->device));
   const std::string arch = prop.gcnArchName;
-  const std::string text = spec_text(ctx->hs, ctx->n_samplers) + (variant == kSpecBatch ? "#define ODW_SPEC_BATCH true\n" : variant == kSpecPower ? "#define ODW_SPEC_POWER true\n" : "");
+  const std::string text = spec_text(ctx->hs, ctx->n_samplers) + (variant == kSpecBatch ? "" : spec_source_text(ctx->spec_source_key)) +
+                           (variant == kSpecBatch ? "#define ODW_SPEC_BATCH true\n" : variant == kSpecPower ? "#define ODW_SPEC_POWER true\n" : "");
   const char* xo = getenv("ODW_SPEC_OPTS");
   const std::string jkey = arch + "|" + (xo ? xo : "") + "|" + text;
   const std::string key = std::to_string(ctx->device) + "|" + jkey;
diff --git a/freecad/optics_design_workbench_amd/simulation/tracer.py b/freecad/optics_design_workbench_amd/simulation/tracer.py
--- a/freecad/optics_design_workbench_amd/simulation/tracer.py
+++ b/freecad/optics_design_workbench_amd/simulation/tracer.py
@@ -164,7 +164,11 @@
     self._chk(f(self._ctx, C.byref(b), C.byref(sec), C.byref(hit)), 'odw_compiled_info')
     pw = C.c_int32(0)
     self._chk(self._lib.odw_compiled_power_info(self._ctx, C.byref(pw)), 'odw_compiled_power_info')
-    return dict(mode=int(b.value), seconds=float(sec.value), cache=int(hit.value), power=int(pw.value))
+    key = C.c_uint64(0)
+    f = self._lib.odw_compiled_source_info
+    f.argtypes = [C.c_void_p, C.POINTER(C.c_uint64)]
+    self._chk(f(self._ctx, C.byref(key)), 'odw_compiled_source_info')
+    return dict(mode=int(b.value), seconds=float(sec.value), cache=int(hit.value), power=int(pw.value), source=int(key.value))
 
   def setSurfaceSeed(self, seed):
     self._chk(self._lib.odw_set_surface_seed(self._ctx, C.c_uint64(int(seed))), 'odw_set_surface_seed')
diff --git a/include/odw_trace.h b/include/odw_trace.h
--- a/include/odw_trace.h
+++ b/include/odw_trace.h
@@ -208,6 +208,7 @@
 
 int odw_upload_scene(odw_ctx* ctx, const odw_scene_desc* scene);
 int odw_upload_source(odw_ctx* ctx, const odw_source_desc* source);
+int odw_upload_source_unguided(odw_ctx* ctx, const odw_source_desc* source);
 int odw_upload_surface_source(odw_ctx* ctx, const odw_surface_source_desc* source);
 int odw_upload_surface_samplers(odw_ctx* ctx, const odw_surface_sampler_desc* samplers,
                                 int32_t n);
@@ -274,7 +275,12 @@
 int odw_compiled_power_info(odw_ctx* ctx, int32_t* bound);
 int odw_compile_check(const odw_scene_desc* scene, const odw_limits* limits, int32_t mode, const char* arch,
                       char* header_out, uint64_t header_capacity, uint64_t* code_bytes);
+int odw_compile_check_source(const odw_scene_desc* scene, const odw_limits* limits, int32_t mode, const char* arch,
+                             const odw_source_desc* source, char* header_out, uint64_t header_capacity,
+                             uint64_t* code_bytes);
+int odw_compiled_source_info(odw_ctx* ctx, uint64_t* structure);
 int odw_build_check(const odw_scene_desc* scene, const odw_limits* limits, int32_t* structure, uint64_t* sizes);
+int odw_table_slopes(const double* cdf, const double* edges, int32_t n_tables, int32_t n_knots, double* slopes);
 
 int odw_upload_scene_batch(odw_ctx* ctx, const odw_scene_desc* scenes, int32_t n_scenes);
 int odw_trace_batch(odw_ctx* ctx, uint64_t first_ray, uint64_t rays_per_scene, uint64_t seed, uint32_t flags,
```
